# Ighina/MultimodalTopicSegmentation

Measured on AMD Instinct MI355X. Metric: sentences/sec (fwd+bwd), higher is better.
Workload: dtype bf16; 1 GPU; BASELINE configs[1]: restricted-window transformer tagger d=1792 heads=8 ff=256 radius=15 layers=1 focal loss, 64 docs x 256 sentences per GPU, fwd+bwd+Adam(eps 1e-7), inputs resident in HBM; global_batch_docs=64, sentences_per_doc=256, parallelism=dp1 (document-sharded, RCCL all-reduce)

## Files before the change

include/mts.h:

```cpp
#ifndef MTS_H
#define MTS_H

#include <stddef.h>
#include <stdint.h>

#ifdef __cplusplus
extern "C" {
#endif

typedef enum {
  MTS_OK = 0,
  MTS_ERR_INVALID = 1,
  MTS_ERR_UNSUPPORTED = 2,
  MTS_ERR_LAUNCH = 3,
  MTS_ERR_WORKSPACE = 4,
  MTS_ERR_TIMEOUT = 5
} mts_status;

typedef enum { MTS_F32 = 0, MTS_BF16 = 1 } mts_dtype;

typedef enum { MTS_LOSS_CE = 0, MTS_LOSS_BCE = 1, MTS_LOSS_FOCAL = 2 } mts_loss_kind;

typedef enum { MTS_NT = 0, MTS_NN = 1, MTS_TN = 2, MTS_TT = 3 } mts_gemm_layout;

#define MTS_EPI_BIAS      1u
#define MTS_EPI_RESIDUAL  2u
#define MTS_EPI_GELU      4u
#define MTS_EPI_COLSCALE  8u
#define MTS_EPI_ACCUM    16u
#define MTS_EPI_RELU     32u

const char* mts_last_error(void);
const char* mts_version(void);
int mts_set_option(const char* key, int value);
int mts_async_status(void);
int mts_gemm_last_plan(int* tile, int* splits);
int mts_gemm_set_mid_hook(void (*fn)(void));
size_t mts_wgrad_pair_workspace(int M, int N, int K);
int mts_wgrad_pair(void* stream, int M, int N, int K, const void* A1, const void* B1, float* C1, int ldc1, const void* A2, const void* B2,
                   float* C2t, int ldc2t, int lda, int ldb, int accumulate, void* workspace, size_t workspace_bytes);
int mts_gemm_plan(int a_dtype, int c_dtype, int layout, int M, int N, int K, unsigned epilogue, size_t workspace_bytes,
                  int* tile, int* splits);

int mts_gemm(void* stream, int a_dtype, int c_dtype, int layout, int M, int N, int K,
             const void* A, int lda, const void* B, int ldb, void* C, int ldc,
             const float* bias, const void* residual, int ldr, void* aux, int ldaux,
             unsigned epilogue, float colscale, int ncols_scaled, void* workspace, size_t workspace_bytes);

size_t mts_colsum_workspace(int N);
int mts_colsum(void* stream, int dtype, int M, int N, const void* X, int ldx, float* out, int accumulate,
               void* partial);

int mts_cast(void* stream, int dst_dtype, const float* src, void* dst, size_t n);
int mts_cast_concat(void* stream, int dst_dtype, size_t rows, int D1, int D2, const float* src1, const float* src2, void* dst);
int mts_collate_pad(int src_dtype, int dst_dtype, int B, int Lmax, int D, const void* const* docs, const int64_t* doc_rows, void* dst,
                    float pad_value, int nthreads);
int mts_gather_pad(void* stream, int src_dtype, int dst_dtype, int B, int Lmax, int D,
                   const void* corpus,
                   const int64_t* row_start,
                   int n_docs,
                   const int32_t* doc_index,
                   void* dst,
                   float pad_value);
int mts_gather_segments(void* stream, int src_dtype, int dst_dtype, int B, int Lmax, int D,
                        const void* corpus,
                        const int64_t* row_start,
                        int n_docs,
                        const int32_t* doc_index,
                        const int32_t* seg_ptr,
                        const int32_t* seg_dst,
                        const int32_t* seg_src,
                        int n_listed,
                        const int32_t* dst_len,
                        const int32_t* close_last,
                        void* dst,
                        float pad_value);
int mts_mask_plan(void* stream, int B, int Lmax,
                  const float* targets,
                  const int64_t* row_start,
                  int n_docs,
                  const int32_t* doc_index,
                  const uint64_t* doc_seed,
                  double keep_probability,
                  int32_t* src_row,
                  int32_t* kept);
int mts_gather_rows(void* stream, int src_dtype, int dst_dtype, int B, int Lmax, int D,
                    const void* corpus,
                    const int64_t* row_start,
                    int n_docs,
                    const int32_t* doc_index,
                    const int32_t* src_row,
                    void* dst,
                    float pad_value);
int mts_pca_colsum(void* stream, int dtype, int rows, int D,
                   const void* x,
                   double* sum_out);
int mts_pca_gram(void* stream, int dtype, int rows, int D,
                 const void* x,
                 const float* center,
                 double* gram_out);
int mts_pca_project(void* stream, int in_dtype, int out_dtype, int rows, int D, int k,
                    const void* x,
                    const float* center,
                    const float* w,
                    void* y);
typedef enum { MTS_POOL_NONE = 0, MTS_POOL_MEAN = 1, MTS_POOL_MAX = 2 } mts_pool_stat;
typedef enum { MTS_EDGE_LAST = 0, MTS_EDGE_DELTA_GAP = 1 } mts_edge_mode;
int mts_frame_pool(void* stream, int in_dtype, int out_dtype, int n_sent, int D, int first, int with_std,
                   const void* frames,
                   int64_t total_frames,
                   const int64_t* frame_start,
                   void* out,
                   int64_t ld_out);
int mts_frame_edges(void* stream, int in_dtype, int out_dtype, int n_sent, int D, int mode,
                    const void* frames,
                    int64_t total_frames,
                    const int64_t* frame_start,
                    const uint8_t* doc_last,
                    void* out,
                    int64_t ld_out);

int mts_embed_layernorm_fwd(void* stream, int dtype, int B, int L, int D, const float* x, const float* pos,
                            int pos_offset, const float* type0, const float* gamma, const float* beta, float eps,
                            void* y, void* pre, float* mean, float* rstd, const int32_t* row_src, int n_rows);
int mts_embed_layernorm_fwd_x16(void* stream, int B, int L, int D, const void* x_bf16, const float* pos, int pos_offset, const float* type0,
                                const float* gamma, const float* beta, float eps, void* y, void* pre, float* mean, float* rstd,
                                const int32_t* row_src, int n_rows);
int mts_embed_layernorm_fwd2(void* stream, int dtype, int B, int L, int D1, int D2, const float* x1, const float* x2, const float* pos,
                             int pos_offset, const float* type0, const float* gamma, const float* beta, float eps,
                             void* y, void* pre, float* mean, float* rstd, const int32_t* row_src, int n_rows);
int mts_layernorm_fwd(void* stream, int dtype, int rows, int D, const void* x, const float* gamma,
                      const float* beta, float eps, void* y, float* mean, float* rstd,
                      const float* head_w, const float* head_b, int n_out, float* scores);
size_t mts_layernorm_bwd_workspace(int D);
int mts_layernorm_bwd(void* stream, int dtype, int rows, int D, const void* x, const void* dy,
                      const float* dlogit, const float* head_w, int n_out,
                      const float* gamma, const float* mean, const float* rstd,
                      void* dx, float* dgamma, float* dbeta, float* dxsum, void* partial,
                      const float* beta, float* dhead_w, float* dhead_b);
int mts_layernorm_loss_tail_supported(int dtype, int D, int n_out);
int mts_layernorm_loss_tail(void* stream, int dtype, int rows, int D, const void* x, const float* gamma, const float* beta, float eps,
                            const float* head_w, const float* head_b, int n_out, int loss_kind, int B, int L, int Lt, const float* targets,
                            const int32_t* lengths, float alpha, float gamma_focal, float grad_scale, const int32_t* row_src, int n_rows,
                            float* scores, float* loss_out, void* dx, float* dgamma, float* dbeta, float* dxsum, float* dhead_w,
                            float* dhead_b, void* workspace);
size_t mts_embed_layernorm_bwd_workspace(int B, int L, int D);
int mts_embed_layernorm_bwd(void* stream, int dtype, int B, int L, int D, const void* pre, const void* dh, const float* gamma,
                            const float* mean, const float* rstd, float* dgamma, float* dbeta, float* dtype0, float* dpos,
                            int pos_offset, const int32_t* row0, const int32_t* lengths, int n_rows, void* workspace, size_t workspace_bytes);
int mts_embed_bwd(void* stream, int dtype, int B, int L, int D, const void* dpre, float* dpos, int pos_offset,
                  const int32_t* row0, const int32_t* lengths);

int mts_dropout_fwd(void* stream, int dtype, size_t n, const void* x, const void* residual, void* y, uint8_t* mask,
                    float p, uint64_t seed);
int mts_dropout_bwd(void* stream, int dtype, size_t n, const void* dy, void* dx, const uint8_t* mask, float p);

int mts_gelu_bwd(void* stream, int dtype, size_t n, const void* u, void* dy);
int mts_relu_bwd(void* stream, int dtype, size_t n, const void* u, void* dy);

int mts_ffn_supported(int dtype, int M, int D, int F);
int mts_ffn_fwd(void* stream, int M, int D, int F, const void* a1, const void* w1, const float* b1, const void* w2, const float* b2,
                int relu, void* u, void* f, void* s2);
int mts_ffn_bwd_data(void* stream, int M, int D, int F, const void* ds2, const void* w1, const void* w2, const void* u, int relu,
                     void* du, void* da1);


int mts_band_slots(int radius);
int mts_band_attn_fwd(void* stream, int dtype, int B, int L, int D, int heads, int radius,
                      const void* qkv, const int32_t* lengths, void* ctx, float* probs, const int32_t* row0,
                      float drop_p, uint64_t drop_seed);
size_t mts_band_attn_bwd_workspace(int B, int L, int D);
int mts_band_attn_bwd(void* stream, int dtype, int B, int L, int D, int heads, int radius, float q_scale,
                      const void* qkv, const int32_t* lengths, const float* probs, const void* dctx,
                      void* dqkv, float* dscores, float* dbias, void* workspace, const int32_t* row0, int n_rows,
                      float drop_p, uint64_t drop_seed);

int mts_full_attn_fwd(void* stream, int dtype, int B, int L, int D, int heads, const void* qkv, const int32_t* lengths,
                      void* ctx, float* lse, const int32_t* row0, float drop_p, uint64_t drop_seed);
size_t mts_full_attn_bwd_workspace(int B, int L, int D, int heads);
int mts_full_attn_bwd(void* stream, int dtype, int B, int L, int D, int heads, float q_scale, const void* qkv,
                      const int32_t* lengths, const float* lse, const void* ctx, const void* dctx, void* dqkv, float* dbias,
                      void* workspace, const int32_t* row0, int n_rows, float drop_p, uint64_t drop_seed);

int mts_t5_local_attn_fwd(void* stream, int dtype, int B, int L, int heads, int head_dim, int radius, const void* qkv,
                          const int32_t* lengths, const float* table, int buckets, const int32_t* bucket_of_offset, void* ctx,
                          float* lse, float drop_p, uint64_t drop_seed);
size_t mts_t5_local_attn_bwd_workspace(int B, int L, int heads, int radius);
int mts_t5_local_attn_bwd(void* stream, int dtype, int B, int L, int heads, int head_dim, int radius, const void* qkv,
                          const int32_t* lengths, const float* table, int buckets, const int32_t* bucket_of_offset,
                          const float* lse, const void* ctx, const void* dctx, void* dqkv, float* dtable, void* workspace,
                          float drop_p, uint64_t drop_seed);

int mts_rmsnorm_fwd(void* stream, int dtype, int rows, int D, const void* x, const float* w, float eps, void* y, float* rstd);
size_t mts_rmsnorm_bwd_workspace(int rows, int D);
int mts_rmsnorm_bwd(void* stream, int dtype, int rows, int D, const void* x, const void* dy, const void* dres, const float* w,
                    const float* rstd, void* dx, float* dw, void* workspace);

int mts_pair_score_fwd(void* stream, int dtype, int B, int L, int H, const void* F, int ldf, const void* G, int ldg, float* scores);
int mts_pair_score_bwd(void* stream, int dtype, int B, int L, int H, const void* F, int ldf, const void* G, int ldg,
                       const float* dscores, void* dF, int lddf, void* dG, int lddg);

int mts_gate_merge_fwd(void* stream, int dtype, size_t rows, int W, const void* a, int lda, const void* h1, int ldh1, const void* h2,
                       int ldh2, void* m, int ldm);
int mts_gate_merge_bwd(void* stream, int dtype, size_t rows, int W, const void* a, int lda, const void* h1, int ldh1, const void* h2,
                       int ldh2, const void* dm, int lddm, void* da, int ldda, void* dh1, int lddh1, void* dh2, int lddh2);

size_t mts_segment_cosine_workspace(int n_seg, int n_pair, int W);
int mts_segment_cosine_fwd(void* stream, int dtype, int B, int L, int W, const void* x, int ldx, int n_seg, const int32_t* seg_table,
                           int n_pair, const int32_t* pair_table, float* loss_out, float* pair_cos, void* workspace);
int mts_segment_cosine_bwd(void* stream, int dtype, int B, int L, int W, int n_seg, const int32_t* seg_table, int n_pair,
                           const int32_t* pair_table, const int32_t* row_map, float scale, int accumulate, void* dx, int lddx,
                           void* workspace);

size_t mts_tagger_loss_workspace(int B, int L);
int mts_tagger_loss(void* stream, int loss_kind, int B, int L, int Lt, int n_out, const float* scores,
                    const float* targets, const int32_t* lengths, float alpha, float gamma,
                    float* loss_out, float* dscores, void* workspace, size_t workspace_bytes,
                    const int32_t* row_src, int n_rows);
int mts_greedy_decode(void* stream, int B, int L, int n_out, const float* scores, const int32_t* lengths,
                      float threshold, uint8_t* tags_out);
int mts_segment_decode(void* stream, int B, int L, int n_out,
                       const float* scores,
                       const int32_t* lengths,
                       float threshold, int min_segment, int close_last, int Smax,
                       uint8_t* tags,
                       float* prob,
                       int32_t* seg_end,
                       int32_t* n_seg);
int mts_threshold_sweep(void* stream, int B, int L, int Lt, int n_out, const float* scores, const float* targets,
                        const int32_t* lengths, int T, const float* thresholds, int end_boundary, int32_t* counts_out);
int mts_winpr_sweep(void* stream, int B, int L, int Lt, int n_out, const float* scores, const float* targets,
                    const int32_t* lengths, int T, const float* thresholds, int end_boundary, int k, int32_t* counts_out);
int mts_bootstrap_sums(void* stream, int n, int M, int S, const double* values, uint64_t seed, double* sums);
int mts_head_fwd(void* stream, int dtype, int rows, int D, int n_out, const void* x, int ldx, const float* w,
                 const float* b, float* scores);
int mts_head_bwd_params(void* stream, int dtype, int rows, int D, int n_out, const void* x, int ldx,
                        const float* dscores, float* dw, float* db, void* partial);
int mts_head_bwd_data(void* stream, int dtype, int rows, int D, int n_out, const float* dscores, const float* w,
                      void* dx, int lddx, int accumulate);

int mts_switch_head_fwd(void* stream, int dtype, int B, int L, int D, int n_out, const void* x, int ldx, const float* w,
                        const float* bias, const int32_t* doc_src, const int32_t* doc_head, float* scores);
size_t mts_switch_head_bwd_workspace(int D);
int mts_switch_head_bwd_params(void* stream, int dtype, int B, int L, int D, int n_out, const void* x, int ldx, const float* dscores,
                               const int32_t* doc_src, const int32_t* doc_head, float* dw, float* db, void* workspace);
int mts_switch_head_bwd_data(void* stream, int dtype, int B, int L, int D, int n_out, const float* dscores, const float* w,
                             const int32_t* doc_tgt, void* dx, int lddx);

size_t mts_lstm_workspace(int dtype, int B, int L, int H, int ndir);
int mts_lstm_fwd(void* stream, int dtype, int B, int L, int H, int ndir, const void* xproj, const float* w_hh,
                 const float* b_hh, const int32_t* lengths, void* out, void* gates, float* cells, void* workspace);
int mts_lstm_bwd(void* stream, int dtype, int B, int L, int H, int ndir, const float* w_hh, const int32_t* lengths,
                 const void* out, const void* gates, const float* cells, const void* dout, void* dxproj,
                 float* dw_hh, void* workspace);
int mts_lstm_bwd_recurrence(void* stream, int dtype, int B, int L, int H, int ndir, const float* w_hh, const int32_t* lengths,
                            const void* out, const void* gates, const float* cells, const void* dout, void* dxproj, void* workspace);
int mts_lstm_bwd_whh(void* stream, int dtype, int B, int L, int H, int ndir, const int32_t* lengths, const void* out, const void* dxproj,
                     float* dw_hh, void* workspace);

size_t mts_crf_workspace(int B, int L, int C);
int mts_crf_nll(void* stream, int B, int L, int C, const float* feats, const float* tags, int Lt,
                const int32_t* lengths, const float* trans, float* loss_out, float* dfeats, float* dtrans,
                float* workspace );
int mts_crf_viterbi(void* stream, int B, int L, int C, const float* feats, const int32_t* lengths,
                    const float* trans, float* best_score, int32_t* paths, int32_t* bp_ws);
int mts_crf_marginals(void* stream, int B, int L, int C, int cls, const float* feats, const int32_t* lengths,
                      const float* trans, float* scores, float* logz, float* workspace );
int mts_crf_nll_packed(void* stream, int B, int L, int C, const float* feats, const float* tags, int Lt,
                       const int32_t* lengths, const float* trans, float* loss_out, float* dfeats, float* dtrans,
                       float* workspace, const int32_t* row0, int n_rows);
int mts_crf_viterbi_packed(void* stream, int B, int L, int C, const float* feats, const int32_t* lengths,
                           const float* trans, float* best_score, int32_t* paths, int32_t* bp_ws, const int32_t* row0, int n_rows);
int mts_crf_marginals_packed(void* stream, int B, int L, int C, int cls, const float* feats, const int32_t* lengths,
                             const float* trans, float* scores, float* logz, float* workspace, const int32_t* row0, int n_rows);

int mts_adam_step(void* stream, size_t n, float* param, const float* grad, float* exp_avg, float* exp_avg_sq,
                  float lr, float beta1, float beta2, float eps, int step, float grad_scale, void* bf16_copy);
int mts_sgd_step(void* stream, size_t n, float* param, const float* grad, float* momentum_buf, float lr,
                 float momentum, float weight_decay, int first_step, float grad_scale, void* bf16_copy);
size_t mts_grad_norm_workspace(void);
int mts_grad_norm(void* stream, const float* grad, int n_spans, const size_t* span_begin_host, const size_t* span_end_host,
                  float grad_scale, float* workspace, float* norm_out);
int mts_adam_step_clipped(void* stream, size_t n, float* param, const float* grad, float* exp_avg, float* exp_avg_sq,
                          float lr, float beta1, float beta2, float eps, int step, float grad_scale, void* bf16_copy,
                          const float* total_norm, float max_norm, float clip_value, float* clip_coef_out);
int mts_sgd_step_clipped(void* stream, size_t n, float* param, const float* grad, float* momentum_buf, float lr,
                         float momentum, float weight_decay, int first_step, float grad_scale, void* bf16_copy,
                         const float* total_norm, float max_norm, float clip_value, float* clip_coef_out);
int mts_scale(void* stream, size_t n, float* x, float scale);

#ifdef __cplusplus
}
#endif
#endif
```

multimodaltopicsegmentation_amd/_lib.py:

```python
import ctypes as C
import os

_HWQ_PRESET = 'GPU_MAX_HW_QUEUES' in os.environ
os.environ.setdefault('GPU_MAX_HW_QUEUES', '8')

import torch

if not _HWQ_PRESET and torch.cuda.is_initialized():
    import warnings
    warnings.warn('multimodaltopicsegmentation_amd was imported after the GPU runtime had been initialised: GPU_MAX_HW_QUEUES=8 could not '
                  'take effect (the late-fusion tagger\'s two encoder streams may share a hardware queue next to RCCL: 13.3 instead of 7.7 ms '
                  'per step at 64 x 512).  Import the package first, or export GPU_MAX_HW_QUEUES=8.', RuntimeWarning, stacklevel=2)

_HERE = os.path.dirname(os.path.abspath(__file__))
LIB_PATH = os.path.join(_HERE, 'libmts_hip.so')

if not os.path.exists(LIB_PATH):
    raise ImportError(
        f'{LIB_PATH} not found: the HIP kernel library has not been built. Run '
        '`python multimodaltopicsegmentation_amd/build.py` (needs hipcc; cross-compiles for gfx950 without a GPU). '
        'There is no CPU/PyTorch fallback for the tagger path.')

lib = C.CDLL(LIB_PATH)

F32, BF16 = 0, 1
LOSS_CE, LOSS_BCE, LOSS_FOCAL = 0, 1, 2
NT, NN, TN, TT = 0, 1, 2, 3
POOL_NONE, POOL_MEAN, POOL_MAX = 0, 1, 2
EDGE_LAST, EDGE_DELTA_GAP = 0, 1
EPI_BIAS, EPI_RESIDUAL, EPI_GELU, EPI_COLSCALE, EPI_ACCUM, EPI_RELU = 1, 2, 4, 8, 16, 32

_vp, _i, _f, _u, _sz = C.c_void_p, C.c_int, C.c_float, C.c_uint, C.c_size_t

SIGNATURES = {
    'mts_last_error': (C.c_char_p, []),
    'mts_version': (C.c_char_p, []),
    'mts_set_option': (_i, [C.c_char_p, _i]),
    'mts_gemm_last_plan': (_i, [_vp, _vp]),
    'mts_gemm_set_mid_hook': (_i, [_vp]),
    'mts_gemm_plan': (_i, [_i, _i, _i, _i, _i, _i, _u, _sz, _vp, _vp]),
    'mts_async_status': (_i, []),
    'mts_gemm': (_i, [_vp, _i, _i, _i, _i, _i, _i, _vp, _i, _vp, _i, _vp, _i, _vp, _vp, _i, _vp, _i, _u, _f, _i, _vp, _sz]),
    'mts_wgrad_pair_workspace': (_sz, [_i, _i, _i]),
    'mts_wgrad_pair': (_i, [_vp, _i, _i, _i, _vp, _vp, _vp, _i, _vp, _vp, _vp, _i, _i, _i, _i, _vp, _sz]),
    'mts_colsum_workspace': (_sz, [_i]),
    'mts_colsum': (_i, [_vp, _i, _i, _i, _vp, _i, _vp, _i, _vp]),
    'mts_cast': (_i, [_vp, _i, _vp, _vp, _sz]),
    'mts_cast_concat': (_i, [_vp, _i, _sz, _i, _i, _vp, _vp, _vp]),
    'mts_embed_layernorm_fwd2': (_i, [_vp, _i, _i, _i, _i, _i, _vp, _vp, _vp, _i, _vp, _vp, _vp, _f, _vp, _vp, _vp, _vp, _vp, _i]),
    'mts_embed_layernorm_fwd': (_i, [_vp, _i, _i, _i, _i, _vp, _vp, _i, _vp, _vp, _vp, _f, _vp, _vp, _vp, _vp, _vp, _i]),
    'mts_embed_layernorm_fwd_x16': (_i, [_vp, _i, _i, _i, _vp, _vp, _i, _vp, _vp, _vp, _f, _vp, _vp, _vp, _vp, _vp, _i]),
    'mts_layernorm_fwd': (_i, [_vp, _i, _i, _i, _vp, _vp, _vp, _f, _vp, _vp, _vp, _vp, _vp, _i, _vp]),
    'mts_layernorm_bwd_workspace': (_sz, [_i]),
    'mts_layernorm_bwd': (_i, [_vp, _i, _i, _i, _vp, _vp, _vp, _vp, _i, _vp, _vp, _vp, _vp, _vp, _vp, _vp, _vp, _vp, _vp, _vp]),
    'mts_layernorm_loss_tail_supported': (_i, [_i, _i, _i]),
    'mts_layernorm_loss_tail': (_i, [_vp, _i, _i, _i, _vp, _vp, _vp, _f, _vp, _vp, _i, _i, _i, _i, _i, _vp, _vp, _f, _f, _f, _vp, _i, _vp, _vp, _vp, _vp, _vp,
                                     _vp, _vp, _vp, _vp]),
    'mts_embed_layernorm_bwd_workspace': (_sz, [_i, _i, _i]),
    'mts_embed_layernorm_bwd': (_i, [_vp, _i, _i, _i, _i, _vp, _vp, _vp, _vp, _vp, _vp, _vp, _vp, _vp, _i, _vp, _vp, _i, _vp, _sz]),
    'mts_embed_bwd': (_i, [_vp, _i, _i, _i, _i, _vp, _vp, _i, _vp, _vp]),
    'mts_dropout_fwd': (_i, [_vp, _i, _sz, _vp, _vp, _vp, _vp, _f, C.c_uint64]),
    'mts_dropout_bwd': (_i, [_vp, _i, _sz, _vp, _vp, _vp, _f]),
    'mts_gelu_bwd': (_i, [_vp, _i, _sz, _vp, _vp]),
    'mts_relu_bwd': (_i, [_vp, _i, _sz, _vp, _vp]),
    'mts_ffn_supported': (_i, [_i, _i, _i, _i]),
    'mts_ffn_fwd': (_i, [_vp, _i, _i, _i, _vp, _vp, _vp, _vp, _vp, _i, _vp, _vp, _vp]),
    'mts_ffn_bwd_data': (_i, [_vp, _i, _i, _i, _vp, _vp, _vp, _vp, _i, _vp, _vp]),
    'mts_band_slots': (_i, [_i]),
    'mts_band_attn_fwd': (_i, [_vp, _i, _i, _i, _i, _i, _i, _vp, _vp, _vp, _vp, _vp, _f, C.c_uint64]),
    'mts_band_attn_bwd_workspace': (_sz, [_i, _i, _i]),
    'mts_band_attn_bwd': (_i, [_vp, _i, _i, _i, _i, _i, _i, _f, _vp, _vp, _vp, _vp, _vp, _vp, _vp, _vp, _vp, _i, _f, C.c_uint64]),
    'mts_full_attn_fwd': (_i, [_vp, _i, _i, _i, _i, _i, _vp, _vp, _vp, _vp, _vp, _f, C.c_uint64]),
    'mts_full_attn_bwd_workspace': (_sz, [_i, _i, _i, _i]),
    'mts_full_attn_bwd': (_i, [_vp, _i, _i, _i, _i, _i, _f, _vp, _vp, _vp, _vp, _vp, _vp, _vp, _vp, _vp, _i, _f, C.c_uint64]),
    'mts_t5_local_attn_fwd': (_i, [_vp, _i, _i, _i, _i, _i, _i, _vp, _vp, _vp, _i, _vp, _vp, _vp, _f, C.c_uint64]),
    'mts_t5_local_attn_bwd_workspace': (_sz, [_i, _i, _i, _i]),
    'mts_t5_local_attn_bwd': (_i, [_vp, _i, _i, _i, _i, _i, _i, _vp, _vp, _vp, _i, _vp, _vp, _vp, _vp, _vp, _vp, _vp, _f, C.c_uint64]),
    'mts_rmsnorm_fwd': (_i, [_vp, _i, _i, _i, _vp, _vp, _f, _vp, _vp]),
    'mts_rmsnorm_bwd_workspace': (_sz, [_i, _i]),
    'mts_rmsnorm_bwd': (_i, [_vp, _i, _i, _i, _vp, _vp, _vp, _vp, _vp, _vp, _vp, _vp]),
    'mts_pair_score_fwd': (_i, [_vp, _i, _i, _i, _i, _vp, _i, _vp, _i, _vp]),
    'mts_pair_score_bwd': (_i, [_vp, _i, _i, _i, _i, _vp, _i, _vp, _i, _vp, _vp, _i, _vp, _i]),
    'mts_gate_merge_fwd': (_i, [_vp, _i, _sz, _i, _vp, _i, _vp, _i, _vp, _i, _vp, _i]),
    'mts_gate_merge_bwd': (_i, [_vp, _i, _sz, _i, _vp, _i, _vp, _i, _vp, _i, _vp, _i, _vp, _i, _vp, _i, _vp, _i]),
    'mts_segment_cosine_workspace': (_sz, [_i, _i, _i]),
    'mts_segment_cosine_fwd': (_i, [_vp, _i, _i, _i, _i, _vp, _i, _i, _vp, _i, _vp, _vp, _vp, _vp]),
    'mts_segment_cosine_bwd': (_i, [_vp, _i, _i, _i, _i, _i, _vp, _i, _vp, _vp, _f, _i, _vp, _i, _vp]),
    'mts_tagger_loss_workspace': (_sz, [_i, _i]),
    'mts_tagger_loss': (_i, [_vp, _i, _i, _i, _i, _i, _vp, _vp, _vp, _f, _f, _vp, _vp, _vp, _sz, _vp, _i]),
    'mts_greedy_decode': (_i, [_vp, _i, _i, _i, _vp, _vp, _f, _vp]),
    'mts_segment_decode': (_i, [_vp, _i, _i, _i, _vp, _vp, _f, _i, _i, _i, _vp, _vp, _vp, _vp]),
    'mts_threshold_sweep': (_i, [_vp, _i, _i, _i, _i, _vp, _vp, _vp, _i, _vp, _i, _vp]),
    'mts_winpr_sweep': (_i, [_vp, _i, _i, _i, _i, _vp, _vp, _vp, _i, _vp, _i, _i, _vp]),
    'mts_bootstrap_sums': (_i, [_vp, _i, _i, _i, _vp, C.c_uint64, _vp]),
    'mts_head_fwd': (_i, [_vp, _i, _i, _i, _i, _vp, _i, _vp, _vp, _vp]),
    'mts_head_bwd_params': (_i, [_vp, _i, _i, _i, _i, _vp, _i, _vp, _vp, _vp, _vp]),
    'mts_head_bwd_data': (_i, [_vp, _i, _i, _i, _i, _vp, _vp, _vp, _i, _i]),
    'mts_switch_head_fwd': (_i, [_vp, _i, _i, _i, _i, _i, _vp, _i, _vp, _vp, _vp, _vp, _vp]),
    'mts_switch_head_bwd_workspace': (_sz, [_i]),
    'mts_switch_head_bwd_params': (_i, [_vp, _i, _i, _i, _i, _i, _vp, _i, _vp, _vp, _vp, _vp, _vp, _vp]),
    'mts_switch_head_bwd_data': (_i, [_vp, _i, _i, _i, _i, _i, _vp, _vp, _vp, _vp, _i]),
    'mts_lstm_workspace': (_sz, [_i, _i, _i, _i, _i]),
    'mts_lstm_fwd': (_i, [_vp, _i, _i, _i, _i, _i, _vp, _vp, _vp, _vp, _vp, _vp, _vp, _vp]),
    'mts_lstm_bwd': (_i, [_vp, _i, _i, _i, _i, _i, _vp, _vp, _vp, _vp, _vp, _vp, _vp, _vp, _vp]),
    'mts_lstm_bwd_recurrence': (_i, [_vp, _i, _i, _i, _i, _i, _vp, _vp, _vp, _vp, _vp, _vp, _vp, _vp]),
    'mts_lstm_bwd_whh': (_i, [_vp, _i, _i, _i, _i, _i, _vp, _vp, _vp, _vp, _vp]),
    'mts_crf_workspace': (_sz, [_i, _i, _i]),
    'mts_crf_nll': (_i, [_vp, _i, _i, _i, _vp, _vp, _i, _vp, _vp, _vp, _vp, _vp, _vp]),
    'mts_crf_viterbi': (_i, [_vp, _i, _i, _i, _vp, _vp, _vp, _vp, _vp, _vp]),
    'mts_crf_marginals': (_i, [_vp, _i, _i, _i, _i, _vp, _vp, _vp, _vp, _vp, _vp]),
    'mts_crf_nll_packed': (_i, [_vp, _i, _i, _i, _vp, _vp, _i, _vp, _vp, _vp, _vp, _vp, _vp, _vp, _i]),
    'mts_crf_viterbi_packed': (_i, [_vp, _i, _i, _i, _vp, _vp, _vp, _vp, _vp, _vp, _vp, _i]),
    'mts_crf_marginals_packed': (_i, [_vp, _i, _i, _i, _i, _vp, _vp, _vp, _vp, _vp, _vp, _vp, _i]),
    'mts_adam_step': (_i, [_vp, _sz, _vp, _vp, _vp, _vp, _f, _f, _f, _f, _i, _f, _vp]),
    'mts_sgd_step': (_i, [_vp, _sz, _vp, _vp, _vp, _f, _f, _f, _i, _f, _vp]),
    'mts_grad_norm_workspace': (_sz, []),
    'mts_grad_norm': (_i, [_vp, _vp, _i, _vp, _vp, _f, _vp, _vp]),
    'mts_adam_step_clipped': (_i, [_vp, _sz, _vp, _vp, _vp, _vp, _f, _f, _f, _f, _i, _f, _vp, _vp, _f, _f, _vp]),
    'mts_sgd_step_clipped': (_i, [_vp, _sz, _vp, _vp, _vp, _f, _f, _f, _i, _f, _vp, _vp, _f, _f, _vp]),
    'mts_scale': (_i, [_vp, _sz, _vp, _f]),
    'mts_collate_pad': (_i, [_i, _i, _i, _i, _i, _vp, _vp, _vp, _f, _i]),
    'mts_gather_pad': (_i, [_vp, _i, _i, _i, _i, _i, _vp, _vp, _i, _vp, _vp, _f]),
    'mts_gather_segments': (_i, [_vp, _i, _i, _i, _i, _i, _vp, _vp, _i, _vp, _vp, _vp, _vp, _i, _vp, _vp, _vp, _f]),
    'mts_mask_plan': (_i, [_vp, _i, _i, _vp, _vp, _i, _vp, _vp, C.c_double, _vp, _vp]),
    'mts_gather_rows': (_i, [_vp, _i, _i, _i, _i, _i, _vp, _vp, _i, _vp, _vp, _vp, _f]),
    'mts_pca_colsum': (_i, [_vp, _i, _i, _i, _vp, _vp]),
    'mts_pca_gram': (_i, [_vp, _i, _i, _i, _vp, _vp, _vp]),
    'mts_pca_project': (_i, [_vp, _i, _i, _i, _i, _i, _vp, _vp, _vp, _vp]),
    'mts_frame_pool': (_i, [_vp, _i, _i, _i, _i, _i, _i, _vp, C.c_int64, _vp, _vp, C.c_int64]),
    'mts_frame_edges': (_i, [_vp, _i, _i, _i, _i, _i, _vp, C.c_int64, _vp, _vp, _vp, C.c_int64]),
}

_missing = []
for _name, (_res, _args) in SIGNATURES.items():
    try:
        _fn = getattr(lib, _name)
    except AttributeError:
        _missing.append(_name)
        continue
    _fn.restype = _res
    _fn.argtypes = _args
if _missing:
    raise ImportError(f'{LIB_PATH} does not export {_missing}: stale build? re-run python multimodaltopicsegmentation_amd/build.py --force')


class MtsError(RuntimeError):
    pass


def check(rc):
    if rc != 0:
        msg = lib.mts_last_error().decode('utf-8', 'replace')
        if rc == 1:
            raise ValueError(msg)
        if rc == 2:
            raise NotImplementedError(msg)
        if rc == 5:
            raise MtsError(f'device-side timeout: {msg}')
        raise MtsError(f'mts error {rc}: {msg}')


def check_async():
    check(lib.mts_async_status())


def stream_ptr():
    return torch.cuda.current_stream().cuda_stream


def ptr(t):
    return None if t is None else t.data_ptr()


def dtype_code(dt):
    if dt == torch.float32:
        return F32
    if dt == torch.bfloat16:
        return BF16
    raise ValueError(f'unsupported activation dtype {dt}')


def require_gpu():
    if not torch.cuda.is_available():
        raise RuntimeError('multimodaltopicsegmentation_amd: no GPU visible. The tagger path runs only on its HIP kernels '
                           '(MI355X / gfx950); there is no CPU fallback.')
```

multimodaltopicsegmentation_amd/csrc/gemm.hip:

```cpp
#include <algorithm>
#include <math.h>
#include <stdlib.h>
#include "common.h"

#include "gemm_common.h"


template <int LAYOUT, typename TC, bool GLDS>
__global__ __launch_bounds__(256, 2) void gemm_bf16_kernel(const GemmArgs a) {
  constexpr bool A_KMAJOR = (LAYOUT == MTS_NT || LAYOUT == MTS_NN);
  constexpr bool B_KMAJOR = (LAYOUT == MTS_NT || LAYOUT == MTS_TT);
  extern __shared__ __attribute__((aligned(16))) char smem[];

  const int tid = threadIdx.x;
  const int lane = tid & 63;
  const int wave = tid >> 6;
  const int wm = wave >> 1, wn = wave & 1;
  const int r16 = lane & 15, g = lane >> 4;

  const int ntn = (a.N + BN - 1) / BN;
  const int ntm = (a.M + BM - 1) / BM;
  const int nt = ntn * ntm;
  int bid = xcd_remap(blockIdx.x, nt);
  const int bm0 = (ntm < ntn ? bid % ntm : bid / ntn) * BM;
// ... 479 lines not shown
                                                            int ldc, int accumulate) {
  const size_t idx = (size_t)blockIdx.x * 256 + threadIdx.x;
  const int n4 = N / 4;
  if (idx >= (size_t)M * n4) return;
  const int m = (int)(idx / n4), n = 4 * (int)(idx % n4);
  float s[4] = {0.f, 0.f, 0.f, 0.f};
  if (accumulate) load4<float>(C + (size_t)m * ldc + n, s);
  const size_t plane = (size_t)M * N;
  for (int z = 0; z < splits; ++z) {
    float v[4];
    load4<float>(slab + z * plane + (size_t)m * N + n, v);
#pragma unroll
    for (int i = 0; i < 4; ++i) s[i] += v[i];
  }
  store4<float>(C + (size_t)m * ldc + n, s);
}

__global__ __launch_bounds__(256) void splitk_reduce_t_kernel(const float* __restrict__ slab, int splits, int M, int N, float* __restrict__ Ct,
                                                              int ldc, int accumulate) {
  __shared__ float tile[32][33];
  const int n0 = blockIdx.x * 32, m0 = blockIdx.y * 32;
  const int tx = threadIdx.x & 31, ty = threadIdx.x >> 5;
  const size_t plane = (size_t)M * N;
#pragma unroll
  for (int r = ty; r < 32; r += 8) {
    const int m = m0 + r, n = n0 + tx;
    float s = 0.f;
    if (m < M && n < N) {
      const float* p = slab + (size_t)m * N + n;
      int z = 0;
      for (; z + 7 < splits; z += 8) {
        float v[8];
#pragma unroll
        for (int u = 0; u < 8; ++u) v[u] = p[(size_t)(z + u) * plane];
#pragma unroll
        for (int u = 0; u < 8; ++u) s += v[u];
      }
      for (; z < splits; ++z) s += p[(size_t)z * plane];
    }
    tile[r][tx] = s;
  }
  __syncthreads();
#pragma unroll
  for (int r = ty; r < 32; r += 8) {
    const int n = n0 + r, m = m0 + tx;
    if (n < N && m < M) {
      float* o = Ct + (size_t)n * ldc + m;
      *o = accumulate ? *o + tile[tx][r] : tile[tx][r];
    }
  }
}

template <typename T> __global__ void cast_kernel(const float* __restrict__ src, T* __restrict__ dst, size_t n) {
  size_t i = ((size_t)blockIdx.x * blockDim.x + threadIdx.x) * 4;
  const size_t stride = (size_t)gridDim.x * blockDim.x * 4;
  for (; i + 3 < n; i += stride) {
    float v[4];
    load4<float>(src + i, v);
    store4<T>(dst + i, v);
  }
  if (i < n && i + 3 >= n)
    for (size_t j = i; j < n; ++j) dst[j] = from_f32<T>(src[j]);
}

template <typename T> __global__ void cast_concat_kernel(const float* __restrict__ s1, const float* __restrict__ s2, T* __restrict__ dst,
                                                          size_t rows, int D1, int D2) {
  const int D = D1 + D2, q = D / 4;
  const size_t total = rows * q;
  for (size_t i = (size_t)blockIdx.x * blockDim.x + threadIdx.x; i < total; i += (size_t)gridDim.x * blockDim.x) {
    const size_t r = i / q;
    const int e = (int)(i - r * q) * 4;
    float v[4];
    load4<float>(e < D1 ? s1 + r * D1 + e : s2 + r * D2 + (e - D1), v);
    store4<T>(dst + r * D + e, v);
  }
}

extern "C" int mts_cast_concat(void* stream, int dst_dtype, size_t rows, int D1, int D2, const float* src1, const float* src2, void* dst) {
  MTS_CHECK_ARG(src1 && src2 && dst && D1 > 0 && D2 > 0 && D1 % 4 == 0 && D2 % 4 == 0, "mts_cast_concat: bad arguments (widths must be multiples of 4)");
  if (rows == 0) return MTS_OK;
  const int blocks = (int)std::min<size_t>(4096, (rows * ((D1 + D2) / 4) + 255) / 256);
  if (dst_dtype == MTS_BF16) hipLaunchKernelGGL(cast_concat_kernel<bf16_t>, dim3(blocks), dim3(256), 0, (hipStream_t)stream, src1, src2, (bf16_t*)dst, rows, D1, D2);
  else if (dst_dtype == MTS_F32) hipLaunchKernelGGL(cast_concat_kernel<float>, dim3(blocks), dim3(256), 0, (hipStream_t)stream, src1, src2, (float*)dst, rows, D1, D2);
  else { mts_set_error("mts_cast_concat: bad dtype %d", dst_dtype); return MTS_ERR_INVALID; }
  MTS_LAUNCH_CHECK("mts_cast_concat");
  return MTS_OK;
}

extern "C" size_t mts_colsum_workspace(int N) { return (size_t)COLSUM_RS * (size_t)N * sizeof(float); }

extern "C" int mts_colsum(void* stream, int dtype, int M, int N, const void* X, int ldx, float* out, int accumulate,
                          void* partial) {
  MTS_CHECK_ARG(M > 0 && N > 0 && X && out && partial, "mts_colsum: bad arguments");
  MTS_CHECK_ARG(dtype == MTS_F32 || dtype == MTS_BF16, "mts_colsum: bad dtype %d", dtype);
  MTS_CHECK_ARG(ldx % 4 == 0, "mts_colsum: ldx must be a multiple of 4");
  hipStream_t st = (hipStream_t)stream;
  const int nparts = min(COLSUM_RS, M);
  dim3 grid(ceil_div(N, 64), COLSUM_RS);
  (void)nparts;
  if (dtype == MTS_F32)
    hipLaunchKernelGGL(colsum_partial_kernel<float>, grid, dim3(256), 0, st, (const float*)X, M, N, ldx, (float*)partial);
  else
    hipLaunchKernelGGL(colsum_partial_kernel<bf16_t>, grid, dim3(256), 0, st, (const bf16_t*)X, M, N, ldx, (float*)partial);
  hipLaunchKernelGGL(colsum_final_kernel, dim3(ceil_div(N, 64)), dim3(256), 0, st, (const float*)partial, N, COLSUM_RS, out,
                     accumulate);
  MTS_LAUNCH_CHECK("mts_colsum");
  return MTS_OK;
}

extern "C" int mts_cast(void* stream, int dst_dtype, const float* src, void* dst, size_t n) {
  MTS_CHECK_ARG(src && dst, "mts_cast: null pointer");
  if (n == 0) return MTS_OK;
  hipStream_t st = (hipStream_t)stream;
  const int blocks = (int)std::min<size_t>(2048, (n / 4 + 255) / 256 + 1);
  if (dst_dtype == MTS_BF16)
    hipLaunchKernelGGL(cast_kernel<bf16_t>, dim3(blocks), dim3(256), 0, st, src, (bf16_t*)dst, n);
  else if (dst_dtype == MTS_F32)
    hipLaunchKernelGGL(cast_kernel<float>, dim3(blocks), dim3(256), 0, st, src, (float*)dst, n);
  else {
    mts_set_error("mts_cast: bad dtype %d", dst_dtype);
    return MTS_ERR_INVALID;
  }
  MTS_LAUNCH_CHECK("mts_cast");
  return MTS_OK;
}

int mts_launch_gemm256(const GemmArgs& a, int layout, bool c_is_f32, int splits, hipStream_t st);
int mts_launch_gemm224(const GemmArgs& a, int layout, bool c_is_f32, int splits, hipStream_t st);
bool mts_gemm224t_applies(const GemmArgs& a, int layout, bool c_is_f32, int splits);

static thread_local int g_gemm_glds = -1;
static thread_local int g_tile_mode = -1;
static thread_local int g_force_splits = 0;
static thread_local int g_tile_order = 1;
static thread_local int g_gemm_deep = 1;
static thread_local int g_chain = 0;
static thread_local int g_combine = 0;
#define MTS_GEMM_WS_HEAD 8192
static thread_local int g_last_tile = 0, g_last_splits = 0;

static thread_local void (*g_mid_hook)(void) = nullptr;
extern "C" int mts_gemm_set_mid_hook(void (*fn)(void)) { g_mid_hook = fn; return MTS_OK; }

extern "C" int mts_gemm_last_plan(int* tile, int* splits) {
  if (tile) *tile = g_last_tile;
  if (splits) *splits = g_last_splits;
  return MTS_OK;
}

void mts_band_set_mfma(int on);
void mts_band_set_fused(int on);
void mts_full_set_mfma(int on);
void mts_t5_set_mfma(int on);
static thread_local int g_f32_mfma = 1;
static thread_local int g_big_min_k = 256;
static thread_local int g_gemm_variant = 0;
void mts_lstm_pair_set_spin_limit(int n);
void mts_lstm_pair_set_max_pairs(int n);
void mts_lstm_pair_set_parts(int n);
extern "C" int mts_set_option(const char* key, int value) {
  if (!key) return MTS_ERR_INVALID;
  if (!strcmp(key, "gemm_tile")) { g_tile_mode = value; return MTS_OK; }
  if (!strcmp(key, "gemm_glds")) { g_gemm_glds = value; return MTS_OK; }
  if (!strcmp(key, "gemm_splits")) { g_force_splits = value; return MTS_OK; }
  if (!strcmp(key, "gemm_order")) { g_tile_order = value; return MTS_OK; }
  if (!strcmp(key, "gemm_chain")) { g_chain = value; return MTS_OK; }
  if (!strcmp(key, "gemm_combine")) { g_combine = value; return MTS_OK; }
  if (!strcmp(key, "gemm_deep")) { g_gemm_deep = value; return MTS_OK; }
  if (!strcmp(key, "gemm_variant")) { g_gemm_variant = value; return MTS_OK; }
  if (!strcmp(key, "gemm_big_min_k")) { g_big_min_k = value; return MTS_OK; }
  if (!strcmp(key, "gemm_f32_mfma")) { g_f32_mfma = value; return MTS_OK; }
  if (!strcmp(key, "band_mfma")) { mts_band_set_mfma(value); return MTS_OK; }
  if (!strcmp(key, "band_fused_bwd")) { mts_band_set_fused(value); return MTS_OK; }
  if (!strcmp(key, "full_mfma")) { mts_full_set_mfma(value); return MTS_OK; }
  if (!strcmp(key, "t5_mfma")) { mts_t5_set_mfma(value); return MTS_OK; }
  if (!strcmp(key, "lstm_pair_spin_limit")) { mts_lstm_pair_set_spin_limit(value); return MTS_OK; }
  if (!strcmp(key, "lstm_pair_max_pairs")) { mts_lstm_pair_set_max_pairs(value); return MTS_OK; }
  if (!strcmp(key, "lstm_parts")) { mts_lstm_pair_set_parts(value); return MTS_OK; }
  mts_set_error("mts_set_option: unknown key %s", key);
  return MTS_ERR_INVALID;
}

template <int LAYOUT, typename TC>
static void launch_bf16(const GemmArgs& a, int splits, hipStream_t st) {
  const int nt = ceil_div(a.M, BM) * ceil_div(a.N, BN);
  if (g_gemm_glds < 0) {
    const char* e = getenv("MTS_GEMM_GLDS");
    g_gemm_glds = (e && e[0] == '0') ? 0 : 1;
  }
  const bool glds = g_gemm_glds && (a.K % BK == 0) && (a.ksplit % BK == 0) && a.M >= 8 && a.N >= 8;
  if (glds) {
    GemmArgs b = a;
    const bool deep = g_gemm_deep && (size_t)nt * splits <= 256 && a.ksplit >= 4 * BK;
    b.nbuf = deep ? 4 : 2;
    auto k = gemm_bf16_kernel<LAYOUT, TC, true>;
    if (deep && mts_dyn_lds(k, 8 * TILE_BYTES, "gemm") != MTS_OK) b.nbuf = 2;
    hipLaunchKernelGGL(k, dim3(nt, 1, splits), dim3(256), (b.nbuf == 4 ? 8 : 4) * TILE_BYTES, st, b);
  } else {
    hipLaunchKernelGGL((gemm_bf16_kernel<LAYOUT, TC, false>), dim3(nt, 1, splits), dim3(256), 4 * TILE_BYTES, st, a);
  }
}

static void plan_bf16(int c_dtype, int layout, int M, int N, int K, unsigned epilogue, bool has_workspace, size_t workspace_bytes,
                      int* use256_out, int* splits_out) {
  if (g_tile_mode < 0) {
    const char* e = getenv("MTS_GEMM_TILE");
    g_tile_mode = e ? atoi(e) : 0;
  }
  const int tile_mode = g_tile_mode;
  const unsigned plain = epilogue & ~MTS_EPI_ACCUM;
  const bool can_split = (c_dtype == MTS_F32 && plain == 0 && has_workspace && N % 4 == 0 && K >= 2048);
  const bool can256 = (K % BK == 0) && K >= g_big_min_k && M >= 8 && N >= 8 && tile_mode != 128;
  const double bw = 3500.0;
  double best = 1e30;
  int splits = 1;
  int use256 = 0;
  const bool can224 = can256 && (N % 224 == 0) && tile_mode != 256;
  for (int big = 0; big <= (can256 ? 2 : 0); ++big) {
    if (big == 2 && !can224) continue;
    if (tile_mode == 256 && can256 && big != 1) continue;
    if (tile_mode == 224 && can224 && big != 2) continue;
    const int tile = big ? 256 : 128;
    const double slots = big ? 256.0 : 512.0;
    const double t_k = layout == MTS_TN ? (big == 2 ? (M % 256 == 0 ? 0.0160 : 0.0200) : big == 1 ? 0.0218 : 0.0145)
                                        : (big ? 0.0232 * (big == 2 ? 0.875 : 1.0) : 0.0180);
    const double t_0 = big ? 7.7 : 6.5;
    const int nt = ceil_div(M, tile) * (big == 2 ? N / 224 : ceil_div(N, tile));
    for (int sp = 1; sp <= (can_split ? 32 : 1); ++sp) {
      const int ks = ceil_div(ceil_div(K, sp), BK) * BK;
      if (ceil_div(K, ks) != sp) continue;
      if (sp > 1 && (size_t)sp * M * N * sizeof(float) > workspace_bytes) break;
      if (g_force_splits > 0 && can_split && sp != g_force_splits) continue;
      const double rounds = ceil((double)nt * sp / slots);
      const double cost = rounds * (ks * t_k + t_0) + (sp > 1 ? (2.0 * sp + 1.0) * M * N * 4.0 / 1e6 / bw : 0.0);
      if (cost < best) { best = cost; splits = sp; use256 = big; }
    }
  }
  *use256_out = use256;
  *splits_out = splits;
}

int mts_gemm224_last_kernel();
int mts_launch_gemm224t_pair(const GemmArgs& a, int splits, const void* A2, const void* B2, float* slab2, hipStream_t st);
bool mts_gemm224t_applies(const GemmArgs& a, int layout, bool c_is_f32, int splits);

static int wgrad_pair_splits(int M, int N, int K, size_t workspace_bytes) {
  if (M % 256 || N % 224 || K % 64 || K < 256) return -1;
  static int cus = 0;
  if (!cus) { int dev = 0; hipDeviceProp_t pr; cus = (hipGetDevice(&dev) == hipSuccess && hipGetDeviceProperties(&pr, dev) == hipSuccess) ? pr.multiProcessorCount : 256; }
  const int nt = (M / 256) * (N / 224);
  int sp = std::max(1, std::min(32, cus / (2 * nt)));
  for (; sp >= 1; --sp) {
    const int ks = ceil_div(ceil_div(K, sp), BK) * BK;
    if (ceil_div(K, ks) != sp) continue;
    if (ks >= 128 && K - (sp - 1) * ks >= 128 && (size_t)2 * sp * M * N * sizeof(float) <= workspace_bytes) return sp;
  }
  return -1;
}
extern "C" size_t mts_wgrad_pair_workspace(int M, int N, int K) {
  const int sp = wgrad_pair_splits(M, N, K, (size_t)-1);
  return sp < 1 ? 0 : (size_t)2 * sp * M * N * sizeof(float);
}
extern "C" int mts_wgrad_pair(void* stream, int M, int N, int K, const void* A1, const void* B1, float* C1, int ldc1, const void* A2, const void* B2,
                              float* C2t, int ldc2t, int lda, int ldb, int accumulate, void* workspace, size_t workspace_bytes) {
  MTS_CHECK_ARG(M > 0 && N > 0 && K > 0 && A1 && B1 && C1 && A2 && B2 && C2t && workspace, "mts_wgrad_pair: bad arguments");
  MTS_CHECK_ARG(ldc1 >= N && ldc2t >= M && ldc1 % 4 == 0, "mts_wgrad_pair: bad output strides");
  const int sp = wgrad_pair_splits(M, N, K, workspace_bytes);
  MTS_UNSUPPORTED(sp >= 1, "mts_wgrad_pair: M=%d N=%d K=%d not covered (M %% 256, N %% 224, K %% 64) or workspace too small", M, N, K);
  hipStream_t st = (hipStream_t)stream;
  GemmArgs a;
  memset(&a, 0, sizeof(a));
  a.A = A1; a.B = B1; a.C = C1;
  a.M = M; a.N = N; a.K = K; a.lda = lda; a.ldb = ldb; a.ldc = ldc1;
  a.epi = 0; a.colscale = 1.0f;
  a.ksplit = ceil_div(ceil_div(K, sp), BK) * BK;
  a.order = 1; a.nbuf = 2; a.variant = 0;
  float* const planes = (float*)workspace;
  a.slab = planes;
  float* const planes2 = planes + (size_t)sp * M * N;
  MTS_UNSUPPORTED(mts_gemm224t_applies(a, MTS_TN, true, sp), "mts_wgrad_pair: operands not covered by the four-wave weight-gradient kernel (alignment / strides)");
  const int rc = mts_launch_gemm224t_pair(a, sp, A2, B2, planes2, st);
  MTS_UNSUPPORTED(rc == MTS_OK, "mts_wgrad_pair: launch refused");
  hipLaunchKernelGGL(splitk_reduce_kernel, dim3((unsigned)(((size_t)M * (N / 4) + 255) / 256)), dim3(256), 0, st, (const float*)planes, sp, M, N, C1, ldc1,
                     accumulate ? 1 : 0);
  hipLaunchKernelGGL(splitk_reduce_t_kernel, dim3(ceil_div(N, 32), ceil_div(M, 32)), dim3(256), 0, st, (const float*)planes2, sp, M, N, C2t, ldc2t,
                     accumulate ? 1 : 0);
  MTS_LAUNCH_CHECK("mts_wgrad_pair");
  return MTS_OK;
}

extern "C" int mts_gemm_plan(int a_dtype, int c_dtype, int layout, int M, int N, int K, unsigned epilogue, size_t workspace_bytes,
                             int* tile, int* splits) {
  MTS_CHECK_ARG(M > 0 && N > 0 && K > 0, "mts_gemm_plan: bad shape M=%d N=%d K=%d", M, N, K);
  MTS_CHECK_ARG(layout == MTS_NT || layout == MTS_NN || layout == MTS_TN || layout == MTS_TT, "mts_gemm_plan: bad layout %d", layout);
  MTS_CHECK_ARG(a_dtype == MTS_F32 || a_dtype == MTS_BF16, "mts_gemm_plan: bad a_dtype %d", a_dtype);
  int use256 = 0, sp = 1;
  const size_t ws_planes = workspace_bytes > MTS_GEMM_WS_HEAD ? workspace_bytes - MTS_GEMM_WS_HEAD : 0;
  if (a_dtype == MTS_BF16) plan_bf16(c_dtype, layout, M, N, K, epilogue, ws_planes > 0, ws_planes, &use256, &sp);
  if (tile) *tile = a_dtype == MTS_F32 ? (g_f32_mfma ? 128 : 64) : use256 == 2 ? 224 : use256 == 1 ? 256 : 128;
  if (splits) *splits = sp;
  return MTS_OK;
}

extern "C" int mts_gemm(void* stream, int a_dtype, int c_dtype, int layout, int M, int N, int K, const void* A, int lda,
                        const void* B, int ldb, void* C, int ldc, const float* bias, const void* residual, int ldr,
                        void* aux, int ldaux, unsigned epilogue, float colscale, int ncols_scaled, void* workspace, size_t workspace_bytes) {
  MTS_CHECK_ARG(M > 0 && N > 0 && K > 0, "mts_gemm: bad shape M=%d N=%d K=%d", M, N, K);
  MTS_CHECK_ARG(A && B && C, "mts_gemm: null operand");
  MTS_CHECK_ARG(layout == MTS_NT || layout == MTS_NN || layout == MTS_TN || layout == MTS_TT, "mts_gemm: bad layout %d", layout);
  MTS_CHECK_ARG(a_dtype == MTS_F32 || a_dtype == MTS_BF16, "mts_gemm: bad a_dtype %d", a_dtype);
  MTS_CHECK_ARG(c_dtype == MTS_F32 || c_dtype == a_dtype, "mts_gemm: c_dtype must be f32 or a_dtype");
  MTS_CHECK_ARG(!(epilogue & MTS_EPI_BIAS) || bias, "mts_gemm: MTS_EPI_BIAS without bias");
  MTS_CHECK_ARG(!(epilogue & MTS_EPI_RESIDUAL) || residual, "mts_gemm: MTS_EPI_RESIDUAL without residual");
  MTS_CHECK_ARG(!(epilogue & MTS_EPI_ACCUM) || c_dtype == MTS_F32, "mts_gemm: MTS_EPI_ACCUM needs fp32 C");
  MTS_CHECK_ARG((epilogue & (MTS_EPI_GELU | MTS_EPI_RELU)) != (MTS_EPI_GELU | MTS_EPI_RELU), "mts_gemm: MTS_EPI_GELU and MTS_EPI_RELU are exclusive");
  hipStream_t st = (hipStream_t)stream;
  GemmArgs a;
  a.A = A; a.B = B; a.C = C; a.bias = bias; a.residual = residual; a.aux = aux;
  a.M = M; a.N = N; a.K = K; a.lda = lda; a.ldb = ldb; a.ldc = ldc; a.ldr = ldr; a.ldaux = ldaux;
  a.epi = epilogue; a.colscale = colscale; a.ncols_scaled = ncols_scaled;
  a.variant = g_gemm_variant;
#ifdef MTS_GEMM_STAMPS
  a.stamps = nullptr;
#endif
  a.ksplit = K; a.slab = nullptr; a.chain = nullptr; a.order = g_tile_order; a.nbuf = 2;

  if (a_dtype == MTS_F32) {
    StrideArgs s;
    if (layout == MTS_NT) { s.sam = lda; s.sak = 1; s.sbn = ldb; s.sbk = 1; }
    else if (layout == MTS_NN) { s.sam = lda; s.sak = 1; s.sbn = 1; s.sbk = ldb; }
    else if (layout == MTS_TT) { s.sam = 1; s.sak = lda; s.sbn = ldb; s.sbk = 1; }
    else { s.sam = 1; s.sak = lda; s.sbn = 1; s.sbk = ldb; }
    MTS_CHECK_ARG(ldc % 4 == 0 && ((uintptr_t)C % 16) == 0, "mts_gemm(f32): C must be 16-byte aligned with ldc %% 4 == 0");
    MTS_CHECK_ARG(!(epilogue & MTS_EPI_RESIDUAL) || (ldr % 4 == 0 && ((uintptr_t)residual % 16) == 0), "mts_gemm(f32): residual must be 16-byte aligned with ldr %% 4 == 0");
    MTS_CHECK_ARG(!aux || (ldaux % 4 == 0 && ((uintptr_t)aux % 16) == 0), "mts_gemm(f32): aux must be 16-byte aligned with ldaux %% 4 == 0");
    const int nt = ceil_div(M, F32_BM) * ceil_div(N, F32_BM);
    int splits = 1;
    if (g_f32_mfma && workspace && !(epilogue & ~MTS_EPI_ACCUM) && N % 4 == 0 && nt <= 128 && K >= 1024) {
      splits = std::min(std::min(16, 256 / nt), K / 512);
      while (splits > 1 && (size_t)splits * M * N * sizeof(float) > workspace_bytes) --splits;
    }
    g_last_tile = 128;
    g_last_splits = splits;
    if (splits > 1) {
      a.ksplit = ceil_div(ceil_div(K, splits), F32_BK) * F32_BK;
      splits = ceil_div(K, a.ksplit);
      a.slab = (float*)workspace;
    }
    if (g_f32_mfma) hipLaunchKernelGGL(gemm_f32_mfma_kernel, dim3(nt, 1, splits), dim3(256), 0, st, a, s);
    else hipLaunchKernelGGL(gemm_f32_kernel, dim3(ceil_div(M, 64) * ceil_div(N, 64)), dim3(256), 0, st, a, s);
    if (splits > 1)
      hipLaunchKernelGGL(splitk_reduce_kernel, dim3((unsigned)(((size_t)M * (N / 4) + 255) / 256)), dim3(256), 0, st, (const float*)workspace,
                         splits, M, N, (float*)C, ldc, (epilogue & MTS_EPI_ACCUM) ? 1 : 0);
    MTS_LAUNCH_CHECK("mts_gemm(f32)");
    return MTS_OK;
  }

  MTS_UNSUPPORTED(lda % 8 == 0 && ldb % 8 == 0 && ((uintptr_t)A % 16) == 0 && ((uintptr_t)B % 16) == 0,
                  "mts_gemm(bf16): A/B must be 16-byte aligned with ld %% 8 == 0 (lda=%d ldb=%d)", lda, ldb);
  if (layout == MTS_NT) MTS_UNSUPPORTED(K % 8 == 0, "mts_gemm(bf16,NT): K %% 8 != 0 (K=%d)", K);
  if (layout == MTS_NN) MTS_UNSUPPORTED(K % 8 == 0 && N % 8 == 0, "mts_gemm(bf16,NN): K,N %% 8 (K=%d N=%d)", K, N);
  if (layout == MTS_TN) MTS_UNSUPPORTED(M % 8 == 0 && N % 8 == 0, "mts_gemm(bf16,TN): M,N %% 8 (M=%d N=%d)", M, N);
  if (layout == MTS_TT) MTS_UNSUPPORTED(M % 8 == 0 && K % 8 == 0, "mts_gemm(bf16,TT): M,K %% 8 (M=%d K=%d)", M, K);
  MTS_UNSUPPORTED(ldc % 4 == 0 && ((uintptr_t)C % (c_dtype == MTS_F32 ? 16 : 8)) == 0, "mts_gemm(bf16): C alignment/ldc");
  MTS_UNSUPPORTED(!(epilogue & MTS_EPI_RESIDUAL) || (ldr % 4 == 0 && ((uintptr_t)residual % 8) == 0), "mts_gemm(bf16): residual alignment");
  MTS_UNSUPPORTED(!aux || (ldaux % 4 == 0 && ((uintptr_t)aux % 8) == 0), "mts_gemm(bf16): aux alignment");

  int splits = 1, use256 = 0;
  const size_t ws_planes = workspace_bytes > MTS_GEMM_WS_HEAD ? workspace_bytes - MTS_GEMM_WS_HEAD : 0;
  float* const planes = workspace ? (float*)((char*)workspace + MTS_GEMM_WS_HEAD) : nullptr;
  plan_bf16(c_dtype, layout, M, N, K, epilogue, workspace != nullptr && ws_planes > 0, ws_planes, &use256, &splits);
  if (use256 && c_dtype != MTS_F32 && ((uintptr_t)C % 16) != 0) use256 = 0;
  g_last_tile = use256 == 2 ? 224 : use256 == 1 ? 256 : 128;
  g_last_splits = splits;
  a.slab = nullptr;
  bool chained = false;
  if (splits > 1) {
    a.ksplit = ceil_div(ceil_div(K, splits), BK) * BK;
    chained = g_chain && !use256;
    if (chained) {
      const size_t nt128 = (size_t)ceil_div(M, BM) * ceil_div(N, BN);
      a.chain = (unsigned*)planes;
      hipError_t e = hipMemsetAsync(planes, 0, nt128 * sizeof(unsigned), st);
      if (e != hipSuccess) { mts_set_error("mts_gemm: hipMemsetAsync: %s", hipGetErrorString(e)); return MTS_ERR_LAUNCH; }
    } else {
      a.slab = planes;
      if (use256 == 2 && g_combine && (a.variant == 0 || a.variant == 11 || a.variant == 12) && (size_t)ceil_div(M, 256) * (N / 224) * sizeof(unsigned) <= MTS_GEMM_WS_HEAD &&
          mts_gemm224t_applies(a, layout, c_dtype == MTS_F32, splits)) {
        a.chain = (unsigned*)workspace;
        chained = true;
      }
    }
  }
  if (use256) {
    int rc = use256 == 2 ? mts_launch_gemm224(a, layout, c_dtype == MTS_F32, splits, st) : mts_launch_gemm256(a, layout, c_dtype == MTS_F32, splits, st);
    if (rc) return rc;
    if (use256 == 2) g_last_tile = mts_gemm224_last_kernel();
  } else if (c_dtype == MTS_F32) {
    if (layout == MTS_NT) launch_bf16<MTS_NT, float>(a, splits, st);
    else if (layout == MTS_NN) launch_bf16<MTS_NN, float>(a, splits, st);
    else if (layout == MTS_TT) launch_bf16<MTS_TT, float>(a, splits, st);
    else launch_bf16<MTS_TN, float>(a, splits, st);
  } else {
    if (layout == MTS_NT) launch_bf16<MTS_NT, bf16_t>(a, splits, st);
    else if (layout == MTS_NN) launch_bf16<MTS_NN, bf16_t>(a, splits, st);
    else if (layout == MTS_TT) launch_bf16<MTS_TT, bf16_t>(a, splits, st);
    else launch_bf16<MTS_TN, bf16_t>(a, splits, st);
  }
  if (g_mid_hook) g_mid_hook();
  if (splits > 1 && !chained)
    hipLaunchKernelGGL(splitk_reduce_kernel, dim3((unsigned)(((size_t)M * (N / 4) + 255) / 256)), dim3(256), 0, st, (const float*)planes,
                       splits, M, N, (float*)C, ldc, (epilogue & MTS_EPI_ACCUM) ? 1 : 0);
  MTS_LAUNCH_CHECK("mts_gemm(bf16)");
  return MTS_OK;
}
```

multimodaltopicsegmentation_amd/csrc/optim.hip:

```cpp
#include <stdarg.h>
#include <algorithm>
#include <math.h>
#include <mutex>
#include "common.h"

static thread_local char g_err[512] = "";
void mts_set_error(const char* fmt, ...) {
  va_list ap;
  va_start(ap, fmt);
  vsnprintf(g_err, sizeof(g_err), fmt, ap);
  va_end(ap);
}
extern "C" const char* mts_last_error(void) { return g_err; }

enum { LDS_KERNELS = 256, LDS_DEVICES = 16 };
struct LdsEntry { const void* fn; std::atomic<uint32_t> bytes[LDS_DEVICES]; };
static LdsEntry g_lds[LDS_KERNELS];
static std::atomic<int> g_lds_n{0};
static std::mutex g_lds_mu;

static LdsEntry* lds_find(const void* kernel, int n) {
  for (int i = 0; i < n; ++i)
    if (g_lds[i].fn == kernel) return &g_lds[i];
  return nullptr;
}

int mts_dyn_lds(const void* kernel, size_t bytes, const char* who) {
  MTS_UNSUPPORTED(bytes <= 160 * 1024, "%s: needs %zu bytes of LDS (> 160 KiB)", who, bytes);
  if (bytes <= 64 * 1024) return MTS_OK;
  int dev = 0;
  hipError_t e = hipGetDevice(&dev);
  if (e != hipSuccess) { mts_set_error("%s: hipGetDevice: %s", who, hipGetErrorString(e)); return MTS_ERR_LAUNCH; }
  const bool tracked = dev >= 0 && dev < LDS_DEVICES;
  LdsEntry* x = tracked ? lds_find(kernel, g_lds_n.load(std::memory_order_acquire)) : nullptr;
  if (x && x->bytes[dev].load(std::memory_order_acquire) >= bytes) return MTS_OK;
  std::lock_guard<std::mutex> lk(g_lds_mu);
  if (tracked && !x) {
    const int n = g_lds_n.load(std::memory_order_relaxed);
    x = lds_find(kernel, n);
    if (!x && n < LDS_KERNELS) {
      x = &g_lds[n];
      x->fn = kernel;
      g_lds_n.store(n + 1, std::memory_order_release);
    }
  }
  if (x && x->bytes[dev].load(std::memory_order_relaxed) >= bytes) return MTS_OK;
  e = hipFuncSetAttribute(kernel, hipFuncAttributeMaxDynamicSharedMemorySize, (int)bytes);
  if (e != hipSuccess) { mts_set_error("%s: hipFuncSetAttribute: %s", who, hipGetErrorString(e)); return MTS_ERR_LAUNCH; }
  if (x) x->bytes[dev].store((uint32_t)bytes, std::memory_order_release);
  return MTS_OK;
}
extern "C" const char* mts_version(void) { return "mts-hip 1 gfx950"; }

enum { CLIP_NONE = 0, CLIP_NORM = 1, CLIP_VALUE = 2 };

template <int CLIP> __device__ __forceinline__ float clip_grad(float gr, float c) {
  if (CLIP == CLIP_NORM) return gr * c;
  if (CLIP == CLIP_VALUE) return gr > c ? c : (gr < -c ? -c : gr);
  return gr;
}

__device__ __forceinline__ float clip_coef(float total_norm, float max_norm) {
  const float c = max_norm / (total_norm + 1e-6f);
  return c > 1.f ? 1.f : c;
}

template <int CLIP>
__device__ __forceinline__ void adam_loop(size_t n, float* __restrict__ p, const float* __restrict__ g, float* __restrict__ m,
                                          float* __restrict__ v, float lr, float b1, float b2, float eps, float bc1, float bc2_sqrt,
                                          float gscale, bf16_t* __restrict__ copy, float c) {
  const size_t stride = (size_t)gridDim.x * 256 * 4;
  const float step_size = lr / bc1;
  for (size_t i = ((size_t)blockIdx.x * 256 + threadIdx.x) * 4; i < n; i += stride) {
    if (i + 3 < n) {
      float pv[4], gv[4], mv[4], vv[4];
      load4<float>(p + i, pv); load4<float>(g + i, gv); load4<float>(m + i, mv); load4<float>(v + i, vv);
#pragma unroll
      for (int j = 0; j < 4; ++j) {
        const float gr = clip_grad<CLIP>(gv[j] * gscale, c);
        mv[j] = mv[j] + (1.f - b1) * (gr - mv[j]);
        vv[j] = b2 * vv[j] + (1.f - b2) * gr * gr;
        const float denom = sqrtf(vv[j]) / bc2_sqrt + eps;
        pv[j] = pv[j] - step_size * (mv[j] / denom);
      }
      store4<float>(p + i, pv); store4<float>(m + i, mv); store4<float>(v + i, vv);
      if (copy) store4<bf16_t>(copy + i, pv);
    } else {
      for (size_t k = i; k < n; ++k) {
        const float gr = clip_grad<CLIP>(g[k] * gscale, c);
        const float mm = m[k] + (1.f - b1) * (gr - m[k]);
        const float vv = b2 * v[k] + (1.f - b2) * gr * gr;
        m[k] = mm; v[k] = vv;
        const float pp = p[k] - step_size * (mm / (sqrtf(vv) / bc2_sqrt + eps));
        p[k] = pp;
        if (copy) copy[k] = (bf16_t)pp;
      }
    }
  }
}

__global__ __launch_bounds__(256) void adam_kernel(size_t n, float* __restrict__ p, const float* __restrict__ g, float* __restrict__ m,
                                                   float* __restrict__ v, float lr, float b1, float b2, float eps, float bc1, float bc2_sqrt,
                                                   float gscale, bf16_t* __restrict__ copy) {
  adam_loop<CLIP_NONE>(n, p, g, m, v, lr, b1, b2, eps, bc1, bc2_sqrt, gscale, copy, 1.f);
}

template <int CLIP>
__global__ __launch_bounds__(256) void adam_clip_kernel(size_t n, float* __restrict__ p, const float* __restrict__ g, float* __restrict__ m,
                                                        float* __restrict__ v, float lr, float b1, float b2, float eps, float bc1,
                                                        float bc2_sqrt, float gscale, bf16_t* __restrict__ copy,
                                                        const float* __restrict__ total_norm, float max_norm, float clip_value,
                                                        float* __restrict__ coef_out) {
  float c = clip_value;
  if (CLIP == CLIP_NORM) {
    c = clip_coef(*total_norm, max_norm);
    if (coef_out && blockIdx.x == 0 && threadIdx.x == 0) *coef_out = c;
  }
  adam_loop<CLIP>(n, p, g, m, v, lr, b1, b2, eps, bc1, bc2_sqrt, gscale, copy, c);
}

template <int CLIP>
__device__ __forceinline__ void sgd_loop(size_t n, float* __restrict__ p, const float* __restrict__ g, float* __restrict__ buf, float lr,
                                         float mom, float wd, int first, float gscale, bf16_t* __restrict__ copy, float c) {
  const size_t stride = (size_t)gridDim.x * 256;
  for (size_t i = (size_t)blockIdx.x * 256 + threadIdx.x; i < n; i += stride) {
    float gr = clip_grad<CLIP>(g[i] * gscale, c) + wd * p[i];
    float b = first ? gr : mom * buf[i] + gr;
    buf[i] = b;
    const float pp = p[i] - lr * b;
    p[i] = pp;
    if (copy) copy[i] = (bf16_t)pp;
  }
}

__global__ __launch_bounds__(256) void sgd_kernel(size_t n, float* __restrict__ p, const float* __restrict__ g, float* __restrict__ buf, float lr,
                                                  float mom, float wd, int first, float gscale, bf16_t* __restrict__ copy) {
  sgd_loop<CLIP_NONE>(n, p, g, buf, lr, mom, wd, first, gscale, copy, 1.f);
}

template <int CLIP>
__global__ __launch_bounds__(256) void sgd_clip_kernel(size_t n, float* __restrict__ p, const float* __restrict__ g, float* __restrict__ buf,
                                                       float lr, float mom, float wd, int first, float gscale, bf16_t* __restrict__ copy,
                                                       const float* __restrict__ total_norm, float max_norm, float clip_value,
                                                       float* __restrict__ coef_out) {
  float c = clip_value;
  if (CLIP == CLIP_NORM) {
    c = clip_coef(*total_norm, max_norm);
    if (coef_out && blockIdx.x == 0 && threadIdx.x == 0) *coef_out = c;
  }
  sgd_loop<CLIP>(n, p, g, buf, lr, mom, wd, first, gscale, copy, c);
}

extern "C" int mts_adam_step(void* stream, size_t n, float* param, const float* grad, float* exp_avg, float* exp_avg_sq, float lr, float beta1,
                             float beta2, float eps, int step, float grad_scale, void* bf16_copy) {
  MTS_CHECK_ARG(param && grad && exp_avg && exp_avg_sq && step >= 1, "mts_adam_step: bad arguments");
  if (n == 0) return MTS_OK;
  const double bc1 = 1.0 - pow((double)beta1, step), bc2 = 1.0 - pow((double)beta2, step);
  const int blocks = (int)std::min<size_t>(2048, (n / 4 + 255) / 256 + 1);
  hipLaunchKernelGGL(adam_kernel, dim3(blocks), dim3(256), 0, (hipStream_t)stream, n, param, grad, exp_avg, exp_avg_sq, lr, beta1, beta2, eps,
                     (float)bc1, (float)sqrt(bc2), grad_scale, (bf16_t*)bf16_copy);
  MTS_LAUNCH_CHECK("mts_adam_step");
  return MTS_OK;
}

extern "C" int mts_sgd_step(void* stream, size_t n, float* param, const float* grad, float* momentum_buf, float lr, float momentum,
                            float weight_decay, int first_step, float grad_scale, void* bf16_copy) {
  MTS_CHECK_ARG(param && grad && momentum_buf, "mts_sgd_step: bad arguments");
  if (n == 0) return MTS_OK;
  const int blocks = (int)std::min<size_t>(2048, (n + 255) / 256);
  hipLaunchKernelGGL(sgd_kernel, dim3(blocks), dim3(256), 0, (hipStream_t)stream, n, param, grad, momentum_buf, lr, momentum, weight_decay,
                     first_step, grad_scale, (bf16_t*)bf16_copy);
  MTS_LAUNCH_CHECK("mts_sgd_step");
  return MTS_OK;
}

static inline bool aligned_to(const void* p, size_t bytes) { return ((uintptr_t)p & (bytes - 1)) == 0; }

static int check_clip_args(const char* name, const float* total_norm, float max_norm, float clip_value) {
  MTS_CHECK_ARG(max_norm >= 0.f, "%s: max_norm must be >= 0 (got %g)", name, (double)max_norm);
  MTS_CHECK_ARG(clip_value >= 0.f, "%s: clip_value must be >= 0 (got %g)", name, (double)clip_value);
  MTS_CHECK_ARG(total_norm ? clip_value == 0.f : clip_value > 0.f,
                "%s: give either total_norm (norm mode, clip_value 0) or clip_value > 0 without total_norm (value mode)", name);
  return MTS_OK;
}

extern "C" int mts_adam_step_clipped(void* stream, size_t n, float* param, const float* grad, float* exp_avg, float* exp_avg_sq, float lr,
                                     float beta1, float beta2, float eps, int step, float grad_scale, void* bf16_copy, const float* total_norm,
                                     float max_norm, float clip_value, float* clip_coef_out) {
  MTS_CHECK_ARG(param && grad && exp_avg && exp_avg_sq && step >= 1, "mts_adam_step_clipped: bad arguments");
  if (int rc = check_clip_args("mts_adam_step_clipped", total_norm, max_norm, clip_value)) return rc;
  MTS_CHECK_ARG(aligned_to(param, 16) && aligned_to(grad, 16) && aligned_to(exp_avg, 16) && aligned_to(exp_avg_sq, 16) && aligned_to(bf16_copy, 8),
                "mts_adam_step_clipped: param, grad and moments must be 16-byte aligned, bf16_copy 8-byte aligned");
  MTS_CHECK_ARG(aligned_to(total_norm, 4) && aligned_to(clip_coef_out, 4), "mts_adam_step_clipped: misaligned scalar");
  if (n == 0) return MTS_OK;
  const double bc1 = 1.0 - pow((double)beta1, step), bc2 = 1.0 - pow((double)beta2, step);
  const int blocks = (int)std::min<size_t>(2048, (n / 4 + 255) / 256 + 1);
  auto kernel = total_norm ? adam_clip_kernel<CLIP_NORM> : adam_clip_kernel<CLIP_VALUE>;
  hipLaunchKernelGGL(kernel, dim3(blocks), dim3(256), 0, (hipStream_t)stream, n, param, grad, exp_avg, exp_avg_sq, lr, beta1, beta2, eps,
                     (float)bc1, (float)sqrt(bc2), grad_scale, (bf16_t*)bf16_copy, total_norm, max_norm, clip_value, clip_coef_out);
  MTS_LAUNCH_CHECK("mts_adam_step_clipped");
  return MTS_OK;
}

extern "C" int mts_sgd_step_clipped(void* stream, size_t n, float* param, const float* grad, float* momentum_buf, float lr, float momentum,
                                    float weight_decay, int first_step, float grad_scale, void* bf16_copy, const float* total_norm,
                                    float max_norm, float clip_value, float* clip_coef_out) {
  MTS_CHECK_ARG(param && grad && momentum_buf, "mts_sgd_step_clipped: bad arguments");
  if (int rc = check_clip_args("mts_sgd_step_clipped", total_norm, max_norm, clip_value)) return rc;
  MTS_CHECK_ARG(aligned_to(param, 4) && aligned_to(grad, 4) && aligned_to(momentum_buf, 4) && aligned_to(bf16_copy, 2) &&
                    aligned_to(total_norm, 4) && aligned_to(clip_coef_out, 4),
                "mts_sgd_step_clipped: misaligned operand");
  if (n == 0) return MTS_OK;
  const int blocks = (int)std::min<size_t>(2048, (n + 255) / 256);
  auto kernel = total_norm ? sgd_clip_kernel<CLIP_NORM> : sgd_clip_kernel<CLIP_VALUE>;
  hipLaunchKernelGGL(kernel, dim3(blocks), dim3(256), 0, (hipStream_t)stream, n, param, grad, momentum_buf, lr, momentum, weight_decay,
                     first_step, grad_scale, (bf16_t*)bf16_copy, total_norm, max_norm, clip_value, clip_coef_out);
  MTS_LAUNCH_CHECK("mts_sgd_step_clipped");
  return MTS_OK;
}

#define NORM_MAX_SPANS 4
#define NORM_MAX_BLOCKS 2048
struct NormSpans {
  const float* p[NORM_MAX_SPANS];
  size_t n[NORM_MAX_SPANS];
};

__device__ __forceinline__ float block_sum_256(float s) {
  __shared__ float wave_part[4];
  s = wave_sum(s);
  if ((threadIdx.x & 63) == 0) wave_part[threadIdx.x >> 6] = s;
  __syncthreads();
  return (wave_part[0] + wave_part[1]) + (wave_part[2] + wave_part[3]);
}

__global__ __launch_bounds__(256) void grad_sumsq_kernel(NormSpans spans, int n_spans, float gscale, float* __restrict__ partials) {
  float acc[4] = {0.f, 0.f, 0.f, 0.f};
  const size_t stride = (size_t)gridDim.x * 256 * 4;
  const size_t first = ((size_t)blockIdx.x * 256 + threadIdx.x) * 4;
#pragma unroll
  for (int s = 0; s < NORM_MAX_SPANS; ++s) {
    if (s >= n_spans) break;
    const float* __restrict__ g = spans.p[s];
    const size_t n = spans.n[s], nv = n & ~(size_t)3;
    size_t i = first;
    for (; i + stride < nv; i += 2 * stride) {
      float a[4], b[4];
      load4<float>(g + i, a); load4<float>(g + i + stride, b);
#pragma unroll
      for (int j = 0; j < 4; ++j) { const float t = a[j] * gscale; acc[j] += t * t; }
#pragma unroll
      for (int j = 0; j < 4; ++j) { const float t = b[j] * gscale; acc[j] += t * t; }
    }
    if (i < nv) {
      float a[4];
      load4<float>(g + i, a);
#pragma unroll
      for (int j = 0; j < 4; ++j) { const float t = a[j] * gscale; acc[j] += t * t; }
    }
    if (first == 0)
      for (size_t k = nv; k < n; ++k) { const float t = g[k] * gscale; acc[0] += t * t; }
  }
  const float total = block_sum_256((acc[0] + acc[1]) + (acc[2] + acc[3]));
  if (threadIdx.x == 0) partials[blockIdx.x] = total;
}

__global__ __launch_bounds__(256) void grad_norm_finalize_kernel(const float* __restrict__ partials, int n_partials, float* __restrict__ norm_out) {
  float s = 0.f;
  for (int i = threadIdx.x; i < n_partials; i += 256) s += partials[i];
  const float total = block_sum_256(s);
  if (threadIdx.x == 0) *norm_out = sqrtf(total);
}

extern "C" size_t mts_grad_norm_workspace(void) { return NORM_MAX_BLOCKS * sizeof(float); }

extern "C" int mts_grad_norm(void* stream, const float* grad, int n_spans, const size_t* span_begin_host, const size_t* span_end_host,
                             float grad_scale, float* workspace, float* norm_out) {
  MTS_CHECK_ARG(grad && span_begin_host && span_end_host && workspace && norm_out, "mts_grad_norm: null pointer");
  MTS_CHECK_ARG(n_spans >= 1 && n_spans <= NORM_MAX_SPANS, "mts_grad_norm: n_spans must be 1..%d (got %d)", NORM_MAX_SPANS, n_spans);
  MTS_CHECK_ARG(aligned_to(workspace, 4) && aligned_to(norm_out, 4), "mts_grad_norm: misaligned workspace or result");
  NormSpans spans = {};
  size_t longest = 0;
  for (int s = 0; s < n_spans; ++s) {
    MTS_CHECK_ARG(span_end_host[s] >= span_begin_host[s], "mts_grad_norm: span %d ends before it begins", s);
    spans.p[s] = grad + span_begin_host[s];
    spans.n[s] = span_end_host[s] - span_begin_host[s];
    MTS_CHECK_ARG(aligned_to(spans.p[s], 16), "mts_grad_norm: span %d does not begin on a 16-byte boundary", s);
    longest = std::max(longest, spans.n[s]);
  }
  if (longest == 0) return MTS_OK;
  const int blocks = (int)std::min<size_t>(NORM_MAX_BLOCKS, std::max<size_t>(1, (longest / 4 + 255) / 256));
  hipLaunchKernelGGL(grad_sumsq_kernel, dim3(blocks), dim3(256), 0, (hipStream_t)stream, spans, n_spans, grad_scale, workspace);
  MTS_LAUNCH_CHECK("mts_grad_norm");
  hipLaunchKernelGGL(grad_norm_finalize_kernel, dim3(1), dim3(256), 0, (hipStream_t)stream, workspace, blocks, norm_out);
  MTS_LAUNCH_CHECK("mts_grad_norm");
  return MTS_OK;
}

__global__ __launch_bounds__(256) void scale_kernel(size_t n, float* __restrict__ x, float scale) {
  const size_t stride = (size_t)gridDim.x * 256;
  for (size_t i = (size_t)blockIdx.x * 256 + threadIdx.x; i < n; i += stride) x[i] *= scale;
}
extern "C" int mts_scale(void* stream, size_t n, float* x, float scale) {
  MTS_CHECK_ARG(x || n == 0, "mts_scale: null pointer");
  if (n == 0 || scale == 1.0f) return MTS_OK;
  const int blocks = (int)std::min<size_t>(1024, (n + 255) / 256);
  hipLaunchKernelGGL(scale_kernel, dim3(blocks), dim3(256), 0, (hipStream_t)stream, n, x, scale);
  MTS_LAUNCH_CHECK("mts_scale");
  return MTS_OK;
}
```

multimodaltopicsegmentation_amd/ops.py:

```python
import ctypes
import math

import torch

from . import _lib as L
from ._lib import check, lib, ptr, stream_ptr, dtype_code

_ws_cache = {}

TIMER = None


class KernelTimer:

    def __init__(self, only=None):
        self.records = {}
        self.only = only

    def begin(self, tag):
        if self.only is not None and not self.only(tag):
            return None
        s, e = torch.cuda.Event(enable_timing=True), torch.cuda.Event(enable_timing=True)
        self.records.setdefault(tag, []).append((s, e))
        s.record()
        return e

    def summary(self):
        return {t: (len(v), sum(s.elapsed_time(e) for s, e in v)) for t, v in self.records.items()}


_pending_end = [None]


@ctypes.CFUNCTYPE(None)
def _mid_hook():
    e = _pending_end[0]
    if e is not None:
        e.record()
        _pending_end[0] = None


_hook_installed = [False]


class _timed:
    def __init__(self, tag):
        self.tag = tag

    def __enter__(self):
        self.e = TIMER.begin(self.tag) if TIMER is not None else None
        if self.e is not None and self.tag[0] == 'gemm':
            if not _hook_installed[0]:
                lib.mts_gemm_set_mid_hook(ctypes.cast(_mid_hook, ctypes.c_void_p))
                _hook_installed[0] = True
            _pending_end[0] = self.e

    def __exit__(self, *a):
        if self.e is not None:
            if self.tag[0] == 'gemm':
                if _pending_end[0] is None:
                    return False
                _pending_end[0] = None
            self.e.record()
        return False


def _scratch(nbytes, device, tag):
    key = (str(device), tag, torch.cuda.current_stream(device).cuda_stream if torch.device(device).type == 'cuda' else 0)
    buf = _ws_cache.get(key)
    if buf is None or buf.numel() < nbytes:
        buf = torch.empty(max(int(nbytes), 1), dtype=torch.uint8, device=device)
        _ws_cache[key] = buf
    return buf


_side_streams = {}


def side_stream(device, idx=0):
    key = (str(torch.device(device)), int(idx))
    s = _side_streams.get(key)
    if s is None:
        s = _side_streams[key] = torch.cuda.Stream(device=device)
    return s


_plan_cache = {}


def gemm(layout, A, B, out, *, M, N, K, lda=None, ldb=None, ldc=None, bias=None, residual=None, aux=None, gelu=False,
         colscale=None, ncols_scaled=0, accumulate=False, relu=False):
    a_dt = dtype_code(A.dtype)
    assert B.dtype == A.dtype
    c_dt = dtype_code(out.dtype)
    epi = 0
    if bias is not None:
        epi |= L.EPI_BIAS
    if residual is not None:
        epi |= L.EPI_RESIDUAL
    if gelu:
        epi |= L.EPI_GELU
    if relu:
        epi |= L.EPI_RELU
    if colscale is not None:
        epi |= L.EPI_COLSCALE
    if accumulate:
        epi |= L.EPI_ACCUM
    lda = lda if lda is not None else A.stride(0)
    ldb = ldb if ldb is not None else B.stride(0)
    ldc = ldc if ldc is not None else out.stride(0)
    ws, ws_bytes = None, 0
    if layout in (L.TN, L.TT) and c_dt == L.F32 and K >= 2048:
        if a_dt == L.BF16:
            ws_bytes = 8192 + min(16, max(1, K // 1024)) * M * N * 4
        elif -(-M // 128) * -(-N // 128) <= 128:
            ws_bytes = min(16, 256 // (-(-M // 128) * -(-N // 128)), max(1, K // 512)) * M * N * 4
        if ws_bytes:
            ws = _scratch(ws_bytes, A.device, 'splitk')
    key = (layout, a_dt, c_dt, M, N, K)
    with _timed(('gemm', *key, _plan_cache.get(key, 0))):
        check(lib.mts_gemm(stream_ptr(), a_dt, c_dt, layout, M, N, K, ptr(A), lda, ptr(B), ldb, ptr(out), ldc, ptr(bias),
                           ptr(residual), residual.stride(0) if residual is not None else 0, ptr(aux),
                           aux.stride(0) if aux is not None else 0, epi, float(colscale or 1.0), int(ncols_scaled),
                           ptr(ws), ws_bytes))
    if a_dt == L.BF16 and key not in _plan_cache:
        t = ctypes.c_int(0)
        lib.mts_gemm_last_plan(ctypes.byref(t), None)
        _plan_cache[key] = t.value
    return out


def linear_fwd(x, w, b, out, **kw):
    return gemm(L.NT, x, w, out, M=x.shape[0], N=w.shape[0], K=x.shape[1], bias=b, **kw)


def linear_dgrad(dy, w, out, **kw):
    return gemm(L.NN, dy, w, out, M=dy.shape[0], N=w.shape[1], K=dy.shape[1], **kw)


def linear_wgrad(dy, x, out, **kw):
    return gemm(L.TN, dy, x, out, M=dy.shape[1], N=x.shape[1], K=dy.shape[0], **kw)


def wgrad_pair_supported(dy1, x1):
    return dy1.dtype == torch.bfloat16 and dy1.is_cuda and lib.mts_wgrad_pair_workspace(dy1.shape[1], x1.shape[1], dy1.shape[0]) > 0


def wgrad_pair(dy1, x1, out1, dy2, x2, out2_t, accumulate=False):
    K, M = dy1.shape
    N = x1.shape[1]
    assert dy2.shape == dy1.shape and x2.shape == x1.shape and dy2.stride(0) == dy1.stride(0) and x2.stride(0) == x1.stride(0)
    assert tuple(out1.shape) == (M, N) and out2_t.shape[0] == N and out2_t.shape[1] >= M
    nbytes = lib.mts_wgrad_pair_workspace(M, N, K)
    ws = _scratch(nbytes, dy1.device, 'wgrad_pair')
    with _timed(('wgrad_pair', M, N, K)):
        check(lib.mts_wgrad_pair(stream_ptr(), M, N, K, ptr(dy1), ptr(x1), ptr(out1), out1.stride(0), ptr(dy2), ptr(x2), ptr(out2_t), out2_t.stride(0),
                                 dy1.stride(0), x1.stride(0), 1 if accumulate else 0, ptr(ws), nbytes))


def colsum(x, out, accumulate=False):
    M, N = x.shape
    ws = _scratch(lib.mts_colsum_workspace(N), x.device, 'colsum')
    check(lib.mts_colsum(stream_ptr(), dtype_code(x.dtype), M, N, ptr(x), x.stride(0), ptr(out), int(accumulate), ptr(ws)))
    return out


def cast(src, dst):
    check(lib.mts_cast(stream_ptr(), dtype_code(dst.dtype), ptr(src), ptr(dst), src.numel()))
    return dst


def cast_concat(x1, x2, dst):
    check(lib.mts_cast_concat(stream_ptr(), dtype_code(dst.dtype), x1.shape[0], x1.shape[1], x2.shape[1], ptr(x1), ptr(x2), ptr(dst)))
    return dst


def gather_pad(corpus, row_start, doc_index, dst, pad_value=0.0):
    B, Lmax = int(dst.shape[0]), int(dst.shape[1])
    D = 1 if corpus.dim() == 1 else int(corpus.shape[1])
    assert dst.numel() == B * Lmax * D and dst.is_contiguous() and corpus.is_contiguous()
    assert row_start.dtype == torch.int64 and row_start.is_contiguous() and row_start.numel() >= 2
    assert doc_index.dtype == torch.int32 and doc_index.is_contiguous() and doc_index.numel() == B
    assert corpus.device == dst.device == row_start.device == doc_index.device
    check(lib.mts_gather_pad(stream_ptr(), dtype_code(corpus.dtype), dtype_code(dst.dtype), B, Lmax, D, ptr(corpus), ptr(row_start),
                             row_start.numel() - 1, ptr(doc_index), ptr(dst), float(pad_value)))
    return dst


def gather_segments(corpus, row_start, doc_index, seg_ptr, seg_dst, seg_src, dst_len, dst, pad_value=0.0, close_last=None):
    B, Lmax = int(dst.shape[0]), int(dst.shape[1])
    D = 1 if corpus.dim() == 1 else int(corpus.shape[1])
    assert dst.numel() == B * Lmax * D and dst.is_contiguous() and corpus.is_contiguous()
    assert row_start.dtype == torch.int64 and row_start.is_contiguous() and row_start.numel() >= 2
    tables = [doc_index, seg_ptr, seg_dst, seg_src, dst_len] + ([close_last] if close_last is not None else [])
    assert all(t.dtype == torch.int32 and t.is_contiguous() and t.device == dst.device for t in tables)
    assert doc_index.numel() == B and seg_ptr.numel() == B + 1 and dst_len.numel() == B and seg_dst.numel() == seg_src.numel()
    assert close_last is None or close_last.numel() == B
    assert corpus.device == dst.device == row_start.device
    check(lib.mts_gather_segments(stream_ptr(), dtype_code(corpus.dtype), dtype_code(dst.dtype), B, Lmax, D, ptr(corpus), ptr(row_start),
                                  row_start.numel() - 1, ptr(doc_index), ptr(seg_ptr), ptr(seg_dst), ptr(seg_src), seg_dst.numel(),
                                  ptr(dst_len), ptr(close_last), ptr(dst), float(pad_value)))
    return dst


def mask_plan(targets, row_start, doc_index, doc_seed, keep_probability, src_row, kept):
    B, Lmax = int(src_row.shape[0]), int(src_row.shape[1])
    assert targets.dtype == torch.float32 and targets.dim() == 1 and targets.is_contiguous()
    assert row_start.dtype == torch.int64 and row_start.is_contiguous() and row_start.numel() >= 2
    assert doc_index.dtype == torch.int32 and doc_index.is_contiguous() and doc_index.numel() == B
    assert doc_seed.dtype == torch.int64 and doc_seed.is_contiguous() and doc_seed.numel() == B
    assert src_row.dtype == torch.int32 and src_row.is_contiguous() and kept.dtype == torch.int32 and kept.is_contiguous() and kept.numel() == B
    assert targets.device == row_start.device == doc_index.device == doc_seed.device == src_row.device == kept.device
    check(lib.mts_mask_plan(stream_ptr(), B, Lmax, ptr(targets), ptr(row_start), row_start.numel() - 1, ptr(doc_index), ptr(doc_seed),
                            float(keep_probability), ptr(src_row), ptr(kept)))
    return src_row, kept


def gather_rows(corpus, row_start, doc_index, src_row, dst, pad_value=0.0):
    B, Lmax = int(dst.shape[0]), int(dst.shape[1])
    D = 1 if corpus.dim() == 1 else int(corpus.shape[1])
    assert dst.numel() == B * Lmax * D and dst.is_contiguous() and corpus.is_contiguous()
    assert row_start.dtype == torch.int64 and row_start.is_contiguous() and row_start.numel() >= 2
    assert doc_index.dtype == torch.int32 and doc_index.is_contiguous() and doc_index.numel() == B
    assert src_row.dtype == torch.int32 and src_row.is_contiguous() and tuple(src_row.shape) == (B, Lmax)
    assert corpus.device == dst.device == row_start.device == doc_index.device == src_row.device
    check(lib.mts_gather_rows(stream_ptr(), dtype_code(corpus.dtype), dtype_code(dst.dtype), B, Lmax, D, ptr(corpus), ptr(row_start),
                              row_start.numel() - 1, ptr(doc_index), ptr(src_row), ptr(dst), float(pad_value)))
    return dst


def _pca_matrix(x):
    assert x.dim() == 2 and x.is_contiguous() and x.is_cuda, 'a contiguous [rows, D] device matrix is expected'
    return int(x.shape[0]), int(x.shape[1])


def pca_colsum(x, out=None):
    rows, D = _pca_matrix(x)
    if out is None:
        out = torch.empty(D, dtype=torch.float64, device=x.device)
    assert out.dtype == torch.float64 and out.is_contiguous() and out.numel() == D and out.device == x.device
    check(lib.mts_pca_colsum(stream_ptr(), dtype_code(x.dtype), rows, D, ptr(x), ptr(out)))
    return out


def pca_gram(x, center, out=None):
    rows, D = _pca_matrix(x)
    if out is None:
        out = torch.empty((D, D), dtype=torch.float64, device=x.device)
    assert center.dtype == torch.float32 and center.is_contiguous() and center.numel() == D
    assert out.dtype == torch.float64 and out.is_contiguous() and out.numel() == D * D and out.device == x.device == center.device
    check(lib.mts_pca_gram(stream_ptr(), dtype_code(x.dtype), rows, D, ptr(x), ptr(center), ptr(out)))
    return out


def pca_project(x, center, w, y=None):
    rows, D = _pca_matrix(x)
    assert w.dim() == 2 and w.dtype == torch.float32 and w.is_contiguous() and int(w.shape[1]) == D
    k = int(w.shape[0])
    if y is None:
        y = torch.empty((rows, k), dtype=x.dtype, device=x.device)
    assert center.dtype == torch.float32 and center.is_contiguous() and center.numel() == D
    assert y.is_contiguous() and y.numel() == rows * k and y.device == x.device == center.device == w.device
    check(lib.mts_pca_project(stream_ptr(), dtype_code(x.dtype), dtype_code(y.dtype), rows, D, k, ptr(x), ptr(center), ptr(w), ptr(y)))
    return y


def _frame_args(frames, frame_start, out, width):
    assert frames.dim() == 2 and frames.is_contiguous() and frames.is_cuda, 'a contiguous [total_frames, D] device matrix is expected'
    assert frame_start.dtype == torch.int64 and frame_start.dim() == 1 and frame_start.is_contiguous() and frame_start.numel() >= 2
    n_sent, D = frame_start.numel() - 1, int(frames.shape[1])
    assert out.dim() == 2 and tuple(out.shape) == (n_sent, width * D) and (out.stride(1) == 1 or out.shape[1] == 1)
    ld_out = int(out.stride(0)) if n_sent > 1 else max(int(out.stride(0)), width * D)
    assert ld_out >= width * D
    assert frames.device == frame_start.device == out.device
    return n_sent, D, ld_out


def frame_pool(frames, frame_start, out, first='mean', with_std=False):
    code = {None: L.POOL_NONE, 'mean': L.POOL_MEAN, 'max': L.POOL_MAX}[first]
    n_sent, D, ld_out = _frame_args(frames, frame_start, out, (first is not None) + bool(with_std))
    check(lib.mts_frame_pool(stream_ptr(), dtype_code(frames.dtype), dtype_code(out.dtype), n_sent, D, code, int(bool(with_std)), ptr(frames),
                             int(frames.shape[0]), ptr(frame_start), ptr(out), ld_out))
    return out


def frame_edges(frames, frame_start, doc_last, out, mode='last'):
    code = {'last': L.EDGE_LAST, 'delta_gap': L.EDGE_DELTA_GAP}[mode]
    n_sent, D, ld_out = _frame_args(frames, frame_start, out, 1)
    assert doc_last is not None or mode == 'last'
    if doc_last is not None:
        assert doc_last.dtype == torch.uint8 and doc_last.is_contiguous() and doc_last.numel() == n_sent and doc_last.device == out.device
    check(lib.mts_frame_edges(stream_ptr(), dtype_code(frames.dtype), dtype_code(out.dtype), n_sent, D, code, ptr(frames), int(frames.shape[0]),
                              ptr(frame_start), ptr(doc_last), ptr(out), ld_out))
    return out


def embed_layernorm_fwd(x, pos, pos_offset, type0, gamma, beta, eps, y, pre, mean, rstd, row_src=None, x2=None):
    B, Lq, D = x.shape
    if x.dtype == torch.bfloat16:
        assert x2 is None and y.dtype == torch.bfloat16
        check(lib.mts_embed_layernorm_fwd_x16(stream_ptr(), B, Lq, D, ptr(x), ptr(pos), pos_offset, ptr(type0), ptr(gamma), ptr(beta), eps, ptr(y),
                                              ptr(pre), ptr(mean), ptr(rstd), ptr(row_src), row_src.numel() if row_src is not None else 0))
        return
    if x2 is not None:
        check(lib.mts_embed_layernorm_fwd2(stream_ptr(), dtype_code(y.dtype), B, Lq, D, x2.shape[2], ptr(x), ptr(x2), ptr(pos), pos_offset,
                                           ptr(type0), ptr(gamma), ptr(beta), eps, ptr(y), ptr(pre), ptr(mean), ptr(rstd), ptr(row_src),
                                           row_src.numel() if row_src is not None else 0))
        return
    check(lib.mts_embed_layernorm_fwd(stream_ptr(), dtype_code(y.dtype), B, Lq, D, ptr(x), ptr(pos), pos_offset, ptr(type0),
                                      ptr(gamma), ptr(beta), eps, ptr(y), ptr(pre), ptr(mean), ptr(rstd), ptr(row_src),
                                      row_src.numel() if row_src is not None else 0))


def layernorm_fwd(x, gamma, beta, eps, y, mean, rstd, head_w=None, head_b=None, scores=None):
    rows, D = x.shape
    n_out = head_w.shape[0] if head_w is not None else 0
    check(lib.mts_layernorm_fwd(stream_ptr(), dtype_code(x.dtype), rows, D, ptr(x), ptr(gamma), ptr(beta), eps, ptr(y),
                                ptr(mean), ptr(rstd), ptr(head_w), ptr(head_b), n_out, ptr(scores)))


def layernorm_bwd(x, dy, gamma, mean, rstd, dx, dgamma, dbeta, dxsum=None, dlogit=None, head_w=None, beta=None, dhead_w=None, dhead_b=None):
    rows, D = x.shape
    ws = _scratch(lib.mts_layernorm_bwd_workspace(D), x.device, 'ln_bwd')
    n_out = head_w.shape[0] if head_w is not None else 0
    check(lib.mts_layernorm_bwd(stream_ptr(), dtype_code(x.dtype), rows, D, ptr(x), ptr(dy), ptr(dlogit), ptr(head_w), n_out,
                                ptr(gamma), ptr(mean), ptr(rstd), ptr(dx), ptr(dgamma), ptr(dbeta), ptr(dxsum), ptr(ws),
                                ptr(beta), ptr(dhead_w), ptr(dhead_b)))


def loss_tail_supported(dtype, D, n_out):
    return dtype in (torch.float32, torch.bfloat16) and bool(lib.mts_layernorm_loss_tail_supported(dtype_code(dtype), D, n_out))


def layernorm_loss_tail(kind, x, gamma, beta, eps, head_w, head_b, targets, lengths, alpha, gamma_f, grad_scale, scores, loss_out, dx, dgamma,
                        dbeta, dxsum, dhead_w, dhead_b, batch_shape, row_src=None):
    rows, D = x.shape
    B, Lq = batch_shape
    ws = _scratch(lib.mts_layernorm_bwd_workspace(D), x.device, 'ln_bwd')
    with _timed(('ln_tail', rows, D, head_w.shape[0])):
        check(lib.mts_layernorm_loss_tail(stream_ptr(), dtype_code(x.dtype), rows, D, ptr(x), ptr(gamma), ptr(beta), eps, ptr(head_w), ptr(head_b),
                                          head_w.shape[0], kind, B, Lq, targets.shape[1], ptr(targets), ptr(lengths), float(alpha), float(gamma_f),
                                          float(grad_scale), ptr(row_src), row_src.numel() if row_src is not None else 0, ptr(scores),
                                          ptr(loss_out), ptr(dx), ptr(dgamma), ptr(dbeta), ptr(dxsum), ptr(dhead_w), ptr(dhead_b), ptr(ws)))


def embed_layernorm_bwd(pre, dh, gamma, mean, rstd, B, Lq, dgamma, dbeta, dtype0, dpos, pos_offset, row0=None, lengths=None):
    rows, D = pre.shape
    nb = lib.mts_embed_layernorm_bwd_workspace(B, Lq, D)
    ws = _scratch(nb, pre.device, 'emb_bwd')
    check(lib.mts_embed_layernorm_bwd(stream_ptr(), dtype_code(pre.dtype), B, Lq, D, ptr(pre), ptr(dh), ptr(gamma), ptr(mean), ptr(rstd),
                                      ptr(dgamma), ptr(dbeta), ptr(dtype0), ptr(dpos), pos_offset, ptr(row0),
                                      ptr(lengths) if row0 is not None else None, rows if row0 is not None else 0, ptr(ws), nb))


def embed_bwd(dpre, B, Lq, dpos, pos_offset, row0=None, lengths=None):
    D = dpre.shape[-1]
    check(lib.mts_embed_bwd(stream_ptr(), dtype_code(dpre.dtype), B, Lq, D, ptr(dpre), ptr(dpos), pos_offset, ptr(row0),
                            ptr(lengths) if row0 is not None else None))


def dropout_fwd(x, y, p, seed, mask=None, residual=None):
    check(lib.mts_dropout_fwd(stream_ptr(), dtype_code(x.dtype), x.numel(), ptr(x), ptr(residual), ptr(y), ptr(mask), float(p), int(seed)))


def dropout_bwd(dy, dx, mask, p):
    check(lib.mts_dropout_bwd(stream_ptr(), dtype_code(dy.dtype), dy.numel(), ptr(dy), ptr(dx), ptr(mask), float(p)))


def gelu_bwd(u, dy):
    check(lib.mts_gelu_bwd(stream_ptr(), dtype_code(u.dtype), u.numel(), ptr(u), ptr(dy)))


def relu_bwd(u, dy):
    check(lib.mts_relu_bwd(stream_ptr(), dtype_code(u.dtype), u.numel(), ptr(u), ptr(dy)))


def ffn_supported(dtype, M, D, F):
    return bool(lib.mts_ffn_supported(dtype_code(dtype), M, D, F)) if dtype in (torch.float32, torch.bfloat16) else False


def ffn_fwd(a1, w1, b1, w2, b2, u, f, s2, relu=False):
    M, D = a1.shape
    with _timed(('ffn_fwd', M, D, w1.shape[0])):
        check(lib.mts_ffn_fwd(stream_ptr(), M, D, w1.shape[0], ptr(a1), ptr(w1), ptr(b1), ptr(w2), ptr(b2), int(relu), ptr(u), ptr(f), ptr(s2)))


def ffn_bwd_data(ds2, w1, w2, u, du, da1, relu=False):
    M, D = ds2.shape
    with _timed(('ffn_bwd', M, D, w1.shape[0])):
        check(lib.mts_ffn_bwd_data(stream_ptr(), M, D, w1.shape[0], ptr(ds2), ptr(w1), ptr(w2), ptr(u), int(relu), ptr(du), ptr(da1)))


def band_slots(radius):
    return lib.mts_band_slots(radius)


def band_attn_fwd(qkv, lengths, B, Lq, D, heads, radius, ctx, probs, row0=None, drop_p=0.0, drop_seed=0):
    with _timed(('band_fwd', B, Lq, D, heads, radius)):
        check(lib.mts_band_attn_fwd(stream_ptr(), dtype_code(qkv.dtype), B, Lq, D, heads, radius, ptr(qkv), ptr(lengths), ptr(ctx), ptr(probs),
                                    ptr(row0), float(drop_p), int(drop_seed)))


def band_attn_bwd(qkv, lengths, probs, dctx, B, Lq, D, heads, radius, dqkv, dscores, dbias=None, row0=None, drop_p=0.0, drop_seed=0):
    q_scale = 1.0 / math.sqrt(D // heads)
    ws = _scratch(lib.mts_band_attn_bwd_workspace(B, Lq, D), qkv.device, 'band_bwd') if dbias is not None else None
    with _timed(('band_bwd', B, Lq, D, heads, radius)):
        check(lib.mts_band_attn_bwd(stream_ptr(), dtype_code(qkv.dtype), B, Lq, D, heads, radius, q_scale, ptr(qkv), ptr(lengths),
                                    ptr(probs), ptr(dctx), ptr(dqkv), ptr(dscores), ptr(dbias), ptr(ws), ptr(row0),
                                    qkv.shape[0] if row0 is not None else 0, float(drop_p), int(drop_seed)))


def full_attn_fwd(qkv, lengths, B, Lq, D, heads, ctx, lse, row0=None, drop_p=0.0, drop_seed=0):
    with _timed(('full_fwd', B, Lq, D, heads)):
        check(lib.mts_full_attn_fwd(stream_ptr(), dtype_code(qkv.dtype), B, Lq, D, heads, ptr(qkv), ptr(lengths), ptr(ctx), ptr(lse),
                                    ptr(row0), float(drop_p), int(drop_seed)))


def full_attn_bwd(qkv, lengths, lse, ctx, dctx, B, Lq, D, heads, dqkv, dbias=None, row0=None, drop_p=0.0, drop_seed=0):
    q_scale = 1.0 / math.sqrt(D // heads)
    ws = _scratch(lib.mts_full_attn_bwd_workspace(B, Lq, D, heads), qkv.device, 'full_bwd')
    with _timed(('full_bwd', B, Lq, D, heads)):
        check(lib.mts_full_attn_bwd(stream_ptr(), dtype_code(qkv.dtype), B, Lq, D, heads, q_scale, ptr(qkv), ptr(lengths), ptr(lse),
                                    ptr(ctx), ptr(dctx), ptr(dqkv), ptr(dbias), ptr(ws), ptr(row0),
                                    qkv.shape[0] if row0 is not None else 0, float(drop_p), int(drop_seed)))


def t5_local_attn_fwd(qkv, lengths, B, Lq, heads, radius, table, bucket_of_offset, ctx, lse, drop_p=0.0, drop_seed=0):
    with _timed(('t5_fwd', B, Lq, heads, radius)):
        check(lib.mts_t5_local_attn_fwd(stream_ptr(), dtype_code(qkv.dtype), B, Lq, heads, 64, radius, ptr(qkv), ptr(lengths), ptr(table),
                                        table.shape[0], ptr(bucket_of_offset), ptr(ctx), ptr(lse), float(drop_p), int(drop_seed)))


def t5_local_attn_bwd(qkv, lengths, B, Lq, heads, radius, table, bucket_of_offset, lse, ctx, dctx, dqkv, dtable, drop_p=0.0, drop_seed=0):
    ws = _scratch(lib.mts_t5_local_attn_bwd_workspace(B, Lq, heads, radius), qkv.device, 't5_bwd')
    with _timed(('t5_bwd', B, Lq, heads, radius)):
        check(lib.mts_t5_local_attn_bwd(stream_ptr(), dtype_code(qkv.dtype), B, Lq, heads, 64, radius, ptr(qkv), ptr(lengths), ptr(table),
                                        table.shape[0], ptr(bucket_of_offset), ptr(lse), ptr(ctx), ptr(dctx), ptr(dqkv), ptr(dtable),
                                        ptr(ws), float(drop_p), int(drop_seed)))


def rmsnorm_fwd(x, w, eps, y, rstd):
    rows, D = x.shape
    check(lib.mts_rmsnorm_fwd(stream_ptr(), dtype_code(x.dtype), rows, D, ptr(x), ptr(w), float(eps), ptr(y), ptr(rstd)))

# ... 56 lines not shown
    if len(segments) < B:
        raise IndexError('list index out of range')
    n = np.clip(np.asarray(lens, dtype=np.int64), 0, L)
    docs = []
    for b in range(B):
        d = segments[b]
        arr = np.asarray(d.tolist() if hasattr(d, 'tolist') else d)
        if arr.size and (arr.ndim != 1 or arr.dtype.kind not in 'iu' or any(isinstance(v, bool) for v in d)):
            raise ValueError(f'segments[{b}] must be a flat list of integers; got {list(d)!r}')
        docs.append(arr.astype(np.int64).reshape(-1))
    counts = np.array([a.size for a in docs], dtype=np.int64)
    K = int(counts.sum())
    ends = np.concatenate(docs) if K else np.zeros(0, dtype=np.int64)
    doc = np.repeat(np.arange(B, dtype=np.int64), counts)
    first = np.zeros(K, dtype=bool)
    first[(np.cumsum(counts) - counts)[counts > 0]] = True
    begins = np.where(first, 0, np.concatenate(([0], ends[:-1]))) if K else ends
    bad = ~((begins < ends) & (ends <= n[doc]))
    if bad.any():
        b = int(doc[np.flatnonzero(bad)[0]])
        raise ValueError(f'segments[{b}] = {docs[b].tolist()} must be strictly ascending with 0 < s <= {int(n[b])} (the length of document {b})')
    has = counts > 0
    rank = np.cumsum(has) - has
    S = K + int(has.sum())
    seg = np.zeros((S, 8), dtype=np.int32)
    seg[:, 4:7] = -1
    at = np.arange(K, dtype=np.int64) + rank[doc]
    seg[at, 0], seg[at, 1], seg[at, 2] = doc, begins, ends
    hd = np.flatnonzero(has)
    tail = np.cumsum(counts)[hd] + rank[hd]
    seg[tail, 0], seg[tail, 1], seg[tail, 2], seg[tail, 3] = hd, ends[np.cumsum(counts)[hd] - 1] if K else 0, n[hd], 1
    pos = at[(ends - begins) > 1]
    npos = pos.size
    pair = np.zeros((npos + K, 4), dtype=np.int32)
    pair[:npos, 0], pair[:npos, 1], pair[:npos, 2] = pos, pos, 1
    pair[npos:, 0], pair[npos:, 1], pair[npos:, 2] = at, at + 1, -1
    seg[pos, 4] = np.arange(npos)
    seg[at, 5] = seg[at + 1, 6] = npos + np.arange(K)
    row_map = np.full(B * L, -1, dtype=np.int32)
    n_rows = (seg[:, 2] - seg[:, 1]).astype(np.int64)
    if n_rows.sum():
        sid = np.repeat(np.arange(S, dtype=np.int64), n_rows)
        k = np.arange(int(n_rows.sum()), dtype=np.int64) - np.repeat(np.cumsum(n_rows) - n_rows, n_rows)
        row_map[np.repeat(seg[:, 0].astype(np.int64) * L + seg[:, 1], n_rows) + k] = (2 * sid + (k & 1)).astype(np.int32)
    return SegmentTable(seg, pair, row_map, B, L)


class _DeviceSegmentTable:
    def __init__(self, tab, device):
        import numpy as np
        self.n_seg, self.n_pair, self.B, self.L = tab.n_seg, tab.n_pair, tab.B, tab.L
        flat = torch.from_numpy(np.concatenate([tab.seg.ravel(), tab.pair.ravel(), tab.row_map])).to(device)
        a, b = tab.seg.size, tab.seg.size + tab.pair.size
        self.seg, self.pair, self.row_map = flat[:a], flat[a:b], flat[b:]


def segment_tables(segments, lengths, B, L, device):
    return _DeviceSegmentTable(segment_table(segments, lengths, B, L), device)


def segment_cosine_fwd(x, tab, loss_out, pair_cos=None):
    W = x.shape[1]
    assert x.shape[0] == tab.B * tab.L and x.stride(1) == 1
    ws = _scratch(lib.mts_segment_cosine_workspace(tab.n_seg, tab.n_pair, W), x.device, 'segcos')
    with _timed(('segcos_fwd', tab.B, tab.L, W)):
        check(lib.mts_segment_cosine_fwd(stream_ptr(), dtype_code(x.dtype), tab.B, tab.L, W, ptr(x), x.stride(0), tab.n_seg, ptr(tab.seg),
                                         tab.n_pair, ptr(tab.pair), ptr(loss_out), ptr(pair_cos), ptr(ws)))
    return ws


def segment_cosine_bwd(tab, scale, dx, ws, accumulate=True):
    W = dx.shape[1]
    assert dx.shape[0] == tab.B * tab.L and dx.stride(1) == 1
    with _timed(('segcos_bwd', tab.B, tab.L, W)):
        check(lib.mts_segment_cosine_bwd(stream_ptr(), dtype_code(dx.dtype), tab.B, tab.L, W, tab.n_seg, ptr(tab.seg), tab.n_pair, ptr(tab.pair),
                                         ptr(tab.row_map), float(scale), int(accumulate), ptr(dx), dx.stride(0), ptr(ws)))


def tagger_loss(kind, scores, targets, lengths, alpha, gamma, loss_out, dscores, row_src=None, batch_shape=None):
    if row_src is None:
        B, Lq, n_out = scores.shape
    else:
        (B, Lq), n_out = batch_shape, scores.shape[-1]
    nb = lib.mts_tagger_loss_workspace(B, Lq)
    ws = _scratch(nb, scores.device, 'loss')
    check(lib.mts_tagger_loss(stream_ptr(), kind, B, Lq, targets.shape[1], n_out, ptr(scores), ptr(targets), ptr(lengths),
                              float(alpha), float(gamma), ptr(loss_out), ptr(dscores), ptr(ws), nb, ptr(row_src),
                              row_src.numel() if row_src is not None else 0))


def greedy_decode(scores, lengths, threshold, tags_out):
    B, Lq, n_out = scores.shape
    check(lib.mts_greedy_decode(stream_ptr(), B, Lq, n_out, ptr(scores), ptr(lengths), float(threshold), ptr(tags_out)))


def segment_decode(scores, lengths, threshold, seg_end, n_seg, min_segment=1, close_last=True, tags=None, prob=None):
    assert scores.dim() == 3 and scores.dtype == torch.float32 and scores.is_contiguous()
    B, Lq, n_out = scores.shape
    assert lengths is None or (lengths.dtype == torch.int32 and lengths.numel() == B and lengths.is_contiguous() and lengths.device == scores.device)
    assert seg_end.dtype == torch.int32 and seg_end.dim() == 2 and seg_end.shape[0] == B and seg_end.is_contiguous()
    assert n_seg.dtype == torch.int32 and n_seg.numel() == B and n_seg.is_contiguous()
    assert tags is None or (tags.dtype == torch.uint8 and tags.numel() == B * Lq and tags.is_contiguous() and tags.device == scores.device)
    assert prob is None or (prob.dtype == torch.float32 and prob.numel() == B * Lq and prob.is_contiguous() and prob.device == scores.device)
    assert scores.device == seg_end.device == n_seg.device
    check(lib.mts_segment_decode(stream_ptr(), B, Lq, n_out, ptr(scores), ptr(lengths), float(threshold), int(min_segment),
                                 int(bool(close_last)), int(seg_end.shape[1]), ptr(tags), ptr(prob), ptr(seg_end), ptr(n_seg)))
    return seg_end, n_seg


def _sweep_operands(scores, targets, lengths, thresholds, counts_out, width):
    B, Lq, n_out = scores.shape
    T = thresholds.numel()
    assert scores.dtype == torch.float32 and targets.dtype == torch.float32 and thresholds.dtype == torch.float32
    assert scores.is_contiguous() and targets.is_contiguous() and thresholds.is_contiguous() and targets.shape[0] == B
    assert lengths is None or (lengths.dtype == torch.int32 and lengths.numel() == B and lengths.is_contiguous())
    assert counts_out.dtype == torch.int32 and counts_out.is_contiguous() and counts_out.numel() == B * T * width
    return B, Lq, n_out, T


def threshold_sweep(scores, targets, lengths, thresholds, counts_out, end_boundary=False):
    B, Lq, n_out, T = _sweep_operands(scores, targets, lengths, thresholds, counts_out, 6)
    check(lib.mts_threshold_sweep(stream_ptr(), B, Lq, targets.shape[1], n_out, ptr(scores), ptr(targets), ptr(lengths), T, ptr(thresholds),
                                  int(bool(end_boundary)), ptr(counts_out)))


def winpr_sweep(scores, targets, lengths, thresholds, counts_out, end_boundary=False, k=10):
    B, Lq, n_out, T = _sweep_operands(scores, targets, lengths, thresholds, counts_out, 3)
    check(lib.mts_winpr_sweep(stream_ptr(), B, Lq, targets.shape[1], n_out, ptr(scores), ptr(targets), ptr(lengths), T, ptr(thresholds),
                              int(bool(end_boundary)), int(k), ptr(counts_out)))


def bootstrap_sums(values, samples, seed=0, out=None):
    if values.dim() == 1:
        values = values.view(1, -1)
    assert values.dim() == 2 and values.dtype == torch.float64 and values.is_contiguous() and values.device.type == 'cuda'
    M, n = values.shape
    S = int(samples)
    if out is None:
        out = torch.empty(M, max(S, 0), dtype=torch.float64, device=values.device)
    assert out.dtype == torch.float64 and out.is_contiguous() and out.numel() == M * max(S, 0) and out.device == values.device
    check(lib.mts_bootstrap_sums(stream_ptr(), n, M, S, ptr(values), int(seed) & 0xFFFFFFFFFFFFFFFF, ptr(out)))
    return out


def head_fwd(x, w, b, scores):
    rows, D = x.shape
    check(lib.mts_head_fwd(stream_ptr(), dtype_code(x.dtype), rows, D, w.shape[0], ptr(x), x.stride(0), ptr(w), ptr(b), ptr(scores)))


def head_bwd_params(x, dscores, dw, db):
    rows, D = x.shape
    ws = _scratch(lib.mts_layernorm_bwd_workspace(D), x.device, 'ln_bwd')
    check(lib.mts_head_bwd_params(stream_ptr(), dtype_code(x.dtype), rows, D, dw.shape[0], ptr(x), x.stride(0), ptr(dscores),
                                  ptr(dw), ptr(db), ptr(ws)))


def head_bwd_data(dscores, w, dx, accumulate=False):
    rows, D = dx.shape
    check(lib.mts_head_bwd_data(stream_ptr(), dtype_code(dx.dtype), rows, D, w.shape[0], ptr(dscores), ptr(w), ptr(dx),
                                dx.stride(0), int(accumulate)))


def switch_doc_maps(domains, B=None):
    if isinstance(domains, torch.Tensor):
        domains = domains.tolist()
    if isinstance(domains, (str, bytes)) or not hasattr(domains, '__len__') or not hasattr(domains, '__iter__'):
        raise ValueError(f'domains must be a sequence of 0 / 1 / bool, one per document; got {type(domains).__name__}')
    doms = list(domains)
    if B is not None and len(doms) != B:
        raise ValueError(f'domains has {len(doms)} entries for a batch of {B} documents')
    for d in doms:
        if isinstance(d, bool) or (hasattr(d, '__index__') and not isinstance(d, float) and int(d) in (0, 1)):
            continue
        raise ValueError(f'domains entries must be 0, 1 or a bool; got {d!r}')
    n = len(doms)
    src, head, tgt = [0] * n, [0] * n, [-1] * (2 * n)
    rank = [0, 0]
    for i, d in enumerate(doms):
        k = 0 if d else 1
        src[i], head[i] = rank[k], k
        tgt[k * n + rank[k]] = i
        rank[k] += 1
    return src, head, tgt


_SWITCH_MAPS_CACHE = {}


def switch_maps(domains, B, device):
    if isinstance(domains, torch.Tensor):
        domains = domains.tolist()
    try:
        key = (tuple((type(d), d) for d in domains), int(B), str(torch.device(device)))
        hit = _SWITCH_MAPS_CACHE.get(key)
    except TypeError:
        key = hit = None
    if hit is None:
        src, head, tgt = switch_doc_maps(domains, B)
        up = torch.tensor([src, head, tgt[:B], tgt[B:]], dtype=torch.int32).reshape(4, B).to(device)
        hit = (up[0], up[1], up[2:].reshape(-1))
        if key is not None:
            if len(_SWITCH_MAPS_CACHE) > 64:
                _SWITCH_MAPS_CACHE.clear()
            _SWITCH_MAPS_CACHE[key] = hit
    return hit


def _switch_check(who, act, B, Lq, w):
    rows, D = act.shape
    if rows != B * Lq:
        raise ValueError(f'{who}: {rows} rows for a batch of {B} x {Lq}')
    if D % 4 or act.stride(0) % 4 or act.stride(1) != 1:
        raise ValueError(f'{who}: D = {D} and the row stride {act.stride(0)} must be multiples of 4 (4-element vectors), columns contiguous')
    if act.data_ptr() % (4 * act.element_size()):
        raise ValueError(f'{who}: the {act.dtype} operand must be aligned to a 4-element vector ({4 * act.element_size()} bytes)')
    if w.dim() != 3 or w.shape[0] != 2 or not 1 <= w.shape[1] <= 4 or w.shape[2] != D or not w.is_contiguous() or w.dtype != torch.float32:
        raise ValueError(f'{who}: head weights must be contiguous fp32 [2, n_out <= 4, {D}], got {tuple(w.shape)}')


def switch_head_fwd(x, w, b, domains, B, Lq, scores):
    _switch_check('switch_head_fwd', x, B, Lq, w)
    src, head, _ = switch_maps(domains, B, x.device)
    check(lib.mts_switch_head_fwd(stream_ptr(), dtype_code(x.dtype), B, Lq, x.shape[1], w.shape[1], ptr(x), x.stride(0), ptr(w), ptr(b),
                                  ptr(src), ptr(head), ptr(scores)))


def switch_head_bwd_params(x, dscores, domains, B, Lq, dw, db):
    _switch_check('switch_head_bwd_params', x, B, Lq, dw)
    src, head, _ = switch_maps(domains, B, x.device)
    ws = _scratch(lib.mts_switch_head_bwd_workspace(x.shape[1]), x.device, 'switch_bwd')
    check(lib.mts_switch_head_bwd_params(stream_ptr(), dtype_code(x.dtype), B, Lq, x.shape[1], dw.shape[1], ptr(x), x.stride(0), ptr(dscores),
                                         ptr(src), ptr(head), ptr(dw), ptr(db), ptr(ws)))


def switch_head_bwd_data(dscores, w, domains, B, Lq, dx):
    _switch_check('switch_head_bwd_data', dx, B, Lq, w)
    _, _, tgt = switch_maps(domains, B, dx.device)
    check(lib.mts_switch_head_bwd_data(stream_ptr(), dtype_code(dx.dtype), B, Lq, dx.shape[1], w.shape[1], ptr(dscores), ptr(w), ptr(tgt),
                                       ptr(dx), dx.stride(0)))


def lstm_workspace(dtype, B, Lq, H, ndir, device, tag='lstm'):
    return _scratch(lib.mts_lstm_workspace(dtype_code(dtype), B, Lq, H, ndir), device, tag)


def lstm_fwd(xproj, w_hh, b_hh, lengths, B, Lq, H, ndir, out, gates, cells):
    ws = lstm_workspace(xproj.dtype, B, Lq, H, ndir, xproj.device)
    check(lib.mts_lstm_fwd(stream_ptr(), dtype_code(xproj.dtype), B, Lq, H, ndir, ptr(xproj), ptr(w_hh), ptr(b_hh), ptr(lengths), ptr(out),
                           ptr(gates), ptr(cells), ptr(ws)))


def lstm_bwd(w_hh, lengths, out, gates, cells, dout, B, Lq, H, ndir, dxproj, dw_hh, ws=None):
    if ws is None:
        ws = lstm_workspace(out.dtype, B, Lq, H, ndir, out.device)
    check(lib.mts_lstm_bwd(stream_ptr(), dtype_code(out.dtype), B, Lq, H, ndir, ptr(w_hh), ptr(lengths), ptr(out), ptr(gates),
                           ptr(cells), ptr(dout), ptr(dxproj), ptr(dw_hh), ptr(ws)))


def crf_nll(feats, tags, lengths, trans, loss_out, dfeats=None, dtrans=None):
    B, Lq, C = feats.shape
    ws = _scratch(lib.mts_crf_workspace(B, Lq, C), feats.device, 'crf')
    check(lib.mts_crf_nll(stream_ptr(), B, Lq, C, ptr(feats), ptr(tags), tags.shape[1], ptr(lengths), ptr(trans), ptr(loss_out),
                          ptr(dfeats), ptr(dtrans), ptr(ws)))


def crf_viterbi(feats, lengths, trans, best_score, paths):
    B, Lq, C = feats.shape
    ws = _scratch(B * Lq * C * 4, feats.device, 'crf_bp')
    check(lib.mts_crf_viterbi(stream_ptr(), B, Lq, C, ptr(feats), ptr(lengths), ptr(trans), ptr(best_score), ptr(paths), ptr(ws)))


def crf_marginals(feats, lengths, trans, scores, cls=1, logz=None):
    B, Lq, C = feats.shape
    ws = _scratch(lib.mts_crf_workspace(B, Lq, C), feats.device, 'crf')
    check(lib.mts_crf_marginals(stream_ptr(), B, Lq, C, int(cls), ptr(feats), ptr(lengths), ptr(trans), ptr(scores), ptr(logz), ptr(ws)))


def crf_nll_packed(feats, tags, lengths, trans, loss_out, shape, row0=None, dfeats=None, dtrans=None):
    (B, Lq), (n_rows, C) = shape, feats.shape
    ws = _scratch(lib.mts_crf_workspace(B, Lq, C), feats.device, 'crf')
    check(lib.mts_crf_nll_packed(stream_ptr(), B, Lq, C, ptr(feats), ptr(tags), tags.shape[1], ptr(lengths), ptr(trans), ptr(loss_out),
                                 ptr(dfeats), ptr(dtrans), ptr(ws), ptr(row0), n_rows))


def crf_viterbi_packed(feats, lengths, trans, best_score, paths, row0=None):
    (B, Lq), (n_rows, C) = paths.shape, feats.shape
    ws = _scratch(max(n_rows, 1) * C * 4, feats.device, 'crf_bp')
    check(lib.mts_crf_viterbi_packed(stream_ptr(), B, Lq, C, ptr(feats), ptr(lengths), ptr(trans), ptr(best_score), ptr(paths), ptr(ws),
                                     ptr(row0), n_rows))


def crf_marginals_packed(feats, lengths, trans, scores, shape, row0=None, cls=1, logz=None):
    (B, Lq), (n_rows, C) = shape, feats.shape
    ws = _scratch(lib.mts_crf_workspace(B, Lq, C), feats.device, 'crf')
    check(lib.mts_crf_marginals_packed(stream_ptr(), B, Lq, C, int(cls), ptr(feats), ptr(lengths), ptr(trans), ptr(scores), ptr(logz), ptr(ws),
                                       ptr(row0), n_rows))


def adam_step(param, grad, exp_avg, exp_avg_sq, lr, beta1, beta2, eps, step, grad_scale=1.0, bf16_copy=None):
    check(lib.mts_adam_step(stream_ptr(), param.numel(), ptr(param), ptr(grad), ptr(exp_avg), ptr(exp_avg_sq), lr, beta1, beta2,
                            eps, step, grad_scale, ptr(bf16_copy)))


def sgd_step(param, grad, buf, lr, momentum, weight_decay, first_step, grad_scale=1.0, bf16_copy=None):
    check(lib.mts_sgd_step(stream_ptr(), param.numel(), ptr(param), ptr(grad), ptr(buf), lr, momentum, weight_decay,
                           int(first_step), grad_scale, ptr(bf16_copy)))


def grad_norm_workspace(device):
    return torch.empty(lib.mts_grad_norm_workspace() // 4, dtype=torch.float32, device=device)


def grad_norm(grad, spans, grad_scale, workspace, out):
    assert grad.dtype == torch.float32 and grad.is_contiguous() and out.dtype == torch.float32 and workspace.dtype == torch.float32
    assert workspace.numel() * 4 >= lib.mts_grad_norm_workspace()
    if not any(b > a for a, b in spans):
        out.zero_()
        return out
    begin = (ctypes.c_size_t * len(spans))(*[a for a, _ in spans])
    end = (ctypes.c_size_t * len(spans))(*[b for _, b in spans])
    check(lib.mts_grad_norm(stream_ptr(), ptr(grad), len(spans), begin, end, grad_scale, ptr(workspace), ptr(out)))
    return out


def adam_step_clipped(param, grad, exp_avg, exp_avg_sq, lr, beta1, beta2, eps, step, grad_scale=1.0, bf16_copy=None, total_norm=None,
                      max_norm=0.0, clip_value=0.0, clip_coef_out=None):
    check(lib.mts_adam_step_clipped(stream_ptr(), param.numel(), ptr(param), ptr(grad), ptr(exp_avg), ptr(exp_avg_sq), lr, beta1, beta2,
                                    eps, step, grad_scale, ptr(bf16_copy), ptr(total_norm), max_norm, clip_value, ptr(clip_coef_out)))


def sgd_step_clipped(param, grad, buf, lr, momentum, weight_decay, first_step, grad_scale=1.0, bf16_copy=None, total_norm=None,
                     max_norm=0.0, clip_value=0.0, clip_coef_out=None):
    check(lib.mts_sgd_step_clipped(stream_ptr(), param.numel(), ptr(param), ptr(grad), ptr(buf), lr, momentum, weight_decay,
                                   int(first_step), grad_scale, ptr(bf16_copy), ptr(total_norm), max_norm, clip_value, ptr(clip_coef_out)))


def scale_(x, scale):
    if scale != 1.0:
        assert x.dtype == torch.float32 and x.is_contiguous()
        check(lib.mts_scale(stream_ptr(), x.numel(), ptr(x), float(scale)))
    return x


def lstm_bwd_recurrence(w_hh, lengths, out, gates, cells, dout, B, Lq, H, ndir, dxproj, ws):
    check(lib.mts_lstm_bwd_recurrence(stream_ptr(), dtype_code(out.dtype), B, Lq, H, ndir, ptr(w_hh), ptr(lengths), ptr(out), ptr(gates),
                                      ptr(cells), ptr(dout), ptr(dxproj), ptr(ws)))


def lstm_bwd_whh(lengths, out, dxproj, B, Lq, H, ndir, dw_hh, ws):
    check(lib.mts_lstm_bwd_whh(stream_ptr(), dtype_code(out.dtype), B, Lq, H, ndir, ptr(lengths), ptr(out), ptr(dxproj), ptr(dw_hh), ptr(ws)))
```

multimodaltopicsegmentation_amd/taggers.py:

```python
import functools
import math
import os
from collections import OrderedDict

import torch
import torch.nn as nn

from . import _lib as L
from . import ops
from .flat import FlatLayout, FlatModule, round_up

LOSS_KINDS = {'CrossEntropy': L.LOSS_CE, 'BinaryCrossEntropy': L.LOSS_BCE, 'FocalLoss': L.LOSS_FOCAL}
DEAD_HF_KEYS = ('word_embeddings', 'query_global', 'key_global', 'value_global', 'pooler', 'position_ids', 'token_type_ids')


def default_compute_dtype():
    v = os.environ.get('MTS_COMPUTE_DTYPE', 'fp32').lower()
    return torch.bfloat16 if v in ('bf16', 'bfloat16') else torch.float32


def _as_dtype(d):
    if d is None:
        return default_compute_dtype()
    if isinstance(d, str):
        return torch.bfloat16 if d.lower() in ('bf16', 'bfloat16') else torch.float32
    return d


def _xavier_uniform(shape, gen):
    bound = math.sqrt(6.0 / (shape[0] + shape[1]))
    return (torch.rand(shape, generator=gen) * 2 - 1) * bound


def _linear_init(out_f, in_f, gen):
    k = 1.0 / math.sqrt(in_f)
    return (torch.rand(out_f, in_f, generator=gen) * 2 - 1) * k, (torch.rand(out_f, generator=gen) * 2 - 1) * k


_LENGTHS_CACHE = {}


class _Workspace:

    def __init__(self):
        self.bufs = {}
        self.generation = 0

    def get(self, name, rows, cols, dtype, device):
        key = name
        t = self.bufs.get(key)
        need = rows * cols
        if t is None or t.numel() < need or t.dtype != dtype or t.device != device:
            t = torch.empty(max(need, 1), dtype=dtype, device=device)
            self.bufs[key] = t
            self.generation += 1
        return t[:need].view(rows, cols)


def _on_model_device(fn):
    @functools.wraps(fn)
    def guarded(self, *args, **kwargs):
        dev = self._flat.device
        if dev.type != 'cuda' or torch.cuda.current_device() == dev.index:
            return fn(self, *args, **kwargs)
        with torch.cuda.device(dev):
            return fn(self, *args, **kwargs)
    guarded._mts_device_guard = True
    return guarded


class _TaggerBase(FlatModule):

    _GUARDED_ENTRY_POINTS = ('loss_and_grad', 'loss', 'encode', 'forward')

    def __init_subclass__(cls, **kw):
        super().__init_subclass__(**kw)
        for name in cls._GUARDED_ENTRY_POINTS:
            fn = cls.__dict__.get(name)
            if fn is not None and not getattr(fn, '_mts_device_guard', False):
                setattr(cls, name, _on_model_device(fn))


    def _init_common(self, loss_fn, threshold, alpha, gamma, compute_dtype):
        if loss_fn not in LOSS_KINDS:
            raise ValueError('Choose one of CrossEntropy or BinaryCrossEntropy as loss function')
        self.loss_kind = LOSS_KINDS[loss_fn]
        self.bce = loss_fn != 'CrossEntropy'
        self.fl = loss_fn == 'FocalLoss'
        self.alpha, self.gamma = float(alpha), float(gamma)
        self.th = threshold
        self.compute_dtype = _as_dtype(compute_dtype)
        self._ws = _Workspace()
        self._wcopy = None
        self._wcopy_version = None
        self.device = 'cuda' if torch.cuda.is_available() else 'cpu'

    def _on_reflatten(self):
        self._wcopy = None
        self._wcopy_version = None

    def _weights_version(self):
        return (self._flat._version, sum(p._version for p in self._flat_params.values()))

    def _weights(self):
        if self.compute_dtype == torch.float32:
            return self._flat
        ver = self._weights_version()
        if self._wcopy is None or self._wcopy.device != self._flat.device:
            self._wcopy = torch.empty(self._flat.numel(), dtype=torch.bfloat16, device=self._flat.device)
            self._wcopy_version = None
        if self._wcopy_version != ver:
            ops.cast(self._flat, self._wcopy)
            self._wcopy_version = ver
        return self._wcopy

    crf_head = False
    loss_grad_scale = 1.0
    _grad_hook = None
    grad_hooks_cover_all = False

    def _grads_ready(self, a, b):
        if self._grad_hook is not None and b > a:
            self._grad_hook(a, b)

    def mark_weights_synced(self):
        self._wcopy_version = self._weights_version()

    def _w(self, wflat, name):
        return self._layout.view(wflat, name)

    def _wspan(self, wflat, first, last, rows, cols):
        off, n = self._layout.span(first, last)
        return wflat[off:off + n].view(rows, cols)

    @staticmethod
    def _split_input(xs):
        if isinstance(xs, (tuple, list)):
            x1, x2 = xs
            if x1.shape[:2] != x2.shape[:2]:
                raise ValueError(f'K-split input parts disagree: {tuple(x1.shape)} vs {tuple(x2.shape)}')
            if x1.shape[2] % 4 or x2.shape[2] % 4:
                raise ValueError('K-split input parts must have widths that are multiples of 4')
            return x1, x2, x1.shape[0], x1.shape[1], x1.shape[2] + x2.shape[2]
        return xs, None, xs.shape[0], xs.shape[1], xs.shape[2]

    @staticmethod
    def _prep_lengths(lengths, B, L, device):
        if lengths is None:
            return torch.full((B,), L, dtype=torch.int32, device=device)
        if lengths.device.type == 'cpu' and lengths.numel() <= 4096:
            key = (tuple(lengths.tolist()), str(device))
            hit = _LENGTHS_CACHE.get(key)
            if hit is None:
                if len(_LENGTHS_CACHE) > 64:
                    _LENGTHS_CACHE.clear()
                hit = _LENGTHS_CACHE[key] = lengths.to(device=device, dtype=torch.int32).contiguous()
            return hit
        return lengths.to(device=device, dtype=torch.int32).contiguous()

    def _decode(self, scores, lengths_i32, lengths, threshold):
        if self.th is not None:
            threshold = self.th
        B, Lq, _ = scores.shape
        tags = torch.empty(B, Lq, dtype=torch.uint8, device=scores.device)
        ops.greedy_decode(scores, lengths_i32, threshold, tags)
        tags_h = tags.cpu().numpy().astype(bool)
        L.check_async()
        lens = [int(v) for v in (lengths.tolist() if lengths is not None else [Lq] * B)]
        return [tags_h[i, :lens[i]].tolist() for i in range(B)]

    ffn_act = 'gelu'
    qkv_release = os.environ.get('MTS_DP_QKV_RELEASE', 'block')
    fuse_ffn = os.environ.get('MTS_FUSE_FFN', '1') != '0'
    fuse_tail = os.environ.get('MTS_FUSE_TAIL', '1') != '0'
    fuse_ffn_min_rows = 12288

    def _lt(self, flat, names, key, rows, cols):
        first, last = names[key]
        return self._wspan(flat, first, last, rows, cols)

    def _band_layer_fwd(self, names, tag, h, lengths_i32, B, Lq, N, radius, row0, pdrop, pattn, head=None, store_out=True, skip_ln2=False):
        dt, dev = self.compute_dtype, h.device
        D, F, H = self.embedding_dim, self._ffp, self.nheads
        ws = self._ws
        wf, pf = self._weights(), self._flat
        slots = ops.band_slots(radius) if radius is not None else 0
        qkv = ws.get(f'qkv{tag}', N, 3 * D, dt, dev)
        ops.linear_fwd(h, self._lt(wf, names, 'wqkv', 3 * D, D), self._lt(pf, names, 'bqkv', 1, 3 * D).view(-1), qkv,
                       colscale=1.0 / math.sqrt(D // H), ncols_scaled=D)
        ctx = ws.get(f'ctx{tag}', N, D, dt, dev)
        aseed = self._drop_seed() if pattn else 0
        if radius is None:
            probs = ws.get(f'lse{tag}', N, H, torch.float32, dev)
            ops.full_attn_fwd(qkv, lengths_i32, B, Lq, D, H, ctx, probs, row0=row0, drop_p=pattn, drop_seed=aseed)
        else:
            probs = ws.get(f'probs{tag}', N, H * slots, torch.float32, dev)
            ops.band_attn_fwd(qkv, lengths_i32, B, Lq, D, H, radius, ctx, probs, row0=row0, drop_p=pattn, drop_seed=aseed)
        s1 = ws.get(f's1_{tag}', N, D, dt, dev)
        m1 = m2 = None
        wo, bo = self._lt(wf, names, 'wo', D, D), self._lt(pf, names, 'bo', 1, D).view(-1)
        if pdrop:
            tmp = ws.get('droptmp', N, D, dt, dev)
            m1 = ws.get(f'dropmask1_{tag}', N, D, torch.uint8, dev)
            ops.linear_fwd(ctx, wo, bo, tmp)
            ops.dropout_fwd(tmp, s1, pdrop, self._drop_seed(), mask=m1, residual=h)
        else:
            ops.linear_fwd(ctx, wo, bo, s1, residual=h)
        a1 = ws.get(f'a1_{tag}', N, D, dt, dev)
        mean1 = ws.get(f'mean1_{tag}', N, 1, torch.float32, dev)
        rstd1 = ws.get(f'rstd1_{tag}', N, 1, torch.float32, dev)
        ops.layernorm_fwd(s1, self._lt(pf, names, 'ln1w', 1, D).view(-1), self._lt(pf, names, 'ln1b', 1, D).view(-1), self.ln_eps,
                          a1, mean1, rstd1)
        Np = round_up(N, 64)
        u = ws.get(f'u{tag}', Np, F, dt, dev)[:N]
        f = ws.get(f'f{tag}', Np, F, dt, dev)[:N]
        relu = self.ffn_act == 'relu'
        s2 = ws.get(f's2_{tag}', Np, D, dt, dev)[:N]
        w2, b2 = self._lt(wf, names, 'w2', D, F), self._lt(pf, names, 'b2', 1, D).view(-1)
        fused = self.fuse_ffn and not pdrop and N >= self.fuse_ffn_min_rows and ops.ffn_supported(dt, N, D, F)
        w1, b1 = self._lt(wf, names, 'w1', F, D), self._lt(pf, names, 'b1', 1, F).view(-1)
        if fused:
            ops.ffn_fwd(a1, w1, b1, w2, b2, u, f, s2, relu=relu)
        else:
            ops.linear_fwd(a1, w1, b1, f, gelu=not relu, relu=relu, aux=u)
        if fused:
            pass
        elif pdrop:
            tmp = ws.get('droptmp', N, D, dt, dev)
            m2 = ws.get(f'dropmask2_{tag}', N, D, torch.uint8, dev)
            ops.linear_fwd(f, w2, b2, tmp)
            ops.dropout_fwd(tmp, s2, pdrop, self._drop_seed(), mask=m2, residual=a1)
        else:
            ops.linear_fwd(f, w2, b2, s2, residual=a1)
        if skip_ln2:
            hout = mean2 = rstd2 = None
        else:
            hout = ws.get(f'hout{tag}', N, D, dt, dev) if (store_out or head is None) else None
            mean2 = ws.get(f'mean2_{tag}', N, 1, torch.float32, dev)
            rstd2 = ws.get(f'rstd2_{tag}', N, 1, torch.float32, dev)
            ops.layernorm_fwd(s2, self._lt(pf, names, 'ln2w', 1, D).view(-1), self._lt(pf, names, 'ln2b', 1, D).view(-1), self.ln_eps,
                              hout, mean2, rstd2, head_w=head[0] if head else None, head_b=head[1] if head else None,
                              scores=head[2] if head else None)
        return dict(hin=h, qkv=qkv, ctx=ctx, probs=probs, s1=s1, a1=a1, mean1=mean1, rstd1=rstd1, u=u, f=f, s2=s2, hout=hout,
                    mean2=mean2, rstd2=rstd2, radius=radius, slots=slots, m1=m1, m2=m2, pattn=pattn, aseed=aseed, fused_ffn=fused)

    pair_ffn_wgrads = os.environ.get('MTS_PAIR_FFN_WGRADS', '1') == '1'

    def _band_layer_bwd(self, names, S, dh, lengths_i32, B, Lq, N, pdrop, row0, wgrad, tail_end, head=None, slot=0, head_grads=None, tail_done=False,
                        wgrad_direct=True):
        dt = self.compute_dtype
        D, F, H = self.embedding_dim, self._ffp, self.nheads
        ws, lay = self._ws, self._layout
        dev = S['s2'].device
        wf, pf = self._weights(), self._flat
        g = self.grad_flat()
        Gv = lambda key, rows, cols: self._lt(g, names, key, rows, cols)
        ds2 = ws.get('ds2', N, D, dt, dev)
        if not tail_done:
            ops.layernorm_bwd(S['s2'], dh, self._lt(pf, names, 'ln2w', 1, D).view(-1), S['mean2'], S['rstd2'], ds2,
                              Gv('ln2w', 1, D).view(-1), Gv('ln2b', 1, D).view(-1), dxsum=Gv('b2', 1, D).view(-1),
                              dlogit=head[0] if head else None, head_w=head[1] if head else None,
                              beta=self._lt(pf, names, 'ln2b', 1, D).view(-1) if head_grads else None,
                              dhead_w=head_grads[0] if head_grads else None, dhead_b=head_grads[1] if head_grads else None)
        ds2d = ds2
        if pdrop:
            ds2d = ws.get('ds2d', N, D, dt, dev)
            ops.dropout_bwd(ds2, ds2d, S['m2'], pdrop)
            ops.colsum(ds2d, Gv('b2', 1, D).view(-1))
        Np = round_up(N, 64)
        du = ws.get('du', Np, F, dt, dev)[:N]
        da1 = ws.get('da1', Np, D, dt, dev)[:N]
        if S.get('fused_ffn') and not pdrop:
            ops.ffn_bwd_data(ds2, self._lt(wf, names, 'w1', F, D), self._lt(wf, names, 'w2', D, F), S['u'], du, da1, relu=self.ffn_act == 'relu')
            if self.pair_ffn_wgrads and wgrad_direct and ops.wgrad_pair_supported(du, S['a1']):
                ops.colsum(du, Gv('b1', 1, F).view(-1))
                ops.wgrad_pair(du, S['a1'], Gv('w1', F, D), S['f'], ds2, Gv('w2', D, F))
            else:
                wgrad(ds2, S['f'], Gv('w2', D, F))
                ops.colsum(du, Gv('b1', 1, F).view(-1))
                wgrad(du, S['a1'], Gv('w1', F, D))
        else:
            wgrad(ds2d, S['f'], Gv('w2', D, F))
            ops.linear_dgrad(ds2d, self._lt(wf, names, 'w2', D, F), du)
            if self.ffn_act == 'relu':
                ops.relu_bwd(S['u'], du)
            else:
                ops.gelu_bwd(S['u'], du)
            ops.colsum(du, Gv('b1', 1, F).view(-1))
            wgrad(du, S['a1'], Gv('w1', F, D))
            ops.linear_dgrad(du, self._lt(wf, names, 'w1', F, D), da1, residual=ds2)
        ds1 = ws.get('ds1', N, D, dt, dev)
        ops.layernorm_bwd(S['s1'], da1, self._lt(pf, names, 'ln1w', 1, D).view(-1), S['mean1'], S['rstd1'], ds1,
                          Gv('ln1w', 1, D).view(-1), Gv('ln1b', 1, D).view(-1), dxsum=Gv('bo', 1, D).view(-1))
        ds1d = ds1
        if pdrop:
            ds1d = ws.get('ds1d', N, D, dt, dev)
            ops.dropout_bwd(ds1, ds1d, S['m1'], pdrop)
            ops.colsum(ds1d, Gv('bo', 1, D).view(-1))
        wgrad(ds1d, S['ctx'], Gv('wo', D, D))
        o_wo = lay.entries[names['wo'][0]][0]
        self._grads_ready(o_wo, tail_end)
        dctx = ws.get('dctx', N, D, dt, dev)
        ops.linear_dgrad(ds1d, self._lt(wf, names, 'wo', D, D), dctx)
        dqkv = ws.get('dqkv', N, 3 * D, dt, dev)
        if S['radius'] is None:
            ops.full_attn_bwd(S['qkv'], lengths_i32, S['probs'], S['ctx'], dctx, B, Lq, D, H, dqkv,
                              dbias=Gv('bqkv', 1, 3 * D).view(-1), row0=row0, drop_p=S['pattn'], drop_seed=S['aseed'])
        else:
            dsc = ws.get('dsc', N, H * S['slots'], torch.float32, dev)
            ops.band_attn_bwd(S['qkv'], lengths_i32, S['probs'], dctx, B, Lq, D, H, S['radius'], dqkv, dsc,
                              dbias=Gv('bqkv', 1, 3 * D).view(-1), row0=row0, drop_p=S['pattn'], drop_seed=S['aseed'])
        o_qkv = lay.entries[names['wqkv'][0]][0]
        if self._grad_hook is not None and self.qkv_release == 'projection':
            gq = Gv('wqkv', 3 * D, D)
            for i in range(3):
                wgrad(dqkv[:, i * D:(i + 1) * D], S['hin'], gq[i * D:(i + 1) * D])
                self._grads_ready(o_qkv + i * D * D, o_qkv + (i + 1) * D * D if i < 2 else o_wo)
        else:
            wgrad(dqkv, S['hin'], Gv('wqkv', 3 * D, D))
            self._grads_ready(o_qkv, o_wo)
        dhin = ws.get(f'dhin{slot}', N, D, dt, dev)
        ops.linear_dgrad(dqkv, self._lt(wf, names, 'wqkv', 3 * D, D), dhin, residual=ds1)
        return dhin

    def _autograd_loss(self, run_fwd_bwd):
        params = list(self._flat_params.values())
        return _NativeLoss.apply(self, run_fwd_bwd, *params)


class _NativeLoss(torch.autograd.Function):

    @staticmethod
    def forward(ctx, model, run, *params):
        loss = run()
        ctx.model = model
        ctx.unused = frozenset(getattr(model, '_unused_params', ()) or ())
        return loss.clone()

    @staticmethod
    def backward(ctx, gout):
        views = ctx.model.grad_views()
        grads = [None if name in ctx.unused else (v * gout).clone() for name, v in views.items()]
        return (None, None, *grads)


def decodes_by_viterbi(model):
    return bool(getattr(model, 'crf_head', False)) and getattr(model, 'decode', 'viterbi') == 'viterbi'


class _TransformerEncoderTagger(_TaggerBase):
    _HEAD_W, _HEAD_B = 'classification.weight', 'classification.bias'

    def _head_groups(self, gen, add):
        raise NotImplementedError

    def _init_encoder(self, tagset_size, embedding_dim, hidden_dim, num_layers, nheads, dropout_in, dropout_out, restricted, window_size,
                      max_position_embedding, seed, n_out):
        self.restricted = bool(restricted)
        if not 0.0 <= float(dropout_in) < 1.0:
            raise ValueError(f'dropout probability has to be between 0 and 1, but got {dropout_in}')
        if not 0.0 <= float(dropout_out) < 1.0:
            raise ValueError(f'dropout probability has to be between 0 and 1, but got {dropout_out}')
        self.dropout_in, self.dropout_out = float(dropout_in), float(dropout_out)
        self._attn_drop = self.dropout_out if self.restricted else 0.1
        self._pos_offset = 2 if self.restricted else 0
        self._drop_calls = 0
        self.embedding_dim, self.hidden_dim, self.tagset_size = embedding_dim, hidden_dim, tagset_size
        self.nheads, self.num_layers = nheads, num_layers
        if self.restricted:
            windows = [k * window_size for k in range(num_layers, 0, -1)]
            assert all(w % 2 == 0 for w in windows), 'All window sizes must be divisible by 2!'
            self.radii = [w // 2 for w in windows]
        else:
            self.radii = [None] * num_layers
        if embedding_dim % nheads != 0:
            raise ValueError(f'The hidden size ({embedding_dim}) is not a multiple of the number of attention heads ({nheads})')
        self.n_out = n_out
        self.ln_eps = 1e-12
        self.max_pos = max_position_embedding
        D, F = embedding_dim, hidden_dim

        gen = torch.Generator().manual_seed(torch.initial_seed() if seed is None else seed)
        std = 0.02
        groups, init, pads = [], {}, {}
        Fp = self._ffp = round_up(F, 8)

        def add(group, name, shape, value, pad=None, storage=None):
            group.append((name, storage or shape))
            init[name] = value
            if pad and storage != shape:
                pads[name] = pad

        e = 'model.model.embeddings.'
        g = []
        pos = torch.randn(self.max_pos, D, generator=gen) * std
        if self.restricted:
            pos[1].zero_()
        add(g, e + 'position_embeddings.weight', (self.max_pos, D), pos)
        gpos = g
        g = []
        add(g, e + 'token_type_embeddings.weight', (2, D), torch.randn(2, D, generator=gen) * std)
        add(g, e + 'LayerNorm.weight', (D,), torch.ones(D))
        add(g, e + 'LayerNorm.bias', (D,), torch.zeros(D))
        groups.append(g)
        groups.append(gpos)
        for li in range(num_layers):
            lp = f'model.model.encoder.layer.{li}.'
            g = []
            for n in ('query', 'key', 'value'):
                add(g, lp + f'attention.self.{n}.weight', (D, D), torch.randn(D, D, generator=gen) * std)
            groups.append(g)
            g = []
            for n in ('query', 'key', 'value'):
                add(g, lp + f'attention.self.{n}.bias', (D,), torch.zeros(D))
            groups.append(g)
            for name, shape, val in (
                    ('attention.output.dense.weight', (D, D), torch.randn(D, D, generator=gen) * std),
                    ('attention.output.dense.bias', (D,), torch.zeros(D)),
                    ('attention.output.LayerNorm.weight', (D,), torch.ones(D)),
                    ('attention.output.LayerNorm.bias', (D,), torch.zeros(D)),
                    ('intermediate.dense.weight', (F, D), torch.randn(F, D, generator=gen) * std),
                    ('intermediate.dense.bias', (F,), torch.zeros(F)),
                    ('output.dense.weight', (D, F), torch.randn(D, F, generator=gen) * std),
                    ('output.dense.bias', (D,), torch.zeros(D)),
                    ('output.LayerNorm.weight', (D,), torch.ones(D)),
                    ('output.LayerNorm.bias', (D,), torch.zeros(D))):
                g = []
                if name == 'intermediate.dense.weight':
                    add(g, lp + name, shape, val, pad=[(0, 1, F, Fp)], storage=(Fp, D))
                elif name == 'intermediate.dense.bias':
                    add(g, lp + name, shape, val, pad=[(0, 1, F, Fp)], storage=(Fp,))
                elif name == 'output.dense.weight':
                    add(g, lp + name, shape, val, pad=[(1, 1, F, Fp)], storage=(D, Fp))
                else:
                    add(g, lp + name, shape, val)
                groups.append(g)
        groups += self._head_groups(gen, add)
        self._init_flat(FlatLayout(groups, pads), init)
        self._register_load_state_dict_pre_hook(self._drop_dead_keys)

    @staticmethod
    def _drop_dead_keys(state_dict, prefix, *args):
        for k in [k for k in state_dict if k.startswith(prefix) and any(d in k for d in DEAD_HF_KEYS)]:
            del state_dict[k]

    def _layer_names(self, li):
        lp = f'model.model.encoder.layer.{li}.'
        a_, o_ = lp + 'attention.self.', lp + 'attention.output.'
        one = lambda n: (n, n)
        return {'wqkv': (a_ + 'query.weight', a_ + 'value.weight'), 'bqkv': (a_ + 'query.bias', a_ + 'value.bias'),
                'wo': one(o_ + 'dense.weight'), 'bo': one(o_ + 'dense.bias'), 'ln1w': one(o_ + 'LayerNorm.weight'),
                'ln1b': one(o_ + 'LayerNorm.bias'), 'w1': one(lp + 'intermediate.dense.weight'), 'b1': one(lp + 'intermediate.dense.bias'),
                'w2': one(lp + 'output.dense.weight'), 'b2': one(lp + 'output.dense.bias'), 'ln2w': one(lp + 'output.LayerNorm.weight'),
                'ln2b': one(lp + 'output.LayerNorm.bias')}

    def _forward_native(self, xs, lengths_i32, want_grad_state=True, pack=None, need_hidden=True, tail=False):
        xs, xs2, B, Lq, D = self._split_input(xs)
        dt, dev = self.compute_dtype, xs.device
        if D != self.embedding_dim:
            raise ValueError(f'expected input dim {self.embedding_dim}, got {D}')
        if Lq + self._pos_offset > self.max_pos:
            if not self.restricted:
                raise ValueError(f'sequence length {Lq} exceeds max_position_embeddings = {self.max_pos}')
            raise ValueError(f'sequence length {Lq} exceeds max_position_embeddings-2 = {self.max_pos - 2}')
        N, F, H = (pack['n'] if pack else B * Lq), self._ffp, self.nheads
        row_src, row0 = (pack['row_src'], pack['row0']) if pack else (None, None)
        ws, lay = self._ws, self._layout
        wf = self._weights()
        pf = self._flat
        keep16 = xs.dtype == torch.bfloat16 and dt == torch.bfloat16 and xs2 is None and D % 4 == 0
        x = xs.contiguous() if keep16 else xs.contiguous().to(torch.float32)
        x2 = xs2.contiguous().to(torch.float32) if xs2 is not None else None
        e = 'model.model.embeddings.'
        st = {'B': B, 'L': Lq, 'N': N, 'lengths': lengths_i32, 'layers': [], 'pack': pack}
        h = ws.get('h0', N, D, dt, dev)
        pre0 = ws.get('pre0', N, D, dt, dev)
        mean0 = ws.get('mean0', N, 1, torch.float32, dev)
        rstd0 = ws.get('rstd0', N, 1, torch.float32, dev)
        ops.embed_layernorm_fwd(x, lay.view(pf, e + 'position_embeddings.weight'), self._pos_offset,
                                lay.view(pf, e + 'token_type_embeddings.weight')[0], lay.view(pf, e + 'LayerNorm.weight'),
                                lay.view(pf, e + 'LayerNorm.bias'), self.ln_eps, h, pre0, mean0, rstd0, row_src=row_src, x2=x2)
        st.update(pre0=pre0, mean0=mean0, rstd0=rstd0)
        pdrop = self.dropout_in if self.training else 0.0
        st['pdrop'] = pdrop
        if pdrop:
            st['m0'] = ws.get('dropmask0', N, D, torch.uint8, dev)
            ops.dropout_fwd(h, h, pdrop, self._drop_seed(), mask=st['m0'])
        scores = ws.get('scores', N, self.n_out, torch.float32, dev)
        for li, radius in enumerate(self.radii):
            last = li == len(self.radii) - 1
            head = (self._w(pf, self._HEAD_W), self._w(pf, self._HEAD_B), scores) if (last and not tail) else None
            S = self._band_layer_fwd(self._layer_names(li), str(li), h, lengths_i32, B, Lq, N, radius, row0, pdrop,
                                     self._attn_drop if self.training else 0.0, head,
                                     store_out=need_hidden or not last or self.n_out > 2, skip_ln2=last and tail)
            st['layers'].append(S)
            h = S['hout']
        st['scores'] = scores if pack else scores.view(B, Lq, self.n_out)
        st['hidden'] = h
        return st

    def _backward_native(self, st, dscores, tail_done=False):
        dt = self.compute_dtype
        B, Lq, N = st['B'], st['L'], st['N']
        D, F, H = self.embedding_dim, self._ffp, self.nheads
        dev = self._flat.device
        ws, lay = self._ws, self._layout
        wf, pf = self._weights(), self._flat
        g = self.grad_flat()
        G = lambda name: lay.view(g, name)
        nl = len(self.radii)
        dh = None
        side = self._side_stream(dev) if (self.overlap_wgrad and self._grad_hook is None and dev.type == 'cuda') else None
        main = torch.cuda.current_stream(dev) if side is not None else None

        def wgrad(dy, x, gview):
            if side is None:
                ops.linear_wgrad(dy, x, gview)
                return
            ev = torch.cuda.Event()
            ev.record(main)
            side.wait_event(ev)
            with torch.cuda.stream(side):
                ops.linear_wgrad(dy, x, gview)

        for li in range(nl - 1, -1, -1):
            last = li == nl - 1
            if side is not None:
                main.wait_stream(side)
            fuse_hg = last and self.n_out <= 2 and not tail_done
            if last and not fuse_hg and not tail_done:
                ops.head_bwd_params(st['layers'][li]['hout'], dscores, G(self._HEAD_W), G(self._HEAD_B))
            tail_end = lay.entries[f'model.model.encoder.layer.{li + 1}.attention.self.query.weight'][0] if li + 1 < nl else g.numel()
            dh = self._band_layer_bwd(self._layer_names(li), st['layers'][li], dh, st['lengths'], B, Lq, N, st['pdrop'],
                                      st['pack']['row0'] if st['pack'] else None, wgrad, tail_end,
                                      head=(dscores, self._w(pf, self._HEAD_W)) if (last and not tail_done) else None, slot=li & 1,
                                      head_grads=(G(self._HEAD_W), G(self._HEAD_B)) if fuse_hg else None,
                                      tail_done=tail_done and last, wgrad_direct=side is None)
        e = 'model.model.embeddings.'
        if st['pdrop']:
            ops.dropout_bwd(dh, dh, st['m0'], st['pdrop'])
        pos_g, type_g = G(e + 'position_embeddings.weight'), G(e + 'token_type_embeddings.weight')
        if D <= 2048:
            off = self._pos_offset
            prev = getattr(self, '_pos_touched', 0)
            if prev > Lq + off:
                pos_g[Lq + off:prev].zero_()
            self._pos_touched = Lq + off
            ops.embed_layernorm_bwd(st['pre0'], dh, self._w(pf, e + 'LayerNorm.weight'), st['mean0'], st['rstd0'], B, Lq,
                                    G(e + 'LayerNorm.weight'), G(e + 'LayerNorm.bias'), type_g[0], pos_g, off,
                                    row0=st['pack']['row0'] if st['pack'] else None, lengths=st['lengths'])
        else:
            dpre = ws.get('ds2', N, D, dt, dev)
            type_g.zero_()
            ops.layernorm_bwd(st['pre0'], dh, self._w(pf, e + 'LayerNorm.weight'), st['mean0'], st['rstd0'], dpre,
                              G(e + 'LayerNorm.weight'), G(e + 'LayerNorm.bias'), dxsum=type_g[0])
            self._pos_touched = max(getattr(self, '_pos_touched', 0), Lq + self._pos_offset)
            pos_g[:self._pos_touched].zero_()
            ops.embed_bwd(dpre, B, Lq, pos_g, self._pos_offset, row0=st['pack']['row0'] if st['pack'] else None, lengths=st['lengths'])
        D_ = self.embedding_dim
        if side is not None:
            main.wait_stream(side)
        p0 = lay.entries[e + 'position_embeddings.weight'][0]
        t0 = lay.entries[e + 'token_type_embeddings.weight'][0]
        assert t0 < p0, 'flat layout: token-type rows and embedding LayerNorm in front of the position table'
        self._grads_ready(t0, p0 + (Lq + self._pos_offset) * D_)

    def _drop_seed(self):
        self._drop_calls += 1
        return (torch.initial_seed() * 1000003 + self._drop_calls * 7919) & 0x7FFFFFFFFFFFFFFF

    overlap_wgrad = os.environ.get('MTS_OVERLAP_WGRAD', '0') == '1'

    def _side_stream(self, dev):
        return ops.side_stream(dev, 0)

    pack_rows = 'auto'

    def _pack_plan(self, lengths, B, Lq, dev):
        if self.pack_rows is False or lengths is None:
            return None
        lens = [max(0, min(int(v), Lq)) for v in (lengths.tolist() if hasattr(lengths, 'tolist') else lengths)]
        n = sum(lens)
        if n == 0 or (self.pack_rows == 'auto' and n > 0.9 * B * Lq):
            return None
        key = (tuple(lens), Lq, str(dev))
        if getattr(self, '_pack_key', None) != key:
            import numpy as np
            row0 = np.zeros(B, dtype=np.int32)
            row0[1:] = np.cumsum(lens[:-1], dtype=np.int64)
            row_src = np.concatenate([b * Lq + np.arange(n_b, dtype=np.int32) for b, n_b in enumerate(lens)]).astype(np.int32)
            self._pack_val = {'row_src': torch.from_numpy(row_src).to(dev), 'row0': torch.from_numpy(row0).to(dev), 'n': n}
            self._pack_key = key
        return self._pack_val

    def encode(self, xs, lengths):
        x1, _, B, Lq, _ = self._split_input(xs)
        st = self._forward_native(xs, self._prep_lengths(lengths, B, Lq, x1.device))
        return st['hidden'].view(B, Lq, -1).to(torch.float32)


class Transformer_segmenter(_TransformerEncoderTagger):
    grad_hooks_cover_all = True

    def __init__(self, tagset_size, embedding_dim, hidden_dim, num_layers=6, nheads=8, dropout_in=0.0, dropout_out=0.0,
                 batch_first=True, loss_fn='CrossEntropy', positional_encoding=True, threshold=None, restricted=True,
                 window_size=127, alpha=0.9, gamma=2, compute_dtype=None, max_position_embedding=4096, seed=None):
        super().__init__()
        self._init_common(loss_fn, threshold, alpha, gamma, compute_dtype)
        self._init_encoder(tagset_size, embedding_dim, hidden_dim, num_layers, nheads, dropout_in, dropout_out, restricted, window_size,
                           max_position_embedding, seed, tagset_size if loss_fn == 'CrossEntropy' else 1)

    def _head_groups(self, gen, add):
        cw, cb = _linear_init(self.n_out, self.embedding_dim, gen)
        g = []
        add(g, 'classification.weight', (self.n_out, self.embedding_dim), cw)
        add(g, 'classification.bias', (self.n_out,), cb)
        return [g]

    def loss_and_grad(self, xs, lengths, tags, want_grad=True):
        L.require_gpu()
        x1, _, B, Lq, _ = self._split_input(xs)
        dev = x1.device
        li32 = self._prep_lengths(lengths, B, Lq, dev)
        pack = self._pack_plan(lengths, B, Lq, dev)
        tg = tags.to(device=dev, dtype=torch.float32).contiguous()
        loss_out = torch.empty(2, dtype=torch.float32, device=dev)
        D = self.embedding_dim
        if (want_grad and self.fuse_tail and self.n_out == (2 if self.loss_kind == L.LOSS_CE else 1) and tg.shape[1] >= Lq
                and ops.loss_tail_supported(self.compute_dtype, D, self.n_out)):
            st = self._forward_native(xs, li32, pack=pack, need_hidden=False, tail=True)
            nm, pf, g, lay = self._layer_names(len(self.radii) - 1), self._flat, self.grad_flat(), self._layout
            N = st['N']
            scores = self._ws.get('scores', N, self.n_out, torch.float32, dev)
            ds2 = self._ws.get('ds2', N, D, self.compute_dtype, dev)
            ops.layernorm_loss_tail(self.loss_kind, st['layers'][-1]['s2'], self._lt(pf, nm, 'ln2w', 1, D).view(-1), self._lt(pf, nm, 'ln2b', 1, D).view(-1),
                                    self.ln_eps, self._w(pf, 'classification.weight'), self._w(pf, 'classification.bias'), tg, li32, self.alpha,
                                    self.gamma, self.loss_grad_scale, scores, loss_out, ds2, self._lt(g, nm, 'ln2w', 1, D).view(-1),
                                    self._lt(g, nm, 'ln2b', 1, D).view(-1), self._lt(g, nm, 'b2', 1, D).view(-1), lay.view(g, 'classification.weight'),
                                    lay.view(g, 'classification.bias'), (B, Lq), row_src=pack['row_src'] if pack else None)
            st['scores'] = scores if pack else scores.view(B, Lq, self.n_out)
            self._backward_native(st, None, tail_done=True)
            return loss_out[0], st['scores']
        st = self._forward_native(xs, li32, pack=pack, need_hidden=False)
        dsc = self._ws.get('dscores', st['N'], self.n_out, torch.float32, dev) if want_grad else None
        ops.tagger_loss(self.loss_kind, st['scores'], tg, li32, self.alpha, self.gamma, loss_out, dsc,
                        row_src=pack['row_src'] if pack else None, batch_shape=(B, Lq))
        if want_grad:
            ops.scale_(dsc, self.loss_grad_scale)
            self._backward_native(st, dsc)
        return loss_out[0], st['scores']

    def loss(self, xs, lengths, tags):
        if torch.is_grad_enabled() and any(p.requires_grad for p in self._flat_params.values()):
            return self._autograd_loss(lambda: self.loss_and_grad(xs, lengths, tags, True)[0])
        return self.loss_and_grad(xs, lengths, tags, False)[0].clone()

    inference_graphs = False

    def _graph_entry(self, xs, li32, threshold):
        th = float(self.th if self.th is not None else threshold)
        key = (tuple(xs.shape), xs.dtype, th, self._ws.generation, self._flat.data_ptr())
        ent = self._graphs.get(key) if hasattr(self, '_graphs') else None
        if ent is not None:
            return ent
        if not hasattr(self, '_graphs'):
            self._graphs = {}
        if len(self._graphs) >= 16:
            return None
        B, Lq = xs.shape[0], xs.shape[1]
        dev = xs.device
        xs_s, li_s = torch.empty_like(xs), torch.empty_like(li32)
        tags = torch.empty(B, Lq, dtype=torch.uint8, device=dev)
        xs_s.copy_(xs)
        li_s.copy_(li32)

        def run():
            st = self._forward_native(xs_s, li_s, need_hidden=False)
            ops.greedy_decode(st['scores'], li_s, th, tags)
            return st['scores']
        self._weights()
        cur = torch.cuda.current_stream(dev)
        side = torch.cuda.Stream(dev)
        side.wait_stream(cur)
        with torch.cuda.stream(side):
            run()
        cur.wait_stream(side)
        key = (tuple(xs.shape), xs.dtype, th, self._ws.generation, self._flat.data_ptr())
        g = torch.cuda.CUDAGraph()
        with torch.cuda.graph(g):
            scores = run()
        ent = self._graphs[key] = (g, xs_s, li_s, scores, tags)
        return ent

    def forward(self, xs, lenghts, threshold=0.4):
        L.require_gpu()
        x1, x2, B, Lq, _ = self._split_input(xs)
        li32 = self._prep_lengths(lenghts, B, Lq, x1.device)
        with torch.no_grad():
            ent = None
            if self.inference_graphs and not self.training and x2 is None and torch.is_tensor(xs) and xs.dtype == torch.float32 and xs.is_contiguous():
                ent = self._graph_entry(xs, li32, threshold)
            if ent is not None:
                g, xs_s, li_s, scores_s, tags_s = ent
                self._weights()
                xs_s.copy_(xs)
                li_s.copy_(li32)
                g.replay()
                scores = scores_s.clone()
                tags_h = tags_s.cpu().numpy().astype(bool)
                L.check_async()
                lens = [int(v) for v in (lenghts.tolist() if lenghts is not None else [Lq] * B)]
                return scores, [tags_h[i, :lens[i]].tolist() for i in range(B)]
            st = self._forward_native(xs, li32, need_hidden=False)
            scores = st['scores'].clone()
            tags = self._decode(scores, li32, lenghts, threshold)
        return scores, tags


class _LegacyLayerFn(torch.autograd.Function):

    @staticmethod
    def forward(ctx, model, x, *params):
        y, st = model._run_forward(x)
        ctx.model, ctx.st, ctx.shape = model, st, tuple(x.shape)
        return y

    @staticmethod
    def backward(ctx, gy):
        m = ctx.model
        dx = m._run_backward(ctx.st, gy)
        grads = [v.clone() for v in m.grad_views().values()]
        return (None, dx.view(ctx.shape), *grads)


class RestrictedTransformerEncoderLayer(_TaggerBase):
    ffn_act = 'relu'

    def __init__(self, d_model, nhead, dim_feedforward=2048, window_size=None, dropout=0.1, activation='relu', layer_norm_eps=1e-5,
                 batch_first=False, norm_first=False, device=None, dtype=None, compute_dtype=None, seed=None):
        super().__init__()
        self._init_common('BinaryCrossEntropy', None, 0.9, 2, compute_dtype)
        if norm_first:
            raise NotImplementedError('norm_first=True (pre-LN variant, RestrictedTransformerLayer.py:291-296) is not built')
        if not batch_first:
            raise NotImplementedError('batch_first=False: every caller in the reference passes batch_first=True')
        act = getattr(activation, '__name__', activation)
        if act not in ('relu', 'gelu'):
            raise RuntimeError(f'activation should be relu/gelu, not {activation}')
        if window_size is None or int(window_size) < 0:
            raise ValueError('window_size (one-sided radius of the attention band) is required')
        if d_model % nhead != 0:
            raise AssertionError('embed_dim must be divisible by num_heads')
        if not 0.0 <= float(dropout) < 1.0:
            raise ValueError(f'dropout probability has to be between 0 and 1, but got {dropout}')
        self.ffn_act = act
        self.embedding_dim, self.nheads, self.hidden_dim = d_model, nhead, dim_feedforward
        self.radius = int(window_size)
        self.ln_eps = float(layer_norm_eps)
        self.dropout_p = float(dropout)
        self._drop_calls = 0
        D, F = d_model, dim_feedforward
        Fp = self._ffp = round_up(F, 8)
        gen = torch.Generator().manual_seed(torch.initial_seed() if seed is None else seed)
        w1, b1 = _linear_init(F, D, gen)
        w2, b2 = _linear_init(D, F, gen)
        wo, _ = _linear_init(D, D, gen)
        groups, init, pads = [], {}, {}
        for name, shape, val, pad, storage in (
                ('self_attn.in_proj_weight', (3 * D, D), _xavier_uniform((3 * D, D), gen), None, None),
                ('self_attn.in_proj_bias', (3 * D,), torch.zeros(3 * D), None, None),
                ('self_attn.out_proj.weight', (D, D), wo, None, None),
                ('self_attn.out_proj.bias', (D,), torch.zeros(D), None, None),
                ('norm1.weight', (D,), torch.ones(D), None, None), ('norm1.bias', (D,), torch.zeros(D), None, None),
                ('linear1.weight', (F, D), w1, [(0, 1, F, Fp)], (Fp, D)), ('linear1.bias', (F,), b1, [(0, 1, F, Fp)], (Fp,)),
                ('linear2.weight', (D, F), w2, [(1, 1, F, Fp)], (D, Fp)), ('linear2.bias', (D,), b2, None, None),
                ('norm2.weight', (D,), torch.ones(D), None, None), ('norm2.bias', (D,), torch.zeros(D), None, None)):
            groups.append([(name, storage or shape)])
            init[name] = val
            if pad and storage != shape:
                pads[name] = pad
        self._init_flat(FlatLayout(groups, pads), init)
        one = lambda n: (n, n)
        self._names = {'wqkv': one('self_attn.in_proj_weight'), 'bqkv': one('self_attn.in_proj_bias'),
                       'wo': one('self_attn.out_proj.weight'), 'bo': one('self_attn.out_proj.bias'), 'ln1w': one('norm1.weight'),
                       'ln1b': one('norm1.bias'), 'w1': one('linear1.weight'), 'b1': one('linear1.bias'), 'w2': one('linear2.weight'),
                       'b2': one('linear2.bias'), 'ln2w': one('norm2.weight'), 'ln2b': one('norm2.bias')}

    def _drop_seed(self):
        self._drop_calls += 1
        return (torch.initial_seed() * 1000003 + self._drop_calls * 7919) & 0x7FFFFFFFFFFFFFFF

    def _run_forward(self, src):
        B, Lq, D = src.shape
        if D != self.embedding_dim:
            raise ValueError(f'expected input dim {self.embedding_dim}, got {D}')
        dt, dev = self.compute_dtype, src.device
        N = B * Lq
        x = self._ws.get('x', N, D, dt, dev)
        x.copy_(src.reshape(N, D))
        pdrop = self.dropout_p if self.training else 0.0
        S = self._band_layer_fwd(self._names, 'L', x, None, B, Lq, N, self.radius, None, pdrop, pdrop)
        return S['hout'].view(B, Lq, D).to(torch.float32), dict(S=S, B=B, L=Lq, N=N, pdrop=pdrop)

    def _run_backward(self, st, gy):
        dt = self.compute_dtype
        N, D = st['N'], self.embedding_dim
        dh = self._ws.get('dy', N, D, dt, gy.device)
        dh.copy_(gy.reshape(N, D))
        wgrad = lambda dy, x, gview: ops.linear_wgrad(dy, x, gview)
        dx = self._band_layer_bwd(self._names, st['S'], dh, None, st['B'], st['L'], N, st['pdrop'], None, wgrad, self.grad_flat().numel())
        return dx.to(torch.float32)

    def forward(self, src, src_mask=None, src_key_padding_mask=None):
        L.require_gpu()
        if src_mask is not None or src_key_padding_mask is not None:
            raise NotImplementedError('src_mask / src_key_padding_mask: the reference drops the padding mask on this path (:467) and '
                                      'no caller passes an attention mask')
        if src.dim() != 3:
            raise ValueError('src must be [batch, sequence, d_model] (batch_first=True)')
        if torch.is_grad_enabled() and (src.requires_grad or any(p.requires_grad for p in self._flat_params.values())):
            return _LegacyLayerFn.apply(self, src, *self._flat_params.values())
        with torch.no_grad():
            return self._run_forward(src)[0]
```

multimodaltopicsegmentation_amd/trainer.py:

```python
import math
import os

import torch
import torch.distributed as dist

from . import ops


def shard_batch(batch, rank, world):
    if world == 1:
        return batch
    out = {}
    for k, v in batch.items():
        if isinstance(v, torch.Tensor) and v.dim() >= 1:
            out[k] = v[rank::world]
        elif isinstance(v, list):
            out[k] = v[rank::world]
        else:
            out[k] = v
    return out


def local_loss_count(model, batch):
    lengths = batch['src_lengths']
    Lq = batch['src_tokens'].shape[1]
    if hasattr(model, 'num_tags'):
        return int(lengths.numel())
    return int(lengths.clamp(max=Lq).sum())


class NativeTrainer:
    def __init__(self, model, lr=1e-3, optimizer='Adam', process_group=None, token_weighted=False, grad_exchange_dtype='fp32',
                 always_hook=False, exchange_schedule=None, gradient_clip_val=None, gradient_clip_algorithm='norm',
                 error_if_nonfinite=False, cosine_loss=False):
        self.model = model.model if hasattr(model, 'training_step') else model
        self.lr, self.kind = float(lr), optimizer
        self.pg = process_group
        self.world = dist.get_world_size(process_group) if (dist.is_available() and dist.is_initialized()) else 1
        self.step_count = 0
        self._m = self._v = None
        self._comm_stream = None
        self.token_weighted = bool(token_weighted)
        self.cosine_loss = bool(cosine_loss)
        if self.cosine_loss and not getattr(self.model, 'takes_segments', False):
            raise NotImplementedError(f'cosine_loss=True: {type(self.model).__name__}.loss_and_grad takes no segments (the cosine auxiliary '
                                      'loss is built for BiLSTM and BiLSTMLateFusion)')
        if self.cosine_loss and self.token_weighted:
            raise ValueError('cosine_loss=True cannot be combined with token_weighted=True: the cosine auxiliary loss averages over the '
                             "rank's segment pairs, which the per-sentence weighting does not cover")
        self.always_hook = bool(always_hook) and dist.is_available() and dist.is_initialized()
        if grad_exchange_dtype not in ('fp32', 'bf16'):
            raise ValueError("grad_exchange_dtype must be 'fp32' or 'bf16'")
        self.exchange_bf16 = grad_exchange_dtype == 'bf16'
        self._xbuf = None
        self.last_global_count = None
        sched = exchange_schedule if exchange_schedule is not None else os.environ.get('MTS_DP_SCHEDULE', 'allreduce')
        if sched not in ('allreduce', 'rs_ag'):
            raise ValueError("exchange_schedule must be 'allreduce' or 'rs_ag'")
        self.exchange_schedule = sched
        self._inflight_shards = []
        if gradient_clip_algorithm not in ('norm', 'value'):
            raise ValueError("gradient_clip_algorithm must be 'norm' or 'value'")
        clip = float(gradient_clip_val) if gradient_clip_val is not None else 0.0
        if not clip >= 0.0:
            raise ValueError('gradient_clip_val must be >= 0 (None or 0.0: no clipping)')
        self.gradient_clip_val = clip
        self.clip_mode = gradient_clip_algorithm if clip > 0.0 else None
        self.error_if_nonfinite = bool(error_if_nonfinite)
        self.last_grad_norm = self.last_clip_coef = None
        self._clip_stats = self._clip_ws = None

    def _state(self):
        flat = self.model.flat
        if self._m is None or self._m.device != flat.device:
            self._m = torch.zeros_like(flat)
            self._v = torch.zeros_like(flat)
        return self._m, self._v

    def _reduce_spans(self):
        m = self.model
        n = m.flat.numel()
        pos = 'model.model.embeddings.position_embeddings.weight'
        if pos in m._layout.entries and getattr(self, '_last_L', None) is not None:
            off, shape = m._layout.entries[pos]
            D = shape[1]
            end = off + shape[0] * D
            return [(0, off + (self._last_L + 2) * D), (end, n)]
        return [(0, n)]

    def _adam_spans(self):
        m = self.model
        n = m.flat.numel()
        pos = 'model.model.embeddings.position_embeddings.weight'
        if pos not in m._layout.entries or getattr(self, '_last_L', None) is None:
            return [(0, n)]
        off, shape = m._layout.entries[pos]
        D = shape[1]
        self._pos_rows = max(getattr(self, '_pos_rows', 0), min(self._last_L + 2, shape[0]))
        lo, hi = off + self._pos_rows * D, off + shape[0] * D
        return [(a, b) for a, b in ((0, lo), (hi, n)) if b > a]

    def exchange_weight(self, batch):
        if not self.token_weighted or self.world == 1:
            return 1.0
        n_local = local_loss_count(self.model, batch)
        dev = self.model.flat.device
        cnt = torch.tensor([float(n_local)], dtype=torch.float64, device=dev if dev.type == 'cuda' else 'cpu')
        dist.all_reduce(cnt, op=dist.ReduceOp.SUM, group=self.pg)
        total = float(cnt.item())
        self.last_global_count = total
        return self.world * n_local / total if total > 0 else 1.0

    def _sum_in_place(self, buf, async_op):
        world = self.world
        if self.exchange_schedule != 'rs_ag' or (world == 1 and not self.always_hook) or buf.numel() < world:
            h = dist.all_reduce(buf, op=dist.ReduceOp.SUM, group=self.pg, async_op=async_op)
            return [h] if async_op else []
        n = buf.numel()
        per = n // world
        body = per * world
        shard = torch.empty(per, dtype=buf.dtype, device=buf.device)
        hs = [dist.reduce_scatter_tensor(shard, buf[:body], op=dist.ReduceOp.SUM, group=self.pg, async_op=async_op)]
        if async_op and dist.get_backend(self.pg) != 'nccl':
            hs[0].wait()
        hs.append(dist.all_gather_into_tensor(buf[:body], shard, group=self.pg, async_op=async_op))
        if body < n:
            hs.append(dist.all_reduce(buf[body:], op=dist.ReduceOp.SUM, group=self.pg, async_op=async_op))
        if async_op and shard.device.type == 'cuda':
            self._inflight_shards.append(shard)
        return hs if async_op else []

    def _exchange(self, a, b, async_op):
        g = self.model.grad_flat()
        if not self.exchange_bf16:
            return self._sum_in_place(g[a:b], async_op), None
        if self._xbuf is None or self._xbuf.numel() < g.numel() or self._xbuf.device != g.device:
            self._xbuf = torch.empty(g.numel(), dtype=torch.bfloat16, device=g.device)
        buf = self._xbuf[a:b]
        buf.copy_(g[a:b])
        return self._sum_in_place(buf, async_op), (a, b)

    def _finish(self, handles, span):
        for handle in handles or ():
            handle.wait()
        if span is not None:
            a, b = span
            self.model.grad_flat()[a:b].copy_(self._xbuf[a:b])

    def allreduce_grads(self):
        if self.world == 1:
            return
        for a, b in self._reduce_spans():
            if b > a:
                _, span = self._exchange(a, b, False)
                self._finish(None, span)

    def _on_grads_ready(self, a, b):
        self._pending.append(self._exchange(a, b, True))

    def step(self, batch):
        dev = self.model.flat.device
        if dev.type == 'cuda' and torch.cuda.current_device() != dev.index:
            with torch.cuda.device(dev):
                return self._step(batch)
        return self._step(batch)

    def _step(self, batch):
        m = self.model
        x, lengths, tags = batch['src_tokens'], batch['src_lengths'], batch['tgt_tokens']
        if self.world > 1:
            self._check_same_length(x.shape[1])
        self._last_L = x.shape[1]
        m.loss_grad_scale = self.exchange_weight(batch)
        overlapped = (self.world > 1 or self.always_hook) and getattr(m, 'grad_hooks_cover_all', False)
        self._pending = []
        self._inflight_shards = []
        m._grad_hook = self._on_grads_ready if overlapped else None
        if self.cosine_loss:
            segments = batch['src_segments']
            if batch.get('src_tokens2') is not None and hasattr(m, '_rnn2'):
                loss, _ = m.loss_and_grad(x, batch['src_tokens2'], lengths, tags, True, segments=segments)
            else:
                loss, _ = m.loss_and_grad(x, lengths, tags, True, segments=segments)
        elif batch.get('src_tokens2') is not None and hasattr(m, '_rnn2'):
            loss, _ = m.loss_and_grad(x, batch['src_tokens2'], lengths, tags, True)
        elif getattr(m, 'takes_domains', False):
            loss, _ = m.loss_and_grad(x, lengths, tags, batch['domain'], True)
        else:
            loss, _ = m.loss_and_grad(x, lengths, tags, True)
        if overlapped:
            for h, span in self._pending:
                self._finish(h, span)
            self._pending = []
            self._inflight_shards = []
        else:
            self.allreduce_grads()
        self.apply_optimizer()
        return loss

    def fit(self, train, val=None, **kw):
        from .fit import fit
        return fit(self, train, val, **kw)

    def evaluate(self, corpus, **kw):
        from .evaluate import evaluate
        return evaluate(self, corpus, **kw)

    def predict(self, corpus, **kw):
        from .predict import predict
        return predict(self, corpus, **kw)

    def _check_same_length(self, Lq):
        seen = getattr(self, '_len_checked', None)
        if seen == Lq:
            return
        dev = self.model.flat.device
        t = torch.tensor([float(Lq), -float(Lq)], dtype=torch.float64, device=dev if dev.type == 'cuda' else 'cpu')
        dist.all_reduce(t, op=dist.ReduceOp.MAX, group=self.pg)
        if int(t[0].item()) != Lq or int(-t[1].item()) != Lq:
            raise ValueError(f'data-parallel ranks collated to different lengths (this rank {Lq}, max {int(t[0].item())}, '
                             f'min {int(-t[1].item())}): shard one collated batch with shard_batch() or pad to a common length')
        self._len_checked = Lq

    def _grad_norm(self, spans, gscale):
        g = self.model.grad_flat()
        if self._clip_stats is None or self._clip_stats.device != g.device:
            self._clip_stats = torch.zeros(2, dtype=torch.float32, device=g.device)
            self._clip_ws = ops.grad_norm_workspace(g.device)
            self.last_grad_norm, self.last_clip_coef = self._clip_stats[0], self._clip_stats[1]
        ops.grad_norm(g, spans, gscale, self._clip_ws, self.last_grad_norm)
        if self.error_if_nonfinite and not math.isfinite(float(self.last_grad_norm)):
            raise RuntimeError(f'the total norm of the gradient is non-finite ({float(self.last_grad_norm)}), so it cannot be clipped '
                               '(NativeTrainer(error_if_nonfinite=True))')

    def apply_optimizer(self):
        m = self.model
        mirror = m._wcopy if (m.compute_dtype == torch.bfloat16 and m._wcopy is not None) else None
        gscale = 1.0 / self.world
        g = m.grad_flat()
        spans = [(0, m.flat.numel())] if self.kind == 'SGD' else self._adam_spans()
        clip = {}
        if self.clip_mode == 'norm':
            self._grad_norm(spans, gscale)
            clip = dict(total_norm=self.last_grad_norm, max_norm=self.gradient_clip_val, clip_coef_out=self.last_clip_coef)
        elif self.clip_mode == 'value':
            clip = dict(clip_value=self.gradient_clip_val)
        self.step_count += 1
        if self.kind == 'SGD':
            buf, _ = self._state()
            if clip:
                ops.sgd_step_clipped(m.flat, g, buf, self.lr, 0.9, 1e-4, self.step_count == 1, gscale, mirror, **clip)
            else:
                ops.sgd_step(m.flat, g, buf, self.lr, 0.9, 1e-4, self.step_count == 1, gscale, mirror)
        else:
            mm, vv = self._state()
            for a, b in spans:
                args = (m.flat[a:b], g[a:b], mm[a:b], vv[a:b], self.lr, 0.9, 0.999, 1e-7, self.step_count, gscale,
                        mirror[a:b] if mirror is not None else None)
                if clip:
                    ops.adam_step_clipped(*args, **clip)
                else:
                    ops.adam_step(*args)
        if mirror is not None:
            m.mark_weights_synced()
        else:
            m._wcopy_version = None
```

Before: 9.359 million sentences/s.

## Defer split-K weight-gradient reduction into a fused multi-segment Adam step

```diff
diff --git a/include/mts.h b/include/mts.h
--- a/include/mts.h
+++ b/include/mts.h
@@ -46,6 +46,10 @@
              const void* A, int lda, const void* B, int ldb, void* C, int ldc,
              const float* bias, const void* residual, int ldr, void* aux, int ldaux,
              unsigned epilogue, float colscale, int ncols_scaled, void* workspace, size_t workspace_bytes);
+
+int mts_gemm_planes(void* stream, int layout, int M, int N, int K, const void* A, int lda, const void* B, int ldb, float* C,
+                    size_t plan_workspace_bytes, float* planes, size_t planes_bytes, int* splits, size_t* plane_stride);
+int mts_splitk_reduce(void* stream, const float* planes, int splits, int M, int N, float* C, int ldc, int accumulate);
 
 size_t mts_colsum_workspace(int N);
 int mts_colsum(void* stream, int dtype, int M, int N, const void* X, int ldx, float* out, int accumulate,
@@ -278,6 +282,11 @@
                   float lr, float beta1, float beta2, float eps, int step, float grad_scale, void* bf16_copy);
 int mts_sgd_step(void* stream, size_t n, float* param, const float* grad, float* momentum_buf, float lr,
                  float momentum, float weight_decay, int first_step, float grad_scale, void* bf16_copy);
+int mts_adam_step_planes(void* stream, size_t n, float* param, const float* planes, int splits, size_t plane_stride, float* exp_avg,
+                         float* exp_avg_sq, float lr, float beta1, float beta2, float eps, int step, float grad_scale, void* bf16_copy);
+int mts_adam_step_segments(void* stream, int n_segs, const size_t* begin_host, const size_t* len_host, const float* const* planes_host,
+                           const int* splits_host, const size_t* stride_host, float* param, const float* grad, float* exp_avg,
+                           float* exp_avg_sq, float lr, float beta1, float beta2, float eps, int step, float grad_scale, void* bf16_copy);
 size_t mts_grad_norm_workspace(void);
 int mts_grad_norm(void* stream, const float* grad, int n_spans, const size_t* span_begin_host, const size_t* span_end_host,
                   float grad_scale, float* workspace, float* norm_out);
diff --git a/multimodaltopicsegmentation_amd/_lib.py b/multimodaltopicsegmentation_amd/_lib.py
--- a/multimodaltopicsegmentation_amd/_lib.py
+++ b/multimodaltopicsegmentation_amd/_lib.py
@@ -41,6 +41,8 @@
     'mts_gemm_plan': (_i, [_i, _i, _i, _i, _i, _i, _u, _sz, _vp, _vp]),
     'mts_async_status': (_i, []),
     'mts_gemm': (_i, [_vp, _i, _i, _i, _i, _i, _i, _vp, _i, _vp, _i, _vp, _i, _vp, _vp, _i, _vp, _i, _u, _f, _i, _vp, _sz]),
+    'mts_gemm_planes': (_i, [_vp, _i, _i, _i, _i, _vp, _i, _vp, _i, _vp, _sz, _vp, _sz, _vp, _vp]),
+    'mts_splitk_reduce': (_i, [_vp, _vp, _i, _i, _i, _vp, _i, _i]),
     'mts_wgrad_pair_workspace': (_sz, [_i, _i, _i]),
     'mts_wgrad_pair': (_i, [_vp, _i, _i, _i, _vp, _vp, _vp, _i, _vp, _vp, _vp, _i, _i, _i, _i, _vp, _sz]),
     'mts_colsum_workspace': (_sz, [_i]),
@@ -113,6 +115,8 @@
     'mts_crf_viterbi_packed': (_i, [_vp, _i, _i, _i, _vp, _vp, _vp, _vp, _vp, _vp, _vp, _i]),
     'mts_crf_marginals_packed': (_i, [_vp, _i, _i, _i, _i, _vp, _vp, _vp, _vp, _vp, _vp, _vp, _i]),
     'mts_adam_step': (_i, [_vp, _sz, _vp, _vp, _vp, _vp, _f, _f, _f, _f, _i, _f, _vp]),
+    'mts_adam_step_planes': (_i, [_vp, _sz, _vp, _vp, _i, _sz, _vp, _vp, _f, _f, _f, _f, _i, _f, _vp]),
+    'mts_adam_step_segments': (_i, [_vp, _i, _vp, _vp, _vp, _vp, _vp, _vp, _vp, _vp, _vp, _f, _f, _f, _f, _i, _f, _vp]),
     'mts_sgd_step': (_i, [_vp, _sz, _vp, _vp, _vp, _f, _f, _f, _i, _f, _vp]),
     'mts_grad_norm_workspace': (_sz, []),
     'mts_grad_norm': (_i, [_vp, _vp, _i, _vp, _vp, _f, _vp, _vp]),
diff --git a/multimodaltopicsegmentation_amd/csrc/gemm.hip b/multimodaltopicsegmentation_amd/csrc/gemm.hip
--- a/multimodaltopicsegmentation_amd/csrc/gemm.hip
+++ b/multimodaltopicsegmentation_amd/csrc/gemm.hip
@@ -805,9 +805,45 @@
   return MTS_OK;
 }
 
+static int gemm_impl(void* stream, int a_dtype, int c_dtype, int layout, int M, int N, int K, const void* A, int lda,
+                     const void* B, int ldb, void* C, int ldc, const float* bias, const void* residual, int ldr,
+                     void* aux, int ldaux, unsigned epilogue, float colscale, int ncols_scaled, void* workspace, size_t workspace_bytes,
+                     float* own_planes, size_t own_planes_bytes, int* own_splits);
+
 extern "C" int mts_gemm(void* stream, int a_dtype, int c_dtype, int layout, int M, int N, int K, const void* A, int lda,
                         const void* B, int ldb, void* C, int ldc, const float* bias, const void* residual, int ldr,
                         void* aux, int ldaux, unsigned epilogue, float colscale, int ncols_scaled, void* workspace, size_t workspace_bytes) {
+  return gemm_impl(stream, a_dtype, c_dtype, layout, M, N, K, A, lda, B, ldb, C, ldc, bias, residual, ldr, aux, ldaux, epilogue, colscale,
+                   ncols_scaled, workspace, workspace_bytes, nullptr, 0, nullptr);
+}
+
+extern "C" int mts_gemm_planes(void* stream, int layout, int M, int N, int K, const void* A, int lda, const void* B, int ldb, float* C,
+                               size_t plan_workspace_bytes, float* planes, size_t planes_bytes, int* splits, size_t* plane_stride) {
+  MTS_CHECK_ARG(planes && splits && plane_stride, "mts_gemm_planes: null planes / splits / plane_stride");
+  MTS_CHECK_ARG(((uintptr_t)planes % 16) == 0, "mts_gemm_planes: planes must be 16-byte aligned");
+  int sp = 1;
+  const int rc = gemm_impl(stream, MTS_BF16, MTS_F32, layout, M, N, K, A, lda, B, ldb, C, N, nullptr, nullptr, 0, nullptr, 0, 0, 1.0f, 0,
+                           planes, plan_workspace_bytes, planes, planes_bytes, &sp);
+  if (rc) return rc;
+  *splits = sp;
+  *plane_stride = (size_t)M * N;
+  return MTS_OK;
+}
+
+extern "C" int mts_splitk_reduce(void* stream, const float* planes, int splits, int M, int N, float* C, int ldc, int accumulate) {
+  MTS_CHECK_ARG(planes && C && splits >= 1 && M > 0 && N > 0, "mts_splitk_reduce: bad arguments");
+  MTS_CHECK_ARG(N % 4 == 0 && ldc % 4 == 0 && ldc >= N && ((uintptr_t)planes % 16) == 0 && ((uintptr_t)C % 16) == 0,
+                "mts_splitk_reduce: N and ldc must be multiples of 4, planes and C 16-byte aligned");
+  hipLaunchKernelGGL(splitk_reduce_kernel, dim3((unsigned)(((size_t)M * (N / 4) + 255) / 256)), dim3(256), 0, (hipStream_t)stream, planes, splits, M, N,
+                     C, ldc, accumulate ? 1 : 0);
+  MTS_LAUNCH_CHECK("mts_splitk_reduce");
+  return MTS_OK;
+}
+
+static int gemm_impl(void* stream, int a_dtype, int c_dtype, int layout, int M, int N, int K, const void* A, int lda,
+                     const void* B, int ldb, void* C, int ldc, const float* bias, const void* residual, int ldr,
+                     void* aux, int ldaux, unsigned epilogue, float colscale, int ncols_scaled, void* workspace, size_t workspace_bytes,
+                     float* own_planes, size_t own_planes_bytes, int* own_splits) {
   MTS_CHECK_ARG(M > 0 && N > 0 && K > 0, "mts_gemm: bad shape M=%d N=%d K=%d", M, N, K);
   MTS_CHECK_ARG(A && B && C, "mts_gemm: null operand");
   MTS_CHECK_ARG(layout == MTS_NT || layout == MTS_NN || layout == MTS_TN || layout == MTS_TT, "mts_gemm: bad layout %d", layout);
@@ -871,8 +907,11 @@
 
   int splits = 1, use256 = 0;
   const size_t ws_planes = workspace_bytes > MTS_GEMM_WS_HEAD ? workspace_bytes - MTS_GEMM_WS_HEAD : 0;
-  float* const planes = workspace ? (float*)((char*)workspace + MTS_GEMM_WS_HEAD) : nullptr;
+  float* const planes = own_planes ? own_planes : workspace ? (float*)((char*)workspace + MTS_GEMM_WS_HEAD) : nullptr;
   plan_bf16(c_dtype, layout, M, N, K, epilogue, workspace != nullptr && ws_planes > 0, ws_planes, &use256, &splits);
+  MTS_CHECK_ARG(!own_planes || splits == 1 || (size_t)splits * M * N * sizeof(float) <= own_planes_bytes,
+                "mts_gemm_planes: %d planes of %d x %d floats do not fit %zu bytes", splits, M, N, own_planes_bytes);
+  if (own_splits) *own_splits = splits;
   if (use256 && c_dtype != MTS_F32 && ((uintptr_t)C % 16) != 0) use256 = 0;
   g_last_tile = use256 == 2 ? 224 : use256 == 1 ? 256 : 128;
   g_last_splits = splits;
@@ -880,7 +919,7 @@
   bool chained = false;
   if (splits > 1) {
     a.ksplit = ceil_div(ceil_div(K, splits), BK) * BK;
-    chained = g_chain && !use256;
+    chained = g_chain && !use256 && !own_planes;
     if (chained) {
       const size_t nt128 = (size_t)ceil_div(M, BM) * ceil_div(N, BN);
       a.chain = (unsigned*)planes;
@@ -888,7 +927,7 @@
       if (e != hipSuccess) { mts_set_error("mts_gemm: hipMemsetAsync: %s", hipGetErrorString(e)); return MTS_ERR_LAUNCH; }
     } else {
       a.slab = planes;
-      if (use256 == 2 && g_combine && (a.variant == 0 || a.variant == 11 || a.variant == 12) && (size_t)ceil_div(M, 256) * (N / 224) * sizeof(unsigned) <= MTS_GEMM_WS_HEAD &&
+      if (use256 == 2 && g_combine && !own_planes && (a.variant == 0 || a.variant == 11 || a.variant == 12) && (size_t)ceil_div(M, 256) * (N / 224) * sizeof(unsigned) <= MTS_GEMM_WS_HEAD &&
           mts_gemm224t_applies(a, layout, c_dtype == MTS_F32, splits)) {
         a.chain = (unsigned*)workspace;
         chained = true;
@@ -911,7 +950,7 @@
     else launch_bf16<MTS_TN, bf16_t>(a, splits, st);
   }
   if (g_mid_hook) g_mid_hook();
-  if (splits > 1 && !chained)
+  if (splits > 1 && !chained && !own_planes)
     hipLaunchKernelGGL(splitk_reduce_kernel, dim3((unsigned)(((size_t)M * (N / 4) + 255) / 256)), dim3(256), 0, st, (const float*)planes,
                        splits, M, N, (float*)C, ldc, (epilogue & MTS_EPI_ACCUM) ? 1 : 0);
   MTS_LAUNCH_CHECK("mts_gemm(bf16)");
diff --git a/multimodaltopicsegmentation_amd/csrc/optim.hip b/multimodaltopicsegmentation_amd/csrc/optim.hip
--- a/multimodaltopicsegmentation_amd/csrc/optim.hip
+++ b/multimodaltopicsegmentation_amd/csrc/optim.hip
@@ -65,44 +65,125 @@
   return c > 1.f ? 1.f : c;
 }
 
-template <int CLIP>
-__device__ __forceinline__ void adam_loop(size_t n, float* __restrict__ p, const float* __restrict__ g, float* __restrict__ m,
+struct GradFlat {
+  const float* __restrict__ g;
+  __device__ __forceinline__ void load4(size_t i, float (&out)[4]) const { ::load4<float>(g + i, out); }
+  __device__ __forceinline__ float load1(size_t k) const { return g[k]; }
+};
+struct GradPlanes {
+  const float* __restrict__ planes;
+  int splits;
+  size_t stride;
+  __device__ __forceinline__ void load4(size_t i, float (&out)[4]) const {
+    float s[4] = {0.f, 0.f, 0.f, 0.f};
+    const float* __restrict__ p = planes + i;
+    for (int z = 0; z < splits; z += 8) {
+      float v[8][4];
+#pragma unroll
+      for (int u = 0; u < 8; ++u)
+        if (z + u < splits) ::load4<float>(p + (size_t)(z + u) * stride, v[u]);
+#pragma unroll
+      for (int u = 0; u < 8; ++u)
+        if (z + u < splits) {
+#pragma unroll
+          for (int j = 0; j < 4; ++j) s[j] += v[u][j];
+        }
+    }
+#pragma unroll
+    for (int j = 0; j < 4; ++j) out[j] = s[j];
+  }
+  __device__ __forceinline__ float load1(size_t k) const {
+    float s = 0.f;
+    for (int z = 0; z < splits; ++z) s += planes[(size_t)z * stride + k];
+    return s;
+  }
+};
+
+template <int CLIP, typename GRAD>
+__device__ __forceinline__ void adam_group(size_t i, size_t n, float* __restrict__ p, const GRAD g, float* __restrict__ m,
+                                           float* __restrict__ v, float step_size, float b1, float b2, float eps, float bc2_sqrt,
+                                           float gscale, bf16_t* __restrict__ copy, float c) {
+  if (i + 3 < n) {
+    float pv[4], gv[4], mv[4], vv[4];
+    load4<float>(p + i, pv); g.load4(i, gv); load4<float>(m + i, mv); load4<float>(v + i, vv);
+#pragma unroll
+    for (int j = 0; j < 4; ++j) {
+      const float gr = clip_grad<CLIP>(gv[j] * gscale, c);
+      mv[j] = mv[j] + (1.f - b1) * (gr - mv[j]);
+      vv[j] = b2 * vv[j] + (1.f - b2) * gr * gr;
+      const float denom = sqrtf(vv[j]) / bc2_sqrt + eps;
+      pv[j] = pv[j] - step_size * (mv[j] / denom);
+    }
+    store4<float>(p + i, pv); store4<float>(m + i, mv); store4<float>(v + i, vv);
+    if (copy) store4<bf16_t>(copy + i, pv);
+  } else {
+    for (size_t k = i; k < n; ++k) {
+      const float gr = clip_grad<CLIP>(g.load1(k) * gscale, c);
+      const float mm = m[k] + (1.f - b1) * (gr - m[k]);
+      const float vv = b2 * v[k] + (1.f - b2) * gr * gr;
+      m[k] = mm; v[k] = vv;
+      const float pp = p[k] - step_size * (mm / (sqrtf(vv) / bc2_sqrt + eps));
+      p[k] = pp;
+      if (copy) copy[k] = (bf16_t)pp;
+    }
+  }
+}
+
+template <int CLIP, typename GRAD>
+__device__ __forceinline__ void adam_loop(size_t n, float* __restrict__ p, const GRAD g, float* __restrict__ m,
                                           float* __restrict__ v, float lr, float b1, float b2, float eps, float bc1, float bc2_sqrt,
                                           float gscale, bf16_t* __restrict__ copy, float c) {
   const size_t stride = (size_t)gridDim.x * 256 * 4;
   const float step_size = lr / bc1;
-  for (size_t i = ((size_t)blockIdx.x * 256 + threadIdx.x) * 4; i < n; i += stride) {
-    if (i + 3 < n) {
-      float pv[4], gv[4], mv[4], vv[4];
-      load4<float>(p + i, pv); load4<float>(g + i, gv); load4<float>(m + i, mv); load4<float>(v + i, vv);
-#pragma unroll
-      for (int j = 0; j < 4; ++j) {
-        const float gr = clip_grad<CLIP>(gv[j] * gscale, c);
-        mv[j] = mv[j] + (1.f - b1) * (gr - mv[j]);
-        vv[j] = b2 * vv[j] + (1.f - b2) * gr * gr;
-        const float denom = sqrtf(vv[j]) / bc2_sqrt + eps;
-        pv[j] = pv[j] - step_size * (mv[j] / denom);
-      }
-      store4<float>(p + i, pv); store4<float>(m + i, mv); store4<float>(v + i, vv);
-      if (copy) store4<bf16_t>(copy + i, pv);
-    } else {
-      for (size_t k = i; k < n; ++k) {
-        const float gr = clip_grad<CLIP>(g[k] * gscale, c);
-        const float mm = m[k] + (1.f - b1) * (gr - m[k]);
-        const float vv = b2 * v[k] + (1.f - b2) * gr * gr;
-        m[k] = mm; v[k] = vv;
-        const float pp = p[k] - step_size * (mm / (sqrtf(vv) / bc2_sqrt + eps));
-        p[k] = pp;
-        if (copy) copy[k] = (bf16_t)pp;
-      }
-    }
-  }
+  for (size_t i = ((size_t)blockIdx.x * 256 + threadIdx.x) * 4; i < n; i += stride)
+    adam_group<CLIP>(i, n, p, g, m, v, step_size, b1, b2, eps, bc2_sqrt, gscale, copy, c);
 }
 
 __global__ __launch_bounds__(256) void adam_kernel(size_t n, float* __restrict__ p, const float* __restrict__ g, float* __restrict__ m,
                                                    float* __restrict__ v, float lr, float b1, float b2, float eps, float bc1, float bc2_sqrt,
                                                    float gscale, bf16_t* __restrict__ copy) {
-  adam_loop<CLIP_NONE>(n, p, g, m, v, lr, b1, b2, eps, bc1, bc2_sqrt, gscale, copy, 1.f);
+  adam_loop<CLIP_NONE>(n, p, GradFlat{g}, m, v, lr, b1, b2, eps, bc1, bc2_sqrt, gscale, copy, 1.f);
+}
+
+__global__ __launch_bounds__(256) void adam_planes_kernel(size_t n, float* __restrict__ p, const float* __restrict__ planes, int splits,
+                                                          size_t plane_stride, float* __restrict__ m, float* __restrict__ v, float lr, float b1,
+                                                          float b2, float eps, float bc1, float bc2_sqrt, float gscale, bf16_t* __restrict__ copy) {
+  adam_loop<CLIP_NONE>(n, p, GradPlanes{planes, splits, plane_stride}, m, v, lr, b1, b2, eps, bc1, bc2_sqrt, gscale, copy, 1.f);
+}
+
+#define ADAM_MAX_SEGS 16
+struct AdamSegs {
+  size_t begin[ADAM_MAX_SEGS], len[ADAM_MAX_SEGS];
+  const float* planes[ADAM_MAX_SEGS];
+  size_t stride[ADAM_MAX_SEGS];
+  size_t first_group[ADAM_MAX_SEGS + 1];
+  int splits[ADAM_MAX_SEGS];
+  int n;
+};
+
+__global__ __launch_bounds__(256) void adam_segments_kernel(AdamSegs t, float* __restrict__ p, const float* __restrict__ g, float* __restrict__ m,
+                                                            float* __restrict__ v, float lr, float b1, float b2, float eps, float bc1,
+                                                            float bc2_sqrt, float gscale, bf16_t* __restrict__ copy) {
+  const size_t total = t.first_group[t.n], stride = (size_t)gridDim.x * 256;
+  const float step_size = lr / bc1;
+  for (size_t vg = (size_t)blockIdx.x * 256 + threadIdx.x; vg < total; vg += stride) {
+    int k = 0;
+#pragma unroll
+    for (int q = 1; q < ADAM_MAX_SEGS; ++q)
+      if (q < t.n && vg >= t.first_group[q]) k = q;
+    size_t begin = 0, len = 0, pstride = 0, g0 = 0;
+    const float* planes = nullptr;
+    int splits = 0;
+#pragma unroll
+    for (int q = 0; q < ADAM_MAX_SEGS; ++q)
+      if (q == k) { begin = t.begin[q]; len = t.len[q]; pstride = t.stride[q]; g0 = t.first_group[q]; planes = t.planes[q]; splits = t.splits[q]; }
+    const size_t i = (vg - g0) * 4;
+    bf16_t* const cp = copy ? copy + begin : nullptr;
+    if (planes)
+      adam_group<CLIP_NONE>(i, len, p + begin, GradPlanes{planes, splits, pstride}, m + begin, v + begin, step_size, b1, b2, eps, bc2_sqrt, gscale, cp, 1.f);
+    else
+      adam_group<CLIP_NONE>(i, len, p + begin, GradFlat{g + begin}, m + begin, v + begin, step_size, b1, b2, eps, bc2_sqrt, gscale, cp, 1.f);
+  }
 }
 
 template <int CLIP>
@@ -116,7 +197,7 @@
     c = clip_coef(*total_norm, max_norm);
     if (coef_out && blockIdx.x == 0 && threadIdx.x == 0) *coef_out = c;
   }
-  adam_loop<CLIP>(n, p, g, m, v, lr, b1, b2, eps, bc1, bc2_sqrt, gscale, copy, c);
+  adam_loop<CLIP>(n, p, GradFlat{g}, m, v, lr, b1, b2, eps, bc1, bc2_sqrt, gscale, copy, c);
 }
 
 template <int CLIP>
@@ -163,6 +244,55 @@
   return MTS_OK;
 }
 
+static inline bool aligned_to(const void* p, size_t bytes) { return ((uintptr_t)p & (bytes - 1)) == 0; }
+
+extern "C" int mts_adam_step_planes(void* stream, size_t n, float* param, const float* planes, int splits, size_t plane_stride, float* exp_avg,
+                                    float* exp_avg_sq, float lr, float beta1, float beta2, float eps, int step, float grad_scale, void* bf16_copy) {
+  MTS_CHECK_ARG(param && planes && exp_avg && exp_avg_sq && step >= 1, "mts_adam_step_planes: bad arguments");
+  MTS_CHECK_ARG(splits >= 1 && plane_stride >= n, "mts_adam_step_planes: splits must be >= 1 and plane_stride >= n (got %d, %zu)", splits, plane_stride);
+  MTS_CHECK_ARG(plane_stride % 4 == 0 && aligned_to(planes, 16) && aligned_to(param, 16) && aligned_to(exp_avg, 16) && aligned_to(exp_avg_sq, 16) &&
+                    aligned_to(bf16_copy, 8),
+                "mts_adam_step_planes: param, planes and moments must be 16-byte aligned (plane_stride a multiple of 4), bf16_copy 8-byte aligned");
+  if (n == 0) return MTS_OK;
+  const double bc1 = 1.0 - pow((double)beta1, step), bc2 = 1.0 - pow((double)beta2, step);
+  const int blocks = (int)std::min<size_t>(2048, (n / 4 + 255) / 256 + 1);
+  hipLaunchKernelGGL(adam_planes_kernel, dim3(blocks), dim3(256), 0, (hipStream_t)stream, n, param, planes, splits, plane_stride, exp_avg, exp_avg_sq,
+                     lr, beta1, beta2, eps, (float)bc1, (float)sqrt(bc2), grad_scale, (bf16_t*)bf16_copy);
+  MTS_LAUNCH_CHECK("mts_adam_step_planes");
+  return MTS_OK;
+}
+
+extern "C" int mts_adam_step_segments(void* stream, int n_segs, const size_t* begin_host, const size_t* len_host, const float* const* planes_host,
+                                      const int* splits_host, const size_t* stride_host, float* param, const float* grad, float* exp_avg,
+                                      float* exp_avg_sq, float lr, float beta1, float beta2, float eps, int step, float grad_scale, void* bf16_copy) {
+  MTS_CHECK_ARG(param && grad && exp_avg && exp_avg_sq && step >= 1 && begin_host && len_host && planes_host && splits_host && stride_host,
+                "mts_adam_step_segments: bad arguments");
+  MTS_CHECK_ARG(n_segs >= 1 && n_segs <= ADAM_MAX_SEGS, "mts_adam_step_segments: n_segs must be 1..%d (got %d)", ADAM_MAX_SEGS, n_segs);
+  MTS_CHECK_ARG(aligned_to(param, 16) && aligned_to(grad, 16) && aligned_to(exp_avg, 16) && aligned_to(exp_avg_sq, 16) && aligned_to(bf16_copy, 8),
+                "mts_adam_step_segments: param, grad and moments must be 16-byte aligned, bf16_copy 8-byte aligned");
+  AdamSegs t = {};
+  size_t groups = 0;
+  for (int s = 0; s < n_segs; ++s) {
+    MTS_CHECK_ARG(begin_host[s] % 4 == 0, "mts_adam_step_segments: span %d does not begin on a multiple of 4 elements", s);
+    MTS_CHECK_ARG(s == 0 || begin_host[s] >= begin_host[s - 1] + len_host[s - 1], "mts_adam_step_segments: span %d overlaps the one before it", s);
+    if (planes_host[s])
+      MTS_CHECK_ARG(splits_host[s] >= 1 && stride_host[s] >= len_host[s] && stride_host[s] % 4 == 0 && aligned_to(planes_host[s], 16),
+                    "mts_adam_step_segments: span %d: splits >= 1, plane stride >= the span and a multiple of 4, planes 16-byte aligned", s);
+    t.begin[s] = begin_host[s]; t.len[s] = len_host[s]; t.planes[s] = planes_host[s]; t.stride[s] = stride_host[s]; t.splits[s] = splits_host[s];
+    t.first_group[s] = groups;
+    groups += (len_host[s] + 3) / 4;
+  }
+  t.first_group[n_segs] = groups;
+  t.n = n_segs;
+  if (groups == 0) return MTS_OK;
+  const double bc1 = 1.0 - pow((double)beta1, step), bc2 = 1.0 - pow((double)beta2, step);
+  const int blocks = (int)std::min<size_t>(2048, (groups + 255) / 256);
+  hipLaunchKernelGGL(adam_segments_kernel, dim3(blocks), dim3(256), 0, (hipStream_t)stream, t, param, grad, exp_avg, exp_avg_sq, lr, beta1, beta2, eps,
+                     (float)bc1, (float)sqrt(bc2), grad_scale, (bf16_t*)bf16_copy);
+  MTS_LAUNCH_CHECK("mts_adam_step_segments");
+  return MTS_OK;
+}
+
 extern "C" int mts_sgd_step(void* stream, size_t n, float* param, const float* grad, float* momentum_buf, float lr, float momentum,
                             float weight_decay, int first_step, float grad_scale, void* bf16_copy) {
   MTS_CHECK_ARG(param && grad && momentum_buf, "mts_sgd_step: bad arguments");
@@ -173,8 +303,6 @@
   MTS_LAUNCH_CHECK("mts_sgd_step");
   return MTS_OK;
 }
-
-static inline bool aligned_to(const void* p, size_t bytes) { return ((uintptr_t)p & (bytes - 1)) == 0; }
 
 static int check_clip_args(const char* name, const float* total_norm, float max_norm, float clip_value) {
   MTS_CHECK_ARG(max_norm >= 0.f, "%s: max_norm must be >= 0 (got %g)", name, (double)max_norm);
diff --git a/multimodaltopicsegmentation_amd/ops.py b/multimodaltopicsegmentation_amd/ops.py
--- a/multimodaltopicsegmentation_amd/ops.py
+++ b/multimodaltopicsegmentation_amd/ops.py
@@ -112,7 +112,7 @@
     ws, ws_bytes = None, 0
     if layout in (L.TN, L.TT) and c_dt == L.F32 and K >= 2048:
         if a_dt == L.BF16:
-            ws_bytes = 8192 + min(16, max(1, K // 1024)) * M * N * 4
+            ws_bytes = _splitk_ws_bytes(M, N, K)
         elif -(-M // 128) * -(-N // 128) <= 128:
             ws_bytes = min(16, 256 // (-(-M // 128) * -(-N // 128)), max(1, K // 512)) * M * N * 4
         if ws_bytes:
@@ -140,6 +140,39 @@
 
 def linear_wgrad(dy, x, out, **kw):
     return gemm(L.TN, dy, x, out, M=dy.shape[1], N=x.shape[1], K=dy.shape[0], **kw)
+
+
+def _splitk_ws_bytes(M, N, K):
+    return 8192 + min(16, max(1, K // 1024)) * M * N * 4
+
+
+def wgrad_planes_supported(dy, x, out):
+    return (dy.dtype == torch.bfloat16 and x.dtype == torch.bfloat16 and dy.is_cuda and out.dtype == torch.float32 and out.is_contiguous()
+            and dy.shape[0] >= 2048)
+
+
+def linear_wgrad_planes(dy, x, out, get_planes):
+    M, N, K = dy.shape[1], x.shape[1], dy.shape[0]
+    assert wgrad_planes_supported(dy, x, out) and tuple(out.shape) == (M, N)
+    ws_bytes = _splitk_ws_bytes(M, N, K)
+    sp = ctypes.c_int(1)
+    check(lib.mts_gemm_plan(L.BF16, L.F32, L.TN, M, N, K, 0, ws_bytes, None, ctypes.byref(sp)))
+    planes = get_planes(sp.value * M * N if sp.value > 1 else 4)
+    stride = ctypes.c_size_t(0)
+    key = (L.TN, L.BF16, L.F32, M, N, K)
+    with _timed(('gemm', *key, _plan_cache.get(key, 0))):
+        check(lib.mts_gemm_planes(stream_ptr(), L.TN, M, N, K, ptr(dy), dy.stride(0), ptr(x), x.stride(0), ptr(out), ws_bytes, ptr(planes),
+                                  planes.numel() * 4, ctypes.byref(sp), ctypes.byref(stride)))
+    if key not in _plan_cache:
+        t = ctypes.c_int(0)
+        lib.mts_gemm_last_plan(ctypes.byref(t), None)
+        _plan_cache[key] = t.value
+    return (planes, sp.value, stride.value) if sp.value > 1 else None
+
+
+def splitk_reduce(planes, splits, M, N, out, accumulate=False):
+    check(lib.mts_splitk_reduce(stream_ptr(), ptr(planes), int(splits), M, N, ptr(out), out.stride(0) if out.dim() == 2 else N, int(accumulate)))
+    return out
 
 
 def wgrad_pair_supported(dy1, x1):
@@ -802,6 +835,27 @@
                             eps, step, grad_scale, ptr(bf16_copy)))
 
 
+def adam_step_planes(param, planes, splits, plane_stride, exp_avg, exp_avg_sq, lr, beta1, beta2, eps, step, grad_scale=1.0, bf16_copy=None):
+    check(lib.mts_adam_step_planes(stream_ptr(), param.numel(), ptr(param), ptr(planes), int(splits), int(plane_stride), ptr(exp_avg),
+                                   ptr(exp_avg_sq), lr, beta1, beta2, eps, step, grad_scale, ptr(bf16_copy)))
+
+
+ADAM_MAX_SEGMENTS = 16
+
+
+def adam_step_segments(segments, param, grad, exp_avg, exp_avg_sq, lr, beta1, beta2, eps, step, grad_scale=1.0, bf16_copy=None):
+    for k in range(0, len(segments), ADAM_MAX_SEGMENTS):
+        seg = segments[k:k + ADAM_MAX_SEGMENTS]
+        n = len(seg)
+        begin = (ctypes.c_size_t * n)(*[a for a, _, _ in seg])
+        length = (ctypes.c_size_t * n)(*[b - a for a, b, _ in seg])
+        planes = (ctypes.c_void_p * n)(*[ptr(pl[0]) if pl is not None else None for _, _, pl in seg])
+        splits = (ctypes.c_int * n)(*[pl[1] if pl is not None else 0 for _, _, pl in seg])
+        stride = (ctypes.c_size_t * n)(*[pl[2] if pl is not None else 0 for _, _, pl in seg])
+        check(lib.mts_adam_step_segments(stream_ptr(), n, begin, length, planes, splits, stride, ptr(param), ptr(grad), ptr(exp_avg), ptr(exp_avg_sq),
+                                         lr, beta1, beta2, eps, step, grad_scale, ptr(bf16_copy)))
+
+
 def sgd_step(param, grad, buf, lr, momentum, weight_decay, first_step, grad_scale=1.0, bf16_copy=None):
     check(lib.mts_sgd_step(stream_ptr(), param.numel(), ptr(param), ptr(grad), ptr(buf), lr, momentum, weight_decay,
                            int(first_step), grad_scale, ptr(bf16_copy)))
diff --git a/multimodaltopicsegmentation_amd/taggers.py b/multimodaltopicsegmentation_amd/taggers.py
--- a/multimodaltopicsegmentation_amd/taggers.py
+++ b/multimodaltopicsegmentation_amd/taggers.py
@@ -122,6 +122,17 @@
     def _grads_ready(self, a, b):
         if self._grad_hook is not None and b > a:
             self._grad_hook(a, b)
+
+    supports_grad_deferral = False
+    defer_grads = False
+    _pending_grads = ()
+
+    def materialize_pending_grads(self):
+        g = self.grad_flat()
+        for off, n, planes, splits, stride in self._pending_grads:
+            assert stride == n
+            ops.splitk_reduce(planes, splits, 1, n, g[off:off + n])
+        self._pending_grads = []
 
     def mark_weights_synced(self):
         self._wcopy_version = self._weights_version()
@@ -255,6 +266,14 @@
         wf, pf = self._weights(), self._flat
         g = self.grad_flat()
         Gv = lambda key, rows, cols: self._lt(g, names, key, rows, cols)
+        defer = self.defer_grads and self.supports_grad_deferral and self._grad_hook is None and wgrad_direct
+
+        def wgrad_keep(dy, x, gview, key):
+            if not (defer and ops.wgrad_planes_supported(dy, x, gview)):
+                return wgrad(dy, x, gview)
+            kept = ops.linear_wgrad_planes(dy, x, gview, lambda n: ws.get('planes.' + names[key][0], 1, n, torch.float32, dev).view(-1))
+            if kept is not None:
+                self._pending_grads.append(((gview.data_ptr() - g.data_ptr()) // 4, gview.numel(), *kept))
         ds2 = ws.get('ds2', N, D, dt, dev)
         if not tail_done:
             ops.layernorm_bwd(S['s2'], dh, self._lt(pf, names, 'ln2w', 1, D).view(-1), S['mean2'], S['rstd2'], ds2,
@@ -297,7 +316,7 @@
             ds1d = ws.get('ds1d', N, D, dt, dev)
             ops.dropout_bwd(ds1, ds1d, S['m1'], pdrop)
             ops.colsum(ds1d, Gv('bo', 1, D).view(-1))
-        wgrad(ds1d, S['ctx'], Gv('wo', D, D))
+        wgrad_keep(ds1d, S['ctx'], Gv('wo', D, D), 'wo')
         o_wo = lay.entries[names['wo'][0]][0]
         self._grads_ready(o_wo, tail_end)
         dctx = ws.get('dctx', N, D, dt, dev)
@@ -317,7 +336,7 @@
                 wgrad(dqkv[:, i * D:(i + 1) * D], S['hin'], gq[i * D:(i + 1) * D])
                 self._grads_ready(o_qkv + i * D * D, o_qkv + (i + 1) * D * D if i < 2 else o_wo)
         else:
-            wgrad(dqkv, S['hin'], Gv('wqkv', 3 * D, D))
+            wgrad_keep(dqkv, S['hin'], Gv('wqkv', 3 * D, D), 'wqkv')
             self._grads_ready(o_qkv, o_wo)
         dhin = ws.get(f'dhin{slot}', N, D, dt, dev)
         ops.linear_dgrad(dqkv, self._lt(wf, names, 'wqkv', 3 * D, D), dhin, residual=ds1)
@@ -510,6 +529,7 @@
         G = lambda name: lay.view(g, name)
         nl = len(self.radii)
         dh = None
+        self._pending_grads = []
         side = self._side_stream(dev) if (self.overlap_wgrad and self._grad_hook is None and dev.type == 'cuda') else None
         main = torch.cuda.current_stream(dev) if side is not None else None
 
@@ -601,6 +621,7 @@
 
 class Transformer_segmenter(_TransformerEncoderTagger):
     grad_hooks_cover_all = True
+    supports_grad_deferral = True
 
     def __init__(self, tagset_size, embedding_dim, hidden_dim, num_layers=6, nheads=8, dropout_in=0.0, dropout_out=0.0,
                  batch_first=True, loss_fn='CrossEntropy', positional_encoding=True, threshold=None, restricted=True,
diff --git a/multimodaltopicsegmentation_amd/trainer.py b/multimodaltopicsegmentation_amd/trainer.py
--- a/multimodaltopicsegmentation_amd/trainer.py
+++ b/multimodaltopicsegmentation_amd/trainer.py
@@ -5,6 +5,22 @@
 import torch.distributed as dist
 
 from . import ops
+
+
+def _split_spans(spans, pending):
+    out = []
+    for a, b in spans:
+        for off, n, planes, splits, stride in pending:
+            if a <= off and off + n <= b:
+                if off > a:
+                    out.append((a, off, None))
+                out.append((off, off + n, (planes, splits, stride)))
+                a = off + n
+            else:
+                assert off + n <= a or off >= b, 'a pending gradient straddles an optimizer span'
+        if b > a:
+            out.append((a, b, None))
+    return out
 
 
 def shard_batch(batch, rank, world):
@@ -69,6 +85,7 @@
         self.error_if_nonfinite = bool(error_if_nonfinite)
         self.last_grad_norm = self.last_clip_coef = None
         self._clip_stats = self._clip_ws = None
+        self.last_deferred = 0
 
     def _state(self):
         flat = self.model.flat
@@ -176,6 +193,29 @@
         self._pending = []
         self._inflight_shards = []
         m._grad_hook = self._on_grads_ready if overlapped else None
+        m.defer_grads = self._defers_grads()
+        try:
+            loss = self._loss_and_grad(m, batch, x, lengths, tags)
+        finally:
+            m.defer_grads = False
+        if overlapped:
+            for h, span in self._pending:
+                self._finish(h, span)
+            self._pending = []
+            self._inflight_shards = []
+        else:
+            self.allreduce_grads()
+        self.apply_optimizer()
+        return loss
+
+    defer_grads = os.environ.get('MTS_DEFER_GRADS', '1') != '0'
+
+    def _defers_grads(self):
+        m = self.model
+        return (self.defer_grads and self.kind != 'SGD' and self.clip_mode is None and self.world == 1 and not self.always_hook
+                and getattr(m, 'supports_grad_deferral', False) and not getattr(m, 'overlap_wgrad', False))
+
+    def _loss_and_grad(self, m, batch, x, lengths, tags):
         if self.cosine_loss:
             segments = batch['src_segments']
             if batch.get('src_tokens2') is not None and hasattr(m, '_rnn2'):
@@ -188,14 +228,6 @@
             loss, _ = m.loss_and_grad(x, lengths, tags, batch['domain'], True)
         else:
             loss, _ = m.loss_and_grad(x, lengths, tags, True)
-        if overlapped:
-            for h, span in self._pending:
-                self._finish(h, span)
-            self._pending = []
-            self._inflight_shards = []
-        else:
-            self.allreduce_grads()
-        self.apply_optimizer()
         return loss
 
     def fit(self, train, val=None, **kw):
@@ -239,6 +271,11 @@
         gscale = 1.0 / self.world
         g = m.grad_flat()
         spans = [(0, m.flat.numel())] if self.kind == 'SGD' else self._adam_spans()
+        pending = sorted(getattr(m, '_pending_grads', ()) or (), key=lambda e: e[0])
+        if pending and (self.kind == 'SGD' or self.clip_mode is not None):
+            m.materialize_pending_grads()
+            pending = []
+        self.last_deferred = len(pending)
         clip = {}
         if self.clip_mode == 'norm':
             self._grad_norm(spans, gscale)
@@ -254,6 +291,10 @@
                 ops.sgd_step(m.flat, g, buf, self.lr, 0.9, 1e-4, self.step_count == 1, gscale, mirror)
         else:
             mm, vv = self._state()
+            if pending:
+                ops.adam_step_segments(_split_spans(spans, pending), m.flat, g, mm, vv, self.lr, 0.9, 0.999, 1e-7, self.step_count, gscale, mirror)
+                m._pending_grads = []
+                spans = []
             for a, b in spans:
                 args = (m.flat[a:b], g[a:b], mm[a:b], vv[a:b], self.lr, 0.9, 0.999, 1e-7, self.step_count, gscale,
                         mirror[a:b] if mirror is not None else None)
```

After: 9.409 million sentences/s, median of 6. Within noise of the previous version (+0.5%).
